# ctu-mrs/vofod

Hardware: AMD Instinct MI355X
Metric: LiDAR frames/sec (131k-pt OS1-128) at 1/2/4/8 MI355X + HBM roofline % (higher is better)
Workload: dtype f32; 1 GPU; os1-128 128x1024 scans, 0.25 m voxels, batched process_scan (configs[1] scan shape in configs[3]'s batched form); points_per_frame=131072, map_voxels=19480981, map_warm_scans=96, gpu_max_hw_queues=4

## Files before the change

vofod_amd/csrc/driver_aux.h:

```cpp
#pragma once

namespace
{

int gscan(vofod_handle* h, const uint32_t* d_in, uint32_t n, uint32_t* d_out, uint32_t* d_bsum, uint32_t* d_total)
{
  const uint32_t nblk = (n + vr::GS_EPB - 1) / vr::GS_EPB;
  if (n == 0)
  {
    HIPCHK(hipMemsetAsync(d_out, 0, sizeof(uint32_t), h->stream));
    if (d_total)
      HIPCHK(hipMemsetAsync(d_total, 0, sizeof(uint32_t), h->stream));
    return VOFOD_OK;
  }
  KLAUNCH(h, vr::k_gscan_a, dim3(nblk), dim3(256), d_in, n, d_bsum);
  KLAUNCH(h, vr::k_gscan_b, dim3(1), dim3(1024), d_bsum, nblk, d_total);
  KLAUNCH(h, vr::k_gscan_c, dim3(nblk), dim3(256), d_in, n, d_bsum, d_out);
  HIPCHK(hipGetLastError());
  return VOFOD_OK;
}

int sep_ensure_words(vofod_handle* h, size_t n_words)
{
  vr::SepState& s = h->sep;
// ... 546 lines not shown
    if (F == 1)
      nt = 1;
    h->pool.reset(new vt::Pool(nt));
  }
  if (do_reset(h) != VOFOD_OK)
    return fail(VOFOD_ERR_DEVICE);
  h->sure_background_sufficient = false;
  h->background_pts_sufficient = false;
  h->last_detection_id = 0;
  (void)hipDeviceSynchronize();
  *out = h;
  return VOFOD_OK;
}

static int world_clear(vofod_handle* h);

int vofod_reset(vofod_handle* h)
{
  if (!h)
    return VOFOD_ERR_INVALID_ARG;
  ApiLock lock(h);
  VCHK(admit(h, WS0_FREE | MAP_UNREAD));
  if (h->world.enabled)
    VCHK(world_clear(h));
  h->wsync.end_chains();
  const int r = do_reset(h);
  h->sure_background_sufficient = false;
  h->background_pts_sufficient = false;
  h->last_detection_id = 0;
  h->cf_off = false;
  forget_detections(h);
  return r;
}

int vofod_set_dynamic_params(vofod_handle* h, const vofod_dyn_params* dp)
{
  if (!h || !dp)
    return VOFOD_ERR_INVALID_ARG;
  ApiLock lock(h, ApiLock::LOCK_ONLY);
  VCHK(admit(h, NEEDS_NOTHING));
  h->dp = *dp;
  return VOFOD_OK;
}

const char* vofod_last_error_string(vofod_handle* h) { return h ? h->err.c_str() : "null handle"; }

int vofod_get_status(vofod_handle* h, vofod_status_info* out)
{
  if (!h || !out)
    return VOFOD_ERR_INVALID_ARG;
  ApiLock lock(h, ApiLock::LOCK_ONLY);
  VCHK(admit(h, NEEDS_NOTHING));
  out->detection_its = h->detection_its;
  out->last_detection_id = h->last_detection_id;
  out->background_pts_sufficient = h->background_pts_sufficient;
  out->sure_background_sufficient = h->sure_background_sufficient;
  out->raycast_pending = h->raycast_pending;
  out->map_size[0] = h->mg.sx;
  out->map_size[1] = h->mg.sy;
  out->map_size[2] = h->mg.sz;
  for (int a = 0; a < 3; a++)
    out->map_offset[a] = h->mg.off[a];
  return VOFOD_OK;
}

int vofod_raycast_begin(vofod_handle* h, const vofod_scan* scan, const float tf[12])
{
  if (!h || !tf)
    return VOFOD_ERR_INVALID_ARG;
  ApiLock lock(h);
  VCHK(admit(h, WS0_FREE));
  return raycast_begin_locked(h, scan, tf, nullptr);
}

int vofod_set_raycast_motion(vofod_handle* h, int on)
{
  if (!h)
    return VOFOD_ERR_INVALID_ARG;
  ApiLock lock(h, ApiLock::LOCK_ONLY);
  VCHK(admit(h, WS0_FREE | MAP_UNREAD | NO_RAYCAST_PASS));
  h->raycast_motion = on != 0;
  return VOFOD_OK;
}

int vofod_set_raycast_exact(vofod_handle* h, int on)
{
  if (!h)
    return VOFOD_ERR_INVALID_ARG;
  ApiLock lock(h, ApiLock::LOCK_ONLY);
  VCHK(admit(h, WS0_FREE | MAP_UNREAD | NO_RAYCAST_PASS));
  if (on && h->ray_log2_units < 0)
  {
    h->err = "exact raycast accumulation: sensor_hrays * sensor_vrays * (2 * voxel_size + 1) does not fit in 32 bits";
    return VOFOD_ERR_INDEX_OVERFLOW;
  }
  h->raycast_exact = on != 0;
  return VOFOD_OK;
}

int vofod_raycast_units(vofod_handle* h, uint32_t* units, size_t n, int32_t* log2_units_per_m)
{
  if (!h || !units || !log2_units_per_m)
    return VOFOD_ERR_INVALID_ARG;
  ApiLock lock(h);
  VCHK(admit(h, NEEDS_NOTHING));
  if (!h->raycast_pending || !h->ray_pass_exact)
    return VOFOD_ERR_NOT_PENDING;
  if (n != h->mg.n)
    return VOFOD_ERR_SIZE_MISMATCH;
  HIPCHK(hipStreamSynchronize(h->stream));
  HIPCHK(hipMemcpy(units, h->d_ray.p, n * sizeof(uint32_t), hipMemcpyDeviceToHost));
  *log2_units_per_m = h->ray_log2_units;
  return VOFOD_OK;
}

int vofod_raycast_finish(vofod_handle* h)
{
  if (!h)
    return VOFOD_ERR_INVALID_ARG;
  ApiLock lock(h);
  VCHK(admit(h, MAP_UNREAD));
  return raycast_finish_locked(h);
}

int vofod_sepclusters_begin(vofod_handle* h, int* sure)
{
  if (!h)
    return VOFOD_ERR_INVALID_ARG;
  ApiLock lock(h);
  VCHK(admit(h, WS0_FREE));
  return sepclusters_begin_locked(h, sure);
}

int vofod_sepclusters_finish(vofod_handle* h)
{
  if (!h)
    return VOFOD_ERR_INVALID_ARG;
  ApiLock lock(h);
  VCHK(admit(h, WS0_FREE | MAP_UNREAD));
  return sepclusters_finish_locked(h);
}

int vofod_voxel_grid_weighted(vofod_handle* h, const vofod_cloud_view* in, float leaf, int align, const float align_center[3], vofod_point_xyzr* out, uint32_t* keys,
                              size_t cap, size_t* n_out, vofod_grid_desc* grid)
{
  if (!h || !in || !(leaf > 0) || (align && !align_center) || in->n > 0x7fffffffu)
    return VOFOD_ERR_INVALID_ARG;
  ApiLock lock(h);
  VCHK(admit(h, WS0_FREE));
  GridParams g;
  FrameHdr hdr{};
  const float l[3] = {leaf, leaf, leaf};
  if (in->n == 0)
  {
    if (n_out)
      *n_out = 0;
    if (grid)
      *grid = vofod_grid_desc{{leaf, leaf, leaf}, {0, 0, 0}, {0, 0, 0}, {0, 0, 0}};
    return VOFOD_OK;
  }
  const int r = voxelize_cloud(h, h->aux, in, g, l, align != 0, align_center, hdr);
  if (r != VOFOD_OK)
  {
    if (n_out)
      *n_out = 0;
    return r;
  }
  return copy_grid_out(h, h->aux, g, hdr, out, keys, cap, n_out, grid);
}

int vofod_voxel_grid_counted(vofod_handle* h, const vofod_cloud_view* in, float leaf, float threshold, vofod_point_xyzr* out, uint32_t* keys, size_t cap, size_t* n_out,
                             vofod_grid_desc* grid)
{
  if (!h || !in || !(leaf > 0) || !in->intensity || in->n > 0x7fffffffu)
    return VOFOD_ERR_INVALID_ARG;
  ApiLock lock(h);
  VCHK(admit(h, WS0_FREE));
  GridParams g;
  FrameHdr hdr{};
  const float l[3] = {leaf, leaf, leaf};
  if (in->n == 0)
  {
    if (n_out)
      *n_out = 0;
    return VOFOD_OK;
  }
  int r = voxelize_cloud(h, h->aux, in, g, l, false, nullptr, hdr);
  if (r != VOFOD_OK)
  {
    if (n_out)
      *n_out = 0;
    return r;
  }
  const uint32_t P = static_cast<uint32_t>(in->n);
  VCHK(sep_ensure_words(h, 1));
  VCHK(sep_ensure_pts(h, P));
  const FrameArgs& a = h->aux.h_args[0];
  KLAUNCH(h, vr::k_flag_over, dim3((P + 255) / 256), dim3(256), a.intensity, a.stride, P, threshold, h->sep.d_sure);
  VCHK(counted_tail(h, h->aux, hdr.V, P, h->sep.d_sure));
  HIPCHK(hipStreamSynchronize(h->stream));
  return copy_grid_out(h, h->aux, g, hdr, out, keys, cap, n_out, grid);
}

int vofod_cluster(vofod_handle* h, const vofod_point_xyzr* pts, const uint32_t* keys, const vofod_grid_desc* grid, size_t n, float tolerance, uint32_t* labels,
                  size_t* n_clusters)
{
  if (!h || (!pts && n) || !labels || !keys || !grid || !(tolerance > 0) || n > 0x7fffffffu)
    return VOFOD_ERR_INVALID_ARG;
  ApiLock lock(h);
  VCHK(admit(h, WS0_FREE));
  if (n_clusters)
    *n_clusters = 0;
  if (n == 0)
    return VOFOD_OK;
  const uint64_t cells = static_cast<uint64_t>(grid->div_b[0]) * grid->div_b[1] * grid->div_b[2];
  if (grid->div_b[0] <= 0 || grid->div_b[1] <= 0 || grid->div_b[2] <= 0 || cells > 0x7fffffffull)
    return VOFOD_ERR_INVALID_ARG;
  for (size_t i = 0; i < n; i++)
    if (keys[i] >= cells || (i && keys[i] <= keys[i - 1]))
    {
      h->err = "vofod_cluster: keys must be strictly ascending lattice keys";
      return VOFOD_ERR_INVALID_ARG;
    }
  Workspace& ws = h->aux;
  const uint32_t words = static_cast<uint32_t>((cells + 63) / 64);
  const uint32_t need_bricks = static_cast<uint32_t>(std::min<uint64_t>(static_cast<uint64_t>((grid->div_b[0] + 3) / 4) * ((grid->div_b[1] + 3) / 4) * ((grid->div_b[2] + 3) / 4), 1u << 28));
  VCHK(grow_workspace(h, ws, "workspace allocation: ", 1, static_cast<uint32_t>(n), static_cast<uint32_t>(n), words + 64, need_bricks));
  GridParams g;
  const float zero[3] = {0, 0, 0};
  fill_grid_params(h, g, grid->leaf, false, zero, ws);
  FrameHdr hdr{};
  hdr.n_in = static_cast<uint32_t>(n);
  hdr.status = VOFOD_OK;
  for (int a = 0; a < 3; a++)
  {
    hdr.offset[a] = grid->offset[a];
    hdr.min_b[a] = grid->min_b[a];
    hdr.div_b[a] = grid->div_b[a];
  }
  hdr.n_cells = static_cast<uint32_t>(cells);
  hdr.n_words = words;
  hdr.V = static_cast<uint32_t>(n);
  std::vector<unsigned long long> bm(words + 2, 0ull);
  for (size_t i = 0; i < n; i++)
    bm[keys[i] >> 6] |= 1ull << (keys[i] & 63);
  std::vector<uint32_t> prefix(words + 2, 0u), ident(n);
  uint32_t run = 0;
  for (uint32_t w = 0; w < words; w++)
  {
    prefix[w] = run;
    run += __builtin_popcountll(bm[w]);
  }
  for (size_t i = 0; i < n; i++)
    ident[i] = static_cast<uint32_t>(i);
  std::vector<int32_t> cbox(6 * n);
  for (size_t i = 0; i < n; i++)
    for (int c = 0; c < 3; c++)
    {
      cbox[6 * i + c] = 0x7fffffff;
      cbox[6 * i + 3 + c] = static_cast<int32_t>(0x80000000u);
    }
  HIPCHK(hipMemcpyAsync(ws.d_hdrs, &hdr, sizeof(hdr), hipMemcpyHostToDevice, h->stream));
  ws.bitmap_clean = false;
  HIPCHK(hipMemcpyAsync(ws.d_bitmaps, bm.data(), sizeof(unsigned long long) * (words + 2), hipMemcpyHostToDevice, h->stream));
  HIPCHK(hipMemcpyAsync(ws.d_wprefix, prefix.data(), sizeof(uint32_t) * (words + 2), hipMemcpyHostToDevice, h->stream));
  HIPCHK(hipMemcpyAsync(ws.va.pts, pts, sizeof(float4) * n, hipMemcpyHostToDevice, h->stream));
  HIPCHK(hipMemcpyAsync(ws.va.key, keys, sizeof(uint32_t) * n, hipMemcpyHostToDevice, h->stream));
  HIPCHK(hipMemcpyAsync(ws.va.parent, ident.data(), sizeof(uint32_t) * n, hipMemcpyHostToDevice, h->stream));
  HIPCHK(hipMemsetAsync(ws.va.csize, 0, sizeof(uint32_t) * n, h->stream));
  HIPCHK(hipMemsetAsync(ws.va.cclose, 0, sizeof(uint32_t) * n, h->stream));
  HIPCHK(hipMemcpyAsync(ws.va.cbox, cbox.data(), sizeof(int32_t) * 6 * n, hipMemcpyHostToDevice, h->stream));
  float cmax = 0;
  for (int a = 0; a < 3; a++)
    cmax = std::max({cmax, std::fabs(grid->offset[a]), std::fabs(grid->offset[a] + grid->leaf[a] * (grid->div_b[a] + 1))});
  vofod_handle::ClusterTables* ct = nullptr;
  VCHK(cluster_tables(h, g, tolerance, cmax, &ct));
  VCHK(launch_cluster(h, ws, plan_cluster_only(h, ws, ct), g, ct));
  HIPCHK(hipMemcpyAsync(labels, ws.d_labels, sizeof(uint32_t) * n, hipMemcpyDeviceToHost, h->stream));
  HIPCHK(hipStreamSynchronize(h->stream));
  if (n_clusters)
  {
    size_t c = 0;
    for (size_t i = 0; i < n; i++)
      c += labels[i] == i;
    *n_clusters = c;
  }
  return VOFOD_OK;
}

int vofod_profile_enable(vofod_handle* h, int on)
{
  if (!h)
    return VOFOD_ERR_INVALID_ARG;
  ApiLock lock(h);
  VCHK(admit(h, NEEDS_NOTHING));
  (void)hipStreamSynchronize(h->stream);
  for (auto& r : h->prof.recs)
  {
    h->prof.pool.push_back(r.a);
    h->prof.pool.push_back(r.b);
  }
  h->prof.recs.clear();
  h->prof.on = on != 0;
  return VOFOD_OK;
}

size_t vofod_profile_read(vofod_handle* h, char* names, double* ms, uint64_t* calls, size_t cap)
{
  if (!h || !names || !ms || !calls)
    return 0;
  ApiLock lock(h);
  if (admit(h, NEEDS_NOTHING) != VOFOD_OK)
    return 0;
  (void)hipStreamSynchronize(h->stream);
  std::vector<std::string> order;
  std::map<std::string, std::pair<double, uint64_t>> acc;
  for (auto& r : h->prof.recs)
  {
    float t = 0;
    (void)hipEventElapsedTime(&t, r.a, r.b);
    std::string nm = r.name;
    const size_t c = nm.rfind(':');
    if (c != std::string::npos)
      nm = nm.substr(c + 1);
    if (!acc.count(nm))
      order.push_back(nm);
    acc[nm].first += t;
    acc[nm].second += 1;
    h->prof.pool.push_back(r.a);
    h->prof.pool.push_back(r.b);
  }
  h->prof.recs.clear();
  size_t n = 0;
  for (const auto& nm : order)
  {
    if (n >= cap)
      break;
    std::memset(names + 64 * n, 0, 64);
    std::strncpy(names + 64 * n, nm.c_str(), 63);
    ms[n] = acc[nm].first;
    calls[n] = acc[nm].second;
    n++;
  }
  return n;
}

}
```

vofod_amd/csrc/frame_prof.h:

```cpp
#pragma once

namespace
{

struct Quantiles
{
  double mean = 0, median = 0, p90 = 0, max = 0;
  explicit Quantiles(std::vector<double>& v)
  {
    std::sort(v.begin(), v.end());
    for (double x : v)
      mean += x / v.size();
    median = v[v.size() / 2];
    p90 = v[v.size() * 9 / 10];
    max = v.back();
  }
  void json(FILE* fp, const char* name) const { std::fprintf(fp, "\"%s\": {\"mean\": %.2f, \"median\": %.2f, \"p90\": %.2f, \"max\": %.2f}", name, mean, median, p90, max); }
};

int slab_emit_prof_buffer(vofod_handle* h, unsigned long long*& d_prof)
{
  if (!h->d_prof_slab && std::getenv("VOFOD_LDS_PROF"))
    HIPCHK(h->d_prof_slab.alloc(16 * 4096));
  d_prof = h->d_prof_slab;
  return VOFOD_OK;
}

int print_slab_emit_prof(vofod_handle* h, uint32_t n)
{
  std::vector<unsigned long long> all(16 * n);
  HIPCHK(hipStreamSynchronize(h->stream));
  HIPCHK(hipMemcpy(all.data(), h->d_prof_slab, sizeof(unsigned long long) * 16 * n, hipMemcpyDeviceToHost));
  const unsigned long long* t = all.data();
  std::fprintf(stderr, "[k_slab_emit] keys %.1f | zero %.1f mark %.1f count+scan %.1f out+emit %.1f us (all slabs of frame 0)\n", t[0] * 0.01, t[1] * 0.01, t[2] * 0.01, t[3] * 0.01, t[4] * 0.01);
  unsigned long long t0 = ~0ull, t1 = 0;
  for (uint32_t f = 0; f < n; f++)
  {
    t0 = std::min(t0, all[16 * f + 5]);
    t1 = std::max(t1, all[16 * f + 6]);
  }
  double smax = 0;
  std::vector<double> dur;
  std::vector<std::pair<double, uint32_t>> byd;
  for (uint32_t f = 0; f < n; f++)
  {
    dur.push_back((all[16 * f + 6] - all[16 * f + 5]) * 0.01);
    byd.push_back({dur.back(), f});
    smax = std::max(smax, (all[16 * f + 5] - t0) * 0.01);
  }
  std::sort(byd.begin(), byd.end());
  for (size_t q : {size_t(0), byd.size() / 4, byd.size() / 2, 3 * byd.size() / 4, byd.size() - 1})
  {
    const uint32_t f = byd[q].second;
    std::fprintf(stderr, "[k_slab_emit]   frame %u: %.1f us, keys %llu, zero %.1f mark %.1f count %.1f emit %.1f\n", f, byd[q].first, all[16 * f + 7], all[16 * f + 1] * 0.01, all[16 * f + 2] * 0.01,
                 all[16 * f + 3] * 0.01, all[16 * f + 4] * 0.01);
  }
  const Quantiles q(dur);
  std::fprintf(stderr, "[k_slab_emit] %u workgroups: span %.1f us, per-workgroup min %.1f mean %.1f max %.1f us, latest start +%.1f us\n", n, (t1 - t0) * 0.01, dur.front(), q.mean, q.max, smax);
  return VOFOD_OK;
}

int frame_prof_slots(vofod_handle* h, Workspace& ws, unsigned long long*& d_prof)
{
  DevBuf<unsigned long long>& d_prof_all = h->d_prof_ccl;
  if (!d_prof_all && std::getenv("VOFOD_LDS_PROF"))
  {
    HIPCHK(d_prof_all.alloc(FR_PROF_WORDS));
    HIPCHK(hipMemset(d_prof_all, 0, sizeof(unsigned long long) * FR_PROF_WORDS));
  }
  ws.prof_deferred = false;
  uint32_t prof_slot0 = 0;
  if (d_prof_all && std::atoi(std::getenv("VOFOD_LDS_PROF") ? std::getenv("VOFOD_LDS_PROF") : "0") == 2 && ws.F <= 256)
    for (int t = 0; t < vofod_handle::MAX_INFLIGHT; t++)
      if (&ws == h->slot(t))
      {
        ws.prof_deferred = true;
        prof_slot0 = 256u * static_cast<uint32_t>(t);
      }
  ws.prof_slot0 = prof_slot0;
  d_prof = d_prof_all ? d_prof_all + 32 * static_cast<size_t>(prof_slot0) : nullptr;
  return VOFOD_OK;
}

int print_frame_prof(vofod_handle* h, uint32_t s0, uint32_t cnt, bool sync)
{
  unsigned long long* d_prof = h->d_prof_ccl;
  std::vector<unsigned long long> t(32 * cnt);
  if (sync)
    HIPCHK(hipStreamSynchronize(h->stream));
  HIPCHK(hipMemcpy(t.data(), d_prof + 32 * static_cast<size_t>(s0), sizeof(unsigned long long) * 32 * cnt, hipMemcpyDeviceToHost));
  unsigned long long* d_wave = d_prof + 32 * static_cast<size_t>(FR_PROF_FRAMES) + 32 * static_cast<size_t>(s0);
  std::vector<unsigned long long> tw(32 * cnt);
  HIPCHK(hipMemcpy(tw.data(), d_wave, sizeof(unsigned long long) * 32 * cnt, hipMemcpyDeviceToHost));
  if (const char* rawf = std::getenv("VOFOD_LDS_PROF_RAW"))
  {
    struct RawLog
    {
      std::vector<unsigned long long> v;
      std::string path;
      uint64_t launch = 0;
      ~RawLog()
      {
        if (FILE* fp = std::fopen(path.c_str(), "w"))
        {
          for (size_t i = 0; i + 3 < v.size(); i += 4)
            std::fprintf(fp, "%llu %.2f %.2f %u %u %u %u\n", v[i], v[i + 1] * 0.01, v[i + 2] * 0.01, static_cast<unsigned>(v[i + 3] >> 32) & 15u, static_cast<unsigned>(v[i + 3] >> 13) & 7u,
                         static_cast<unsigned>(v[i + 3] >> 12) & 1u, static_cast<unsigned>(v[i + 3] >> 8) & 15u);
          std::fclose(fp);
        }
      }
    };
    static RawLog log;
    log.path = rawf;
    for (uint32_t f = 0; f < cnt; f++)
      if (t[32 * f + 13])
      {
        const unsigned long long rec[4] = {log.launch, t[32 * f], t[32 * f + 13], t[32 * f + 21]};
        log.v.insert(log.v.end(), rec, rec + 4);
      }
    log.launch++;
    HIPCHK(hipMemsetAsync(d_prof + 32 * static_cast<size_t>(s0), 0, sizeof(unsigned long long) * 32 * cnt, h->stream));
    HIPCHK(hipMemsetAsync(d_wave, 0, sizeof(unsigned long long) * 32 * cnt, h->stream));
    return VOFOD_OK;
  }
  static const char* names[13] = {"bits", "prefix", "words", "rank-a/b", "rank-c", "emit", "extras", "probe", "adjacent", "far", "exact", "minima+stats", "labels"};
  std::vector<std::pair<double, uint32_t>> byd;
  unsigned long long t0 = ~0ull, t1 = 0;
  for (uint32_t f = 0; f < cnt; f++)
  {
    if (!t[32 * f + 13])
      continue;
    byd.push_back({(t[32 * f + 13] - t[32 * f]) * 0.01, f});
    t0 = std::min(t0, t[32 * f]);
    t1 = std::max(t1, t[32 * f + 13]);
  }
  std::sort(byd.begin(), byd.end());
  double mean = 0;
  for (auto& b : byd)
    mean += b.first / byd.size();
  for (size_t q : {size_t(0), byd.size() / 2, byd.size() - 1})
  {
    if (byd.empty())
      break;
    const uint32_t f = byd[q].second;
    if (t[32 * f + 31] == ~0ull)
    {
      auto us = [&](int a, int b) { return (t[32 * f + b] - t[32 * f + a]) * 0.01; };
      const double t_count = us(15, 14), t_closebits = us(3, 15);
      std::fprintf(stderr,
                   "[k_frame_lds_far] frame %u: %.1f us | keys %llu V %llu bricks %llu pure-far bricks %llu far clusters %llu candidate members %llu | input+fragile %.1f prefix %.1f words %.1f count %.1f closebits "
                   "%.1f rank-a/b %.1f rank-c %.1f emit %.1f extras %.1f near+far %.1f open %.1f stats %.1f table %.1f members %.1f\n",
                   f, byd[q].first, t[32 * f + 27], t[32 * f + 29], t[32 * f + 26], t[32 * f + 24], t[32 * f + 25], t[32 * f + 30], us(0, 1), us(1, 2), us(2, 3), t_count, t_closebits, us(14, 4), us(4, 5),
                   us(5, 6), us(6, 7), us(7, 8), us(8, 9), us(9, 10), us(10, 11), us(11, 13));
      continue;
    }
    std::fprintf(stderr, "[k_frame_lds] frame %u: %.1f us | keys %llu V %llu bricks %llu extras %llu hits %llu open %llu surviving %llu |", f, byd[q].first, t[32 * f + 27], t[32 * f + 29],
                 t[32 * f + 26], t[32 * f + 28], t[32 * f + 24], t[32 * f + 25], t[32 * f + 30]);
    for (int i = 0; i < 13; i++)
      std::fprintf(stderr, " %s %.1f", names[i], (t[32 * f + i + 1] - t[32 * f + i]) * 0.01);
    std::fprintf(stderr, " (count %.1f of rank-a/b; %llu bricks outside the largest component, %llu far hits)\n", (t[32 * f + 14] - t[32 * f + 3]) * 0.01, t[32 * f + 31] & 0xffffffffull,
                 t[32 * f + 31] >> 32);
  }
  if (!byd.empty())
    std::fprintf(stderr, "[k_frame_lds] %zu workgroups: span %.1f us, mean %.1f us\n", byd.size(), (t1 - t0) * 0.01, mean);
  if (const char* jf = std::getenv("VOFOD_LDS_PROF_JSON"); jf && !byd.empty() && t[32 * byd[0].second + 31] == ~0ull)
  {
    static const int cuts[][2] = {{0, 16}, {16, 17}, {17, 18}, {18, 19}, {19, 20}, {20, 1}, {1, 2}, {2, 3}, {15, 14}, {3, 15}, {14, 4}, {4, 5}, {5, 6}, {6, 7}, {7, 8}, {8, 9}, {9, 10}, {10, 11}, {11, 13}, {0, 13}};
    static const char* cnames[] = {"input", "input_wait", "grid", "grid_wait", "fragile", "fragile_wait", "prefix", "words", "count", "closebits", "rank_ab", "rank_c", "emit", "extras_restore", "cf_edges", "cf_open", "cf_stats", "cf_table", "cf_members", "total"};
    if (FILE* fp = std::fopen(jf, "a"))
    {
      double busy = 0;
      for (auto& b : byd)
        busy += b.first;
      std::fprintf(fp, "{\"frames\": %zu, \"span_us\": %.1f, \"t0_abs_us\": %.1f, \"busy_us_sum\": %.1f, \"phases\": {", byd.size(), (t1 - t0) * 0.01, t0 * 0.01, busy);
      for (size_t c = 0; c < sizeof(cuts) / sizeof(cuts[0]); c++)
      {
        std::vector<double> v;
        for (auto& b : byd)
          v.push_back((t[32 * b.second + cuts[c][1]] - t[32 * b.second + cuts[c][0]]) * 0.01);
        std::fprintf(fp, "%s", c ? ", " : "");
        Quantiles(v).json(fp, cnames[c]);
      }
      std::vector<double> st, en;
      for (auto& b : byd)
      {
        st.push_back((t[32 * b.second] - t0) * 0.01);
        en.push_back((t[32 * b.second + 13] - t0) * 0.01);
      }
      std::sort(st.begin(), st.end());
      std::sort(en.begin(), en.end());
      std::vector<double> w_mean, w_last, w_share;
      for (auto& b : byd)
      {
        const unsigned long long* w = &tw[32 * b.second];
        const unsigned long long f0 = t[32 * b.second];
        double e_sum = 0, e_max = 0, s_sum = 0;
        int nw = 0;
        for (int k = 0; k < FR_THREADS / 64; k++)
          if (w[2 * k] > f0)
          {
            const double e = (w[2 * k] - f0) * 0.01;
            e_sum += e;
            e_max = std::max(e_max, e);
            s_sum += w[2 * k + 1] / e;
            nw++;
          }
        if (nw)
        {
          w_mean.push_back(e_sum / nw);
          w_last.push_back(e_max);
          w_share.push_back(s_sum / nw);
        }
      }
      std::fprintf(fp, "}");
      if (!w_mean.empty())
      {
        std::fprintf(fp, ", \"input_waves\": {");
        Quantiles(w_mean).json(fp, "mean_wave_end");
        std::fprintf(fp, ", ");
        Quantiles(w_last).json(fp, "last_wave_end");
        std::fprintf(fp, ", ");
        Quantiles(w_share).json(fp, "load_wait_pct");
        std::fprintf(fp, "}");
      }
      std::fprintf(fp, ", \"start_us\": {\"median\": %.1f, \"max\": %.1f}, \"end_us\": {\"median\": %.1f, \"max\": %.1f}", st[st.size() / 2], st.back(), en[en.size() / 2], en.back());
      std::vector<double> bx, ex, fi, to, lag;
      for (auto& b : byd)
      {
        const unsigned long long a0 = t[32 * b.second + 22], pk = t[32 * b.second + 23];
        if (!a0)
          continue;
        const double d1 = (pk & 0xfffffull) * 0.01, d2 = ((pk >> 20) & 0xfffffull) * 0.01, d3 = ((pk >> 40) & 0xfffffull) * 0.01;
        bx.push_back(d1);
        ex.push_back(d2 - d1);
        fi.push_back(d3 - d2);
        to.push_back(d3);
        lag.push_back((static_cast<double>(a0) - static_cast<double>(t[32 * b.second + 13])) * 0.01);
      }
      if (!to.empty())
      {
        std::fprintf(fp, ", \"tail\": {");
        Quantiles(bx).json(fp, "boxes_gates");
        std::fprintf(fp, ", ");
        Quantiles(ex).json(fp, "flood_fills");
        std::fprintf(fp, ", ");
        Quantiles(fi).json(fp, "records");
        std::fprintf(fp, ", ");
        Quantiles(to).json(fp, "total");
        std::fprintf(fp, ", ");
        Quantiles(lag).json(fp, "start_after_frame_end");
        std::fprintf(fp, "}");
      }
      std::fprintf(fp, "}\n");
      std::fclose(fp);
    }
  }
  HIPCHK(hipMemset(d_prof + 32 * static_cast<size_t>(s0), 0, sizeof(unsigned long long) * 32 * cnt));
  HIPCHK(hipMemset(d_wave, 0, sizeof(unsigned long long) * 32 * cnt));
  return VOFOD_OK;
}

int print_deferred_prof(vofod_handle* h, Workspace& ws, uint32_t n)
{
  if (!ws.prof_deferred || !h->d_prof_ccl)
    return VOFOD_OK;
  ws.prof_deferred = false;
  return print_frame_prof(h, ws.prof_slot0, n, false);
}

}
```

vofod_amd/csrc/frames_collect.h:

```cpp
#pragma once

namespace
{

int adopt_status(vofod_handle* h, Workspace& ws, uint32_t n)
{
  if (ws.plan.dtail)
    for (uint32_t f = 0; f < n; f++)
      ws.h_packed[f].hdr.status = ws.h_dets[f].status;
  for (uint32_t f = 0; f < n; f++)
    if (ws.h_packed[f].hdr.status == CCL_RETRY_STATUS)
    {
      h->lds_ccl_off = true;
      ws.rerun = true;
      ws.job_n = n;
      ws.bitmap_clean = false;
      return CCL_RETRY_STATUS;
    }
  return VOFOD_OK;
}

void book_map_images(vofod_handle* h, Workspace& ws)
{
  if (ws.plan.mapbits_patched && ws.h_packed[0].hdr.status == VOFOD_OK && h->mapbits_valid)
  {
    h->bgcount_stale = true;
    h->mapbits_gen++;
  }
  else
    h->mapbits_valid = false;
}

int check_close_first_overflow(vofod_handle* h, Workspace& ws, uint32_t n)
{
  for (uint32_t f = 0; f < n; f++)
    if (ws.h_packed[f].hdr.status == CF_RETRY_STATUS)
    {
      h->cf_off = true;
      h->cf_off_bg = h->n_bg_voxels;
      ws.rerun = true;
      ws.job_n = n;
      return CCL_RETRY_STATUS;
    }
  return VOFOD_OK;
}

struct RecordSink
{
  vofod_handle* h;
  Workspace& ws;
  const FrameCall& call;
  vofod_detection* out;
  size_t cap;
  uint32_t* n_out_per_frame;
  size_t total = 0, frame_begin = 0;
  RecordSink(vofod_handle* h_, Workspace& ws_, const FrameCall& call_, vofod_detection* out_, size_t cap_, uint32_t* n_out_per_frame_)
      : h(h_), ws(ws_), call(call_), out(out_), cap(cap_), n_out_per_frame(n_out_per_frame_)
  {
    ws.det_begin(call.submitted, call.g);
  }
  void add(uint32_t f, uint32_t root, const float center[3], uint32_t n_points, double conf_sum)
  {
    const vofod_detection det = vt::make_detection(h->last_detection_id++, call.tfs + 12 * f, center, n_points, conf_sum, f, h->sp, *call.dp);
    ws.det_refs.push_back({det.id, f, root, n_points});
    if (out && total < cap)
      out[total] = det;
    total++;
  }
  void frame_done(uint32_t f)
  {
    if (n_out_per_frame)
      n_out_per_frame[f] = static_cast<uint32_t>(total - frame_begin);
    frame_begin = total;
  }
  int close(int ret, size_t* n_out)
  {
    *n_out = total;
    if (total > cap)
      ret = VOFOD_ERR_CAPACITY;
    ws.det_valid = ret == VOFOD_OK;
    return ret;
  }
};

int device_tail_records(vofod_handle* h, Workspace& ws, const FrameCall& call, vofod_detection* out, size_t cap, uint32_t* n_out_per_frame, size_t* n_out)
{
  const uint32_t n = call.n;
  int ret = VOFOD_OK;
  if (call.submitted && out)
  {
    size_t need = 0;
    for (uint32_t f = 0; f < n; f++)
      need += ws.h_dets[f].n;
    if (need > cap)
    {
      ws.pending = true;
      *n_out = need;
      return VOFOD_ERR_CAPACITY;
    }
  }
  RecordSink sink(h, ws, call, out, cap, n_out_per_frame);
  for (uint32_t f = 0; f < n; f++)
  {
    const vtd::FrameDets& D = ws.h_dets[f];
    if (D.status != VOFOD_OK)
      ret = D.status;
    for (uint32_t i = 0; i < D.n; i++)
      sink.add(f, D.d[i].root, D.d[i].center, D.d[i].n_points, D.d[i].conf_sum);
    sink.frame_done(f);
  }
  if (trace_on())
    std::fprintf(stderr, "[vofod trace] n=%u device tail: sync %.3f end %.3f ms, %zu detections\n", n, call.tr_sync1, ms_since(call.t0), sink.total);
  return sink.close(ret, n_out);
}

int device_tail_overflow_records(vofod_handle* h, Workspace& ws, const FrameCall& call, uint32_t fb, vofod_detection* out, size_t cap, uint32_t* n_out_per_frame, size_t* n_out)
{
  if (fb & vtd::TAIL_FB_EXPLORE)
  {
    h->err = "device tail: flood-fill work list overflow";
    return VOFOD_ERR_DEVICE;
  }
  std::vector<vtd::TailCluster> tc(vtd::TP_MAXC);
  std::vector<vc::ExploreResult> res(vtd::TP_MAXC);
  HIPCHK(hipMemcpy(tc.data(), ws.d_tailc, sizeof(vtd::TailCluster) * vtd::TP_MAXC, hipMemcpyDeviceToHost));
  HIPCHK(hipMemcpy(res.data(), h->explore.d_results, sizeof(vc::ExploreResult) * vtd::TP_MAXC, hipMemcpyDeviceToHost));
  RecordSink sink(h, ws, call, out, cap, n_out_per_frame);
  for (int c = 0; c < vtd::TP_MAXC; c++)
    if (tc[c].job >= 0 && tc[c].job < vtd::TP_MAXC && res[tc[c].job].floating)
      sink.add(0u, tc[c].root, tc[c].obb_center, tc[c].n_members, res[tc[c].job].conf_sum);
  sink.frame_done(0u);
  return sink.close(VOFOD_OK, n_out);
}

struct FrameTail
{
  std::vector<HostCluster> cl;
  vt::MemberIndex by_root;
  std::vector<int> job_of;
  bool host_fallback = false;
  std::vector<ClusterRec> recs_big;
  std::vector<CandMemberX> members_big;
  bool big_recs = false, big_members = false;
  std::vector<vc::ExploreJob> jobs;
  std::vector<int> members;
};

struct ExploreWork
{
  std::vector<vc::ExploreJob> jobs;
  std::vector<uint32_t> job_begin;
  std::vector<int> job_members;
  std::vector<vc::ExploreResult> results;
};

int fetch_big_tables(vofod_handle* h, Workspace& ws, const GridParams& g, uint32_t n, std::vector<FrameTail>& tails, int& ret)
{
  for (uint32_t f = 0; f < n; f++)
  {
    FrameTail& T = tails[f];
    const FrameHdr& hdr = ws.h_packed[f].hdr;
    if (hdr.status != VOFOD_OK)
      ret = hdr.status;
    T.big_recs = hdr.C > SPEC_C;
    T.big_members = hdr.n_cand > SPEC_M;
    if (T.big_recs)
    {
      T.recs_big.resize(hdr.C);
      HIPCHK(hipMemcpy(T.recs_big.data(), ws.d_table + static_cast<size_t>(f) * ws.vox_cap, sizeof(ClusterRec) * hdr.C, hipMemcpyDeviceToHost));
    }
    if (T.big_members)
    {
      T.members_big.resize(hdr.n_cand);
      CandMemberX* d_tmp = static_cast<CandMemberX*>(ws.d_members_big);
      KLAUNCH(h, k_gather_members, dim3((hdr.n_cand + 255) / 256), dim3(256), g, f, hdr.n_cand, ws.d_cand, ws.va, d_tmp);
      HIPCHK(hipMemcpyAsync(T.members_big.data(), d_tmp, sizeof(CandMemberX) * hdr.n_cand, hipMemcpyDeviceToHost, h->stream));
      HIPCHK(hipStreamSynchronize(h->stream));
    }
  }
  return VOFOD_OK;
}

void prep_frame_tail(const vofod_handle* h, const PackedFrame& pf, uint32_t f, const float* tf, const vt::TailParams& tp, FrameTail& T)
{
  const FrameHdr& hdr = pf.hdr;
  const ClusterRec* recs = T.big_recs ? T.recs_big.data() : pf.table;
  const CandMemberX* members = T.big_members ? T.members_big.data() : pf.members;
  T.cl.resize(hdr.C);
  for (uint32_t c = 0; c < hdr.C; c++)
    T.cl[c].rec = recs[c];
  std::sort(T.cl.begin(), T.cl.end(), [](const HostCluster& a, const HostCluster& b) {
    if (a.rec.size != b.rec.size)
      return a.rec.size > b.rec.size;
    return a.rec.root < b.rec.root;
  });
  {
    std::vector<std::pair<uint64_t, vt::Member>> tmp(hdr.n_cand);
    for (uint32_t i = 0; i < hdr.n_cand; i++)
    {
      const CandMemberX& m = members[i];
      tmp[i] = {(static_cast<uint64_t>(m.root) << 32) | m.v, vt::Member{m.v, {m.x, m.y, m.z}, m.count}};
    }
    T.by_root.build(tmp);
  }
  T.job_of.assign(hdr.C, -1);
  std::vector<vc::ExploreJob>& jl = T.jobs;
  std::vector<int>& ml = T.members;
  for (uint32_t ci = 0; ci < hdr.C; ci++)
  {
    HostCluster& c = T.cl[ci];
    if (c.rec.close)
      continue;
    c.cclass = VOFOD_CLASS_INVALID;
    if (!c.rec.cand)
      continue;
    const vt::MemberSpan mem = T.by_root.of(c.rec.root);
    auto get = [&](size_t i, float p[3]) {
      for (int a = 0; a < 3; a++)
        p[a] = mem[i].p[a];
    };
    c.gates = vt::classify_gates(static_cast<uint32_t>(mem.size()), get, tf, tp, h->hg.off, h->hg.vs_inv, h->hg.s);
    if (c.gates.passed && !c.gates.explore)
      c.cclass = VOFOD_CLASS_UNKNOWN;
    if (!c.gates.explore)
      continue;
    vc::ExploreJob job{};
    job.frame = f;
    job.n_members = static_cast<uint32_t>(mem.size());
    job.member_off = static_cast<uint32_t>(ml.size() / 3);
    job.R = c.gates.R;
    for (int a = 0; a < 3; a++)
    {
      job.box_lo[a] = c.gates.box_lo[a];
      job.box_hi[a] = c.gates.box_hi[a];
    }
    for (const vt::Member& m : mem)
    {
      int o[3];
      h->hg.coordToIdx(m.p, o);
      ml.insert(ml.end(), o, o + 3);
    }
    if (job.R > vc::EX_MAX_R || job.R < 0)
      T.host_fallback = true;
    T.job_of[ci] = static_cast<int>(jl.size());
    jl.push_back(job);
  }
  if (jl.size() > vc::EX_MAX_JOBS)
    T.host_fallback = true;
}

void concat_jobs(std::vector<FrameTail>& tails, ExploreWork& w)
{
  const uint32_t n = static_cast<uint32_t>(tails.size());
  w.job_begin.assign(n + 1, 0);
  for (uint32_t f = 0; f < n; f++)
  {
    w.job_begin[f] = static_cast<uint32_t>(w.jobs.size());
    const uint32_t jbase = static_cast<uint32_t>(w.jobs.size()), mbase = static_cast<uint32_t>(w.job_members.size() / 3);
    for (vc::ExploreJob j : tails[f].jobs)
    {
      j.member_off += mbase;
      j.result_slot = static_cast<uint32_t>(w.jobs.size());
      w.jobs.push_back(j);
    }
    w.job_members.insert(w.job_members.end(), tails[f].members.begin(), tails[f].members.end());
    for (int& ji : tails[f].job_of)
      if (ji >= 0)
        ji += static_cast<int>(jbase);
  }
  w.job_begin[n] = static_cast<uint32_t>(w.jobs.size());
  w.results.resize(w.jobs.size());
}

int explore_on_device(vofod_handle* h, const FrameCall& call, ExploreWork& w, float thr_new, bool no_update)
{
  const uint32_t n = call.n;
  VCHK(ensure_explore(h, h->explore, h->ws.F, w.jobs.size(), w.job_members.size() / 3));
  StreamScope tail_scope(h, call.submitted ? h->stream_tail : nullptr);
  ExploreBufs& eb = h->explore;
  if (h->ev_explore)
    HIPCHK(hipStreamWaitEvent(h->stream, h->ev_explore, 0));
  HIPCHK(hipMemcpyAsync(eb.d_jobs, w.jobs.data(), sizeof(vc::ExploreJob) * w.jobs.size(), hipMemcpyHostToDevice, h->stream));
  HIPCHK(hipMemcpyAsync(eb.d_job_begin, w.job_begin.data(), sizeof(uint32_t) * (n + 1), hipMemcpyHostToDevice, h->stream));
  HIPCHK(hipMemcpyAsync(eb.d_members, w.job_members.data(), sizeof(int) * w.job_members.size(), hipMemcpyHostToDevice, h->stream));
  const vc::ExploreParams ep = explore_params(*call.dp, thr_new, no_update);
  KLAUNCH(h, vc::k_explore, dim3(n), dim3(64), ep, h->mg, eb.d_jobs, eb.d_job_begin, eb.d_job_begin + 1, eb.d_members, h->d_map, eb.d_overlay, eb.d_stack, eb.d_explored, eb.d_touched,
          eb.d_ovl_list, eb.d_ovl_count, eb.d_results, eb.d_visited);
  HIPCHK(hipMemcpyAsync(w.results.data(), eb.d_results, sizeof(vc::ExploreResult) * w.jobs.size(), hipMemcpyDeviceToHost, h->stream));
  if (h->ev_explore)
    HIPCHK(hipEventRecord(h->ev_explore, h->stream));
  HIPCHK(hipStreamSynchronize(h->stream));
  if (!no_update)
    h->mapbits_valid = false;
  return VOFOD_OK;
}

void extract_detections(RecordSink& sink, const FrameTail& T, uint32_t f, const std::vector<vc::ExploreResult>& results)
{
  for (size_t ci = 0; ci < T.cl.size(); ci++)
  {
    const HostCluster& c = T.cl[ci];
    if (c.rec.close || c.cclass != VOFOD_CLASS_MAV)
      continue;
    sink.add(f, c.rec.root, c.gates.obb_center, static_cast<uint32_t>(T.by_root.of(c.rec.root).size()), results[T.job_of[ci]].conf_sum);
  }
  sink.frame_done(f);
}

int fill_debug_view(vofod_handle* h, Workspace& ws, const GridParams& g, uint32_t f, const FrameTail& T, bool far_view, vofod_scan_debug& d, int& ret)
{
  const FrameHdr& hdr = ws.h_packed[f].hdr;
  d.n_input_after_crop = hdr.n_in;
  d.n_bg_voxels = h->n_bg_voxels;
  d.background_pts_sufficient = h->background_pts_sufficient;
  d.sure_background_sufficient = h->sure_background_sufficient;
  uint32_t n_shown = hdr.C;
  if (far_view && !hdr.far_only)
  {
    n_shown = 0;
    for (uint32_t c = 0; c < hdr.C; c++)
      n_shown += T.cl[c].rec.close ? 0u : 1u;
  }
  d.n_weighted = hdr.V;
  d.n_clusters = n_shown;
  if ((d.weighted || d.labels) && d.weighted_cap < hdr.V)
    ret = VOFOD_ERR_CAPACITY;
  else
  {
    if (d.weighted && hdr.V)
      HIPCHK(hipMemcpy(d.weighted, ws.va.pts + static_cast<size_t>(f) * ws.vox_cap, sizeof(float4) * hdr.V, hipMemcpyDeviceToHost));
    if (d.labels && hdr.V)
    {
      HIPCHK(hipMemcpy(d.labels, ws.d_labels + static_cast<size_t>(f) * ws.vox_cap, sizeof(uint32_t) * hdr.V, hipMemcpyDeviceToHost));
      if (far_view && !hdr.far_only)
      {
        std::vector<uint32_t> far_roots;
        for (uint32_t c = 0; c < hdr.C; c++)
          if (!T.cl[c].rec.close)
            far_roots.push_back(T.cl[c].rec.root);
        std::sort(far_roots.begin(), far_roots.end());
        for (uint32_t v = 0; v < hdr.V; v++)
          if (!std::binary_search(far_roots.begin(), far_roots.end(), d.labels[v]))
            d.labels[v] = CF_LABEL_NONE;
      }
    }
  }
  if (d.clusters)
  {
    if (d.clusters_cap < n_shown)
      ret = VOFOD_ERR_CAPACITY;
    else
      for (uint32_t c = 0, c_out = 0; c < hdr.C; c++)
      {
        const HostCluster& hc = T.cl[c];
        if (far_view && hc.rec.close)
          continue;
        vofod_cluster_info& ci = d.clusters[c_out++];
        ci.first_member = hc.rec.root;
        ci.n_points = hc.rec.size;
        ci.is_close = hc.rec.close;
        ci.cclass = hc.cclass;
        for (int a = 0; a < 3; a++)
        {
          ci.aabb_min[a] = (static_cast<float>(hc.rec.imin[a]) + 0.5f) * g.leaf[a] + hdr.offset[a];
          ci.aabb_max[a] = (static_cast<float>(hc.rec.imax[a]) + 0.5f) * g.leaf[a] + hdr.offset[a];
          ci.obb_center[a] = hc.gates.evaluated ? hc.gates.obb_center[a] : NAN;
        }
        ci.obb_size = hc.gates.obb_size;
      }
  }
  return VOFOD_OK;
}

int host_tail(vofod_handle* h, Workspace& ws, const FrameCall& call, const double dev_ms[4], vofod_detection* out, size_t cap, uint32_t* n_out_per_frame, size_t* n_out)
{
  const uint32_t n = call.n;
  const vofod_dyn_params& dp = *call.dp;
  vofod_scan_debug* dbg = call.dbg;
  const bool no_update = call.flags & VOFOD_SCAN_NO_MAP_UPDATE;
  const auto t_tail = clk::now();
  const float thr_new = static_cast<float>(dp.voxel_map__thresholds__new_obstacles);
  const float thr_frontiers = static_cast<float>(dp.voxel_map__thresholds__frontiers);
  const vt::TailParams tp = tail_params(h, dp);
  int ret = VOFOD_OK;
  std::vector<FrameTail> tails(n);
  ExploreWork w;
  VCHK(fetch_big_tables(h, ws, call.g, n, tails, ret));
  h->pool->parallel_for(n, [&](uint32_t f) { prep_frame_tail(h, ws.h_packed[f], f, call.tfs + 12 * f, tp, tails[f]); });
  concat_jobs(tails, w);
  const double tr_prep = ms_since(call.t0);

  bool any_host = std::getenv("VOFOD_EXPLORE") && std::strcmp(std::getenv("VOFOD_EXPLORE"), "host") == 0;
  for (const FrameTail& T : tails)
    any_host |= T.host_fallback;
  if (!w.jobs.empty() && !any_host)
    VCHK(explore_on_device(h, call, w, thr_new, no_update));
  const double tr_explore = ms_since(call.t0);

  RecordSink sink(h, ws, call, out, cap, n_out_per_frame);
  for (uint32_t f = 0; f < n; f++)
  {
    FrameTail& T = tails[f];
    if (any_host && w.job_begin[f + 1] > w.job_begin[f])
    {
      VCHK(host_explore_frame(h, T.cl, T.by_root, T.job_of, w.jobs, w.results, no_update, thr_frontiers, thr_new, dp));
    }
    for (size_t ci = 0; ci < T.cl.size(); ci++)
      if (const int ji = T.job_of[ci]; ji >= 0)
        T.cl[ci].cclass = w.results[ji].floating ? VOFOD_CLASS_MAV : VOFOD_CLASS_UNKNOWN;
    extract_detections(sink, T, f, w.results);
    if (dbg)
    {
      vofod_scan_debug& d = dbg[f];
      VCHK(fill_debug_view(h, ws, call.g, f, T, dbg[0].far_only != 0, d, ret));
      for (int i = 0; i < 4; i++)
        d.stage_ms[i] = dev_ms[i];
      d.stage_ms[4] = ms_since(t_tail);
      d.stage_ms[5] = ms_since(call.t0);
    }
  }
  if (trace_on())
  {
    size_t sumC = 0, sumCand = 0, sumEval = 0;
    for (uint32_t f = 0; f < n; f++)
    {
      sumC += ws.h_packed[f].hdr.C;
      sumCand += ws.h_packed[f].hdr.n_cand;
      for (const auto& c : tails[f].cl)
        sumEval += c.gates.evaluated;
    }
    std::fprintf(stderr, "[vofod trace] n=%u launch %.3f sync1 %.3f prep %.3f explore %.3f end %.3f ms jobs %zu C %zu cand_members %zu evaluated %zu\n", n, call.tr_launch, call.tr_sync1, tr_prep,
                 tr_explore, ms_since(call.t0), w.jobs.size(), sumC, sumCand, sumEval);
  }
  return sink.close(ret, n_out);
}

int collect_frames(vofod_handle* h, Workspace& ws, FrameCall& call, vofod_detection* out, size_t cap, uint32_t* n_out_per_frame, size_t* n_out)
{
  const uint32_t n = call.n;
  if (n == 0)
  {
    GridParams g{};
    g.vox_cap = ws.vox_cap;
    ws.det_begin(call.submitted, g);
    ws.det_valid = true;
    return VOFOD_OK;
  }
  const bool no_update = call.flags & VOFOD_SCAN_NO_MAP_UPDATE;
  if (call.submitted)
  {
    HIPCHK(hipEventSynchronize(ws.ev_done));
    ws.pending = false;
  }
  else
    HIPCHK(hipStreamSynchronize(h->stream));
  VCHK(print_deferred_prof(h, ws, n));
  call.tr_sync1 = ms_since(call.t0);

  VCHK(adopt_status(h, ws, n));
  if (!no_update)
    book_map_images(h, ws);
  VCHK(latch_background(h));
  VCHK(check_close_first_overflow(h, ws, n));
  if (!no_update && !call.rc_done)
  {
    h->detection_its++;
    if (call.flags & VOFOD_SCAN_AUTO_RAYCAST)
    {
      if (h->raycast_pending)
        raycast_finish_locked(h);
      else
        raycast_begin_locked(h, &call.scans[0], call.tfs, staged_pose_table(ws, call.scans[0]));
    }
  }
  double dev_ms[4] = {0, 0, 0, 0};
  if (call.dbg)
    for (int i = 0; i < 4; i++)
    {
      float ms = 0;
      (void)hipEventElapsedTime(&ms, call.ev[i], call.ev[i + 1]);
      dev_ms[i] = ms;
    }

  if (ws.plan.dtail)
  {
    uint32_t fb = 0;
    for (uint32_t f = 0; f < n; f++)
      fb |= ws.h_dets[f].fallback;
    if (!fb)
      return device_tail_records(h, ws, call, out, cap, n_out_per_frame, n_out);
    if (!no_update && (fb & (vtd::TAIL_FB_DETS | vtd::TAIL_FB_EXPLORE)))
      return device_tail_overflow_records(h, ws, call, fb, out, cap, n_out_per_frame, n_out);
    VCHK(read_back_full(h, ws, call.g, n));
    HIPCHK(hipStreamSynchronize(h->stream));
  }
  return host_tail(h, ws, call, dev_ms, out, cap, n_out_per_frame, n_out);
}

template <class First, class Again>
int with_reruns(First&& first, Again&& again)
{
  int r = first();
  for (int attempt = 0; attempt < 2 && r == CCL_RETRY_STATUS; attempt++)
    r = again();
  return r;
}

int process_frames(vofod_handle* h, const vofod_scan* scans, const float* tfs, uint32_t n, int flags, vofod_detection* out, size_t cap, uint32_t* n_out_per_frame, size_t* n_out,
                   vofod_scan_debug* dbg)
{
  auto once = [&] {
    FrameCall call{false, scans, tfs, n, flags, dbg};
    const int r = launch_frames(h, h->ws, call);
    return r != VOFOD_OK ? r : collect_frames(h, h->ws, call, out, cap, n_out_per_frame, n_out);
  };
  return with_reruns(once, once);
}

}
```

vofod_amd/csrc/frames_launch.h:

```cpp
#pragma once

namespace
{

struct FrameCall
{
  bool submitted;
  const vofod_scan* scans;
  const float* tfs;
  uint32_t n;
  int flags;
  vofod_scan_debug* dbg;
  const vofod_dyn_params* dp = nullptr;
  GridParams g{};
  bool rc_done = false;
  hipStream_t tail_stream_used = nullptr;
  DevEvent ev[5];
  clk::time_point t0 = clk::now();
  double tr_launch = 0, tr_sync1 = 0;
};

struct LaunchRoute
{
  bool staged = false;
  hipStream_t chain = nullptr;
  int own_tail = -1;
};

struct StreamScope
{
  vofod_handle* h;
  hipStream_t saved;
  explicit StreamScope(vofod_handle* h_, hipStream_t st = nullptr) : h(h_), saved(h_->stream)
  {
    if (st)
      h->stream = st;
  }
  ~StreamScope() { h->stream = saved; }
};

int ensure_chain_stream(vofod_handle* h, int t)
{
  if (!h->chain_stream[t])
    HIPCHK(h->chain_stream[t].create(hipStreamCreateWithFlags, hipStreamNonBlocking));
  return VOFOD_OK;
}

int slot_index(vofod_handle* h, const Workspace& ws)
{
  for (int t = 0; t < vofod_handle::MAX_INFLIGHT; t++)
    if (&ws == h->slot(t))
      return t;
  return -1;
}

inline bool trace_on()
{
  static const bool v = std::getenv("VOFOD_TRACE") != nullptr;
  return v;
}

int latch_background(vofod_handle* h)
{
  if (h->bgcount_fresh)
  {
    if (h->ev_bgcount)
      HIPCHK(hipEventSynchronize(h->ev_bgcount));
    uint64_t t = 0;
    for (int i = 0; i < MB_SLOTS; i++)
      t += h->h_bgcount[8 * i];
    h->n_bg_voxels = t;
    h->bgcount_fresh = false;
  }
  if (h->n_bg_voxels > h->background_min_sufficient_pts)
    h->background_pts_sufficient = true;
  return VOFOD_OK;
}

vc::ExploreParams explore_params(const vofod_dyn_params& dp, float thr_new, bool no_update)
{
  vc::ExploreParams ep{};
  ep.thr_unknown = static_cast<float>(dp.voxel_map__thresholds__frontiers);
  ep.thr_ground = thr_new;
  ep.frontier_value = static_cast<float>(dp.voxel_map__thresholds__frontiers);
  ep.ray_score = dp.voxel_map__scores__ray;
  ep.no_update = no_update ? 1 : 0;
  ep.stack_cap = vc::EX_CELLS;
  return ep;
}

vt::TailParams tail_params(const vofod_handle* h, const vofod_dyn_params& dp)
{
  vt::TailParams tp{};
  tp.min_points = dp.classification__min_points;
  tp.max_distance = dp.classification__max_distance;
  tp.max_size = dp.classification__max_size;
  tp.max_explore = dp.classification__max_explore_distance;
  tp.voxel_size = h->sp.voxel_size;
  tp.latches = (h->background_pts_sufficient && h->sure_background_sufficient) ? 1 : 0;
  return tp;
}

int read_back_full(vofod_handle* h, Workspace& ws, const GridParams& g, uint32_t n)
{
  KLAUNCH(h, k_pack, fgrid(g, (std::max(SPEC_C, SPEC_M) + 255) / 256), dim3(256), g, ws.d_hdrs, ws.d_table, ws.d_cand, ws.va, ws.d_packed);
  HIPCHK(hipMemcpyAsync(ws.h_packed, ws.d_packed, sizeof(PackedFrame) * n, hipMemcpyDeviceToHost, h->stream));
  return VOFOD_OK;
}

int route_submitted(vofod_handle* h, const Workspace& ws, uint32_t n, LaunchRoute& rt)
{
  if (!h->stream_key || !h->stream_frame || n < 128u)
  {
    const int t = slot_index(h, ws);
    if (t >= 1)
    {
      VCHK(ensure_chain_stream(h, t));
      rt.chain = h->chain_stream[t];
    }
    if (n < 128u)
      rt.own_tail = t;
  }
  else
  {
    rt.chain = h->stream_key;
    rt.staged = true;
  }
  return VOFOD_OK;
}

inline bool is_range_image(const vofod_scan& s) { return !s.x && !s.y && !s.z && s.range; }

inline int check_col_tfs(vofod_handle* h, const vofod_scan& s)
{
  if (!s.col_tfs)
    return VOFOD_OK;
  if (!is_range_image(s) && !h->point_motion)
  {
    h->err = "col_tfs: only a range image (x == y == z == NULL) may carry a pose per column unless vofod_set_point_motion is on";
    return VOFOD_ERR_INVALID_ARG;
  }
  if (s.memspace == VOFOD_MEM_DEVICE && reinterpret_cast<uintptr_t>(s.col_tfs) % 4 != 0)
  {
    h->err = "device-resident col_tfs: the table must be 4-byte aligned";
    return VOFOD_ERR_INVALID_ARG;
  }
  return VOFOD_OK;
}

int pose_slot(vofod_handle* h, Workspace& ws, size_t k, const float* src, hipStream_t st, float*& slot)
{
  const size_t tab = static_cast<size_t>(h->sp.sensor_hrays) * 12;
  if (!ws.d_poses)
    HIPCHK(ws.d_poses.alloc(static_cast<size_t>(ws.F) * tab));
  slot = ws.d_poses + k * tab;
  if (src)
    HIPCHK(hipMemcpyAsync(slot, src, tab * sizeof(float), hipMemcpyHostToDevice, st));
  return VOFOD_OK;
}

int stage_pose_tables(vofod_handle* h, Workspace& ws, const vofod_scan* scans, uint32_t n)
{
  const size_t tab = static_cast<size_t>(h->sp.sensor_hrays) * 12;
  std::vector<const float*> host;
  std::vector<const float**> entry_of;
  uint32_t jm = 0, jp = 0;
  for (uint32_t f = 0; f < n; f++)
  {
    if (!scans[f].col_tfs)
      continue;
    const float** entry = is_range_image(scans[f]) ? &ws.h_rjobs.p[jm++].poses : &ws.h_pjobs.p[jp++].poses;
    if (scans[f].memspace != VOFOD_MEM_DEVICE)
    {
      host.push_back(scans[f].col_tfs);
      entry_of.push_back(entry);
    }
  }
  if (host.empty())
    return VOFOD_OK;
  const ptrdiff_t pitch = host.size() >= 2 ? reinterpret_cast<const char*>(host[1]) - reinterpret_cast<const char*>(host[0]) : 0;
  bool constant = pitch >= static_cast<ptrdiff_t>(tab * sizeof(float));
  for (size_t k = 2; k < host.size() && constant; k++)
    constant = reinterpret_cast<const char*>(host[k]) == reinterpret_cast<const char*>(host[0]) + static_cast<ptrdiff_t>(k) * pitch;
  for (size_t k = 0; k < host.size(); k++)
  {
    float* slot = nullptr;
    VCHK(pose_slot(h, ws, k, constant ? nullptr : host[k], h->stream, slot));
    *entry_of[k] = slot;
  }
  if (constant)
    HIPCHK(hipMemcpy2DAsync(ws.d_poses, tab * sizeof(float), host[0], static_cast<size_t>(pitch), tab * sizeof(float), host.size(), hipMemcpyHostToDevice, h->stream));
  return VOFOD_OK;
}

inline const float* staged_pose_table(const Workspace& ws, const vofod_scan& s) { return s.col_tfs ? ws.first_poses : nullptr; }

int stage_inputs(vofod_handle* h, Workspace& ws, const vofod_scan* scans, const float* tfs, uint32_t n, size_t npts, bool& host_copies)
{
  bool staged_2d = false;
  ws.det_valid = false;
  ws.n_rjobs = ws.n_mjobs = ws.n_pjobs = 0;
  ws.first_poses = nullptr;
  vrd::RangeJob* const jobs = ws.h_rjobs.p;
  uint32_t n_jobs = 0;
  vpd::PointJob* const pjobs = ws.h_pjobs.p;
  uint32_t n_pjobs = 0;
  auto slot = [&](uint32_t f) { return ws.d_stage + static_cast<size_t>(f) * ws.pt_cap * 5; };
  auto slot_args = [&](uint32_t f) {
    float* base = slot(f);
    return stage_cloud(h, ws, f, base, base + ws.pt_cap, base + 2 * static_cast<size_t>(ws.pt_cap), nullptr, nullptr, 4, npts, VOFOD_MEM_DEVICE, FA_SCAN, tfs + 12 * f);
  };
  if (n >= 2 && scans[0].memspace == VOFOD_MEM_HOST && scans[0].x)
  {
    const char* x0 = static_cast<const char*>(scans[0].x);
    const ptrdiff_t pitch = static_cast<const char*>(scans[1].x) - x0;
    bool ok = pitch >= static_cast<ptrdiff_t>(npts * 12);
    for (uint32_t f = 0; f < n && ok; f++)
    {
      const vofod_scan& s = scans[f];
      const char* xf = x0 + static_cast<ptrdiff_t>(f) * pitch;
      ok = s.memspace == VOFOD_MEM_HOST && s.stride_bytes == 4 && static_cast<const char*>(s.x) == xf && static_cast<const char*>(s.y) == xf + npts * 4 &&
           static_cast<const char*>(s.z) == xf + npts * 8;
    }
    if (ok && ws.pt_cap == npts)
    {
      HIPCHK(hipMemcpy2DAsync(ws.d_stage, sizeof(float) * 5 * ws.pt_cap, x0, static_cast<size_t>(pitch), npts * 12, n, hipMemcpyHostToDevice, h->stream));
      for (uint32_t f = 0; f < n; f++)
      {
        VCHK(slot_args(f));
        if (scans[f].col_tfs)
          pjobs[n_pjobs++] = vpd::PointJob{ws.h_args[f].x, ws.h_args[f].y, ws.h_args[f].z, slot(f), 4, scans[f].col_tfs};
      }
      staged_2d = true;
    }
  }
  if (n >= 2 && scans[0].memspace == VOFOD_MEM_HOST && is_range_image(scans[0]))
  {
    const char* r0 = static_cast<const char*>(scans[0].range);
    const ptrdiff_t pitch = static_cast<const char*>(scans[1].range) - r0;
    bool ok = pitch >= static_cast<ptrdiff_t>(npts * 4);
    for (uint32_t f = 0; f < n && ok; f++)
    {
      const vofod_scan& s = scans[f];
      ok = s.memspace == VOFOD_MEM_HOST && is_range_image(s) && s.stride_bytes == 4 && static_cast<const char*>(s.range) == r0 + static_cast<ptrdiff_t>(f) * pitch;
    }
    if (ok)
    {
      HIPCHK(hipMemcpy2DAsync(ws.d_stage + 4 * static_cast<size_t>(ws.pt_cap), sizeof(float) * 5 * ws.pt_cap, r0, static_cast<size_t>(pitch), npts * 4, n, hipMemcpyHostToDevice, h->stream));
      for (uint32_t f = 0; f < n; f++)
      {
        VCHK(slot_args(f));
        jobs[n_jobs++] = vrd::RangeJob{reinterpret_cast<const char*>(slot(f) + 4 * static_cast<size_t>(ws.pt_cap)), slot(f), 4, scans[f].col_tfs};
      }
      staged_2d = true;
    }
  }
  host_copies = staged_2d;
  for (uint32_t f = 0; f < n && !staged_2d; f++)
  {
    const vofod_scan& s = scans[f];
    host_copies |= s.memspace != VOFOD_MEM_DEVICE;
    if (!is_range_image(s))
    {
      VCHK(stage_cloud(h, ws, f, s.x, s.y, s.z, nullptr, nullptr, s.stride_bytes, npts, s.memspace, FA_SCAN, tfs + 12 * f));
      if (!s.col_tfs)
        continue;
      if (s.memspace == VOFOD_MEM_DEVICE &&
          (s.stride_bytes % 4 != 0 || (reinterpret_cast<uintptr_t>(s.x) | reinterpret_cast<uintptr_t>(s.y) | reinterpret_cast<uintptr_t>(s.z)) % 4 != 0))
      {
        h->err = "device-resident point scan with col_tfs: the columns' bases and stride must be multiples of 4 bytes";
        return VOFOD_ERR_INVALID_ARG;
      }
      const FrameArgs& a = ws.h_args[f];
      pjobs[n_pjobs++] = vpd::PointJob{a.x, a.y, a.z, slot(f), a.stride, s.col_tfs};
      VCHK(slot_args(f));
      continue;
    }
    vrd::RangeJob job{static_cast<const char*>(s.range), slot(f), s.stride_bytes, s.col_tfs};
    if (s.memspace != VOFOD_MEM_DEVICE)
    {
      VCHK(stage_host_column(h, slot(f) + 4 * static_cast<size_t>(ws.pt_cap), s.range, s.stride_bytes, npts));
      job.src = reinterpret_cast<const char*>(slot(f) + 4 * static_cast<size_t>(ws.pt_cap));
      job.stride = 4;
    }
    else if (s.stride_bytes % 4 != 0 || reinterpret_cast<uintptr_t>(s.range) % 4 != 0)
    {
      h->err = "device-resident range column: base and stride must be multiples of 4 bytes";
      return VOFOD_ERR_INVALID_ARG;
    }
    VCHK(slot_args(f));
    jobs[n_jobs++] = job;
  }
  ws.n_mjobs = static_cast<uint32_t>(std::stable_partition(jobs, jobs + n_jobs, [](const vrd::RangeJob& job) { return job.poses != nullptr; }) - jobs);
  ws.n_rjobs = n_jobs - ws.n_mjobs;
  ws.n_pjobs = n_pjobs;
  if (ws.n_mjobs || n_pjobs)
    VCHK(stage_pose_tables(h, ws, scans, n));
  ws.first_poses = !scans[0].col_tfs ? nullptr : is_range_image(scans[0]) ? jobs[0].poses : pjobs[0].poses;
  if (n_jobs)
    HIPCHK(hipMemcpyAsync(ws.d_rjobs, jobs, sizeof(vrd::RangeJob) * n_jobs, hipMemcpyHostToDevice, h->stream));
  if (n_pjobs)
    HIPCHK(hipMemcpyAsync(ws.d_pjobs, pjobs, sizeof(vpd::PointJob) * n_pjobs, hipMemcpyHostToDevice, h->stream));
  return VOFOD_OK;
}

int deskew_points(vofod_handle* h, Workspace& ws, size_t npts)
{
  if (!ws.n_pjobs || !npts)
    return VOFOD_OK;
  bool vec = npts % 4 == 0 && ws.pt_cap % 4 == 0, pose16 = true;
  for (uint32_t j = 0; j < ws.n_pjobs; j++)
  {
    const vpd::PointJob& job = ws.h_pjobs.p[j];
    vec = vec && job.stride == 4 &&
          (reinterpret_cast<uintptr_t>(job.x) | reinterpret_cast<uintptr_t>(job.y) | reinterpret_cast<uintptr_t>(job.z) | reinterpret_cast<uintptr_t>(job.dst)) % 16 == 0;
    pose16 = pose16 && reinterpret_cast<uintptr_t>(job.poses) % 16 == 0;
  }
  vrd::MotionArgs ma{};
  ma.shift = h->d_col_shift.p;
  ma.width = static_cast<uint32_t>(h->sp.sensor_hrays);
  exclude_box(h, ma.lo, ma.hi);
  const uint32_t n_px = static_cast<uint32_t>(npts), per_block = vpd::PD_THREADS * (vec ? 4u : 1u);
  const dim3 grid((n_px + per_block - 1) / per_block, ws.n_pjobs);
  auto pick = [&](auto v) {
    constexpr bool V = decltype(v)::value;
    return pose16 ? vpd::k_point_deskew_t<V, true> : vpd::k_point_deskew_t<V, false>;
  };
  auto kern = vec ? pick(std::true_type{}) : pick(std::false_type{});
  KLAUNCH_AS(h, "k_point_deskew", kern, grid, dim3(vpd::PD_THREADS), ws.d_pjobs.p, n_px, ws.pt_cap, ma);
  HIPCHK(hipGetLastError());
  return VOFOD_OK;
}

int decode_span(vofod_handle* h, Workspace& ws, size_t npts, bool motion, uint32_t first, uint32_t n_jobs)
{
  if (!n_jobs)
    return VOFOD_OK;
  bool vec = npts % 4 == 0 && ws.pt_cap % 4 == 0, pose16 = true;
  for (uint32_t j = first; j < first + n_jobs; j++)
  {
    const vrd::RangeJob& job = ws.h_rjobs.p[j];
    vec = vec && job.stride == 4 && reinterpret_cast<uintptr_t>(job.src) % 16 == 0;
    pose16 = pose16 && reinterpret_cast<uintptr_t>(job.poses) % 16 == 0;
  }
  vrd::MotionArgs ma{};
  if (motion)
  {
    ma.shift = h->d_col_shift.p;
    ma.width = static_cast<uint32_t>(h->sp.sensor_hrays);
    exclude_box(h, ma.lo, ma.hi);
  }
  const uint32_t chunk = std::min(std::max(n_jobs / 16u, 1u), vrd::RD_CHUNK_MAX);
  const uint32_t n_px = static_cast<uint32_t>(npts), threads = vec ? n_px / 4u : n_px;
  const dim3 grid((threads + vrd::RD_THREADS - 1) / vrd::RD_THREADS, (n_jobs + chunk - 1) / chunk);
  auto pick = [&](auto v) {
    constexpr bool V = decltype(v)::value;
    return !motion ? vrd::k_range_decode_t<V, false, true> : pose16 ? vrd::k_range_decode_t<V, true, true> : vrd::k_range_decode_t<V, true, false>;
  };
  auto kern = vec ? pick(std::true_type{}) : pick(std::false_type{});
  KLAUNCH_AS(h, motion ? "k_range_decode_motion" : "k_range_decode", kern, grid, dim3(vrd::RD_THREADS), ws.d_rjobs.p + first, n_jobs, chunk, n_px, ws.pt_cap, h->d_lut_dirs.p, h->d_lut_offs.p, ma);
  HIPCHK(hipGetLastError());
  return VOFOD_OK;
}

int decode_ranges(vofod_handle* h, Workspace& ws, size_t npts)
{
  VCHK(decode_span(h, ws, npts, true, 0, ws.n_mjobs));
  return decode_span(h, ws, npts, false, ws.n_mjobs, ws.n_rjobs);
}

struct H2DGuard
{
  hipEvent_t ev;
  bool armed;
  ~H2DGuard()
  {
    if (armed)
      (void)hipEventSynchronize(ev);
  }
};

int prepare_map_images(vofod_handle* h, const vofod_dyn_params& dp, float thr_new, bool use_dilated, bool want_bgcount, CloseParams& cpar)
{
  VCHK(ensure_mapbits(h, thr_new));
  if (want_bgcount)
    VCHK(refresh_bgcount(h));
  if (!h->closetab.valid || h->closetab.max_dist != static_cast<float>(dp.ground_points_max_distance))
  {
    std::vector<CloseRow> crows;
    if (const int r = build_close_rows(static_cast<float>(dp.ground_points_max_distance), h->mg.vs_inv, crows); r != VOFOD_OK)
    {
      h->err = "ground_points_max_distance / voxel_size exceeds the 63-bit window";
      return r;
    }
    HIPCHK(hipMemcpy(h->d_crows, crows.data(), sizeof(CloseRow) * crows.size(), hipMemcpyHostToDevice));
    h->closetab.valid = true;
    h->closetab.max_dist = static_cast<float>(dp.ground_points_max_distance);
    h->closetab.n_rows = static_cast<int>(crows.size());
  }
  cpar = CloseParams{h->closetab.n_rows, thr_new};
  if (use_dilated)
    return ensure_mapclose(h, cpar);
  return VOFOD_OK;
}

int enter_frame_stream(vofod_handle* h, Workspace& ws)
{
  HIPCHK(hipEventRecord(ws.ev_key, h->stream));
  h->frame_toggle = (h->frame_toggle + 1) % std::max(h->n_frame_streams, 1);
  h->stream = h->stream_frames[h->frame_toggle];
  HIPCHK(hipStreamWaitEvent(h->stream, ws.ev_key, 0));
  return VOFOD_OK;
}

int cluster_far_single(vofod_handle* h, Workspace& ws, const vplan::ChainPlan& plan, const GridParams& g, const vofod_handle::ClusterTables* ct, const CloseParams& cpar, const UpdateParams& up,
                       float thr_new)
{
  const uint32_t gv = (ws.vox_cap + 255u) / 256u;
  uint32_t* far_list = ws.d_labels;
  KLAUNCH(h, k_closefar, fgrid(g, gv), dim3(256), g, h->mg, cpar, h->d_crows, ws.d_hdrs, h->d_mapbits, ws.va, static_cast<const uint32_t*>(nullptr), static_cast<const unsigned long long*>(nullptr), ws.d_cand,
          ws.d_hdrs);
  KLAUNCH(h, k_closefar_sweep, fgrid(g, (ws.vox_cap * 16u + 255u) / 256u), dim3(256), g, h->mg, cpar, h->d_crows, ws.d_hdrs, h->d_mapbits, ws.va, ws.d_cand, far_list, ws.d_hdrs, ws.vox_cap);
  const uint32_t items = FAR_MAX * 2u * static_cast<uint32_t>(ct->n_rows);
  KLAUNCH(h, k_far_edges, dim3((items + 255u) / 256u), dim3(256), g, ct->cp, ct->d_rows, ws.d_hdrs, ws.d_bitmaps, ws.d_wprefix, ws.va, far_list);
  KLAUNCH(h, k_far_final, dim3(1), dim3(1024), g, ws.d_hdrs, ws.va, far_list, up, ws.d_table, ws.d_cand);
  KLAUNCH(h, k_finalize_far, dim3(gv), dim3(256), g, h->mg, up, ws.d_hdrs, ws.va, h->d_map, h->d_flags, ws.d_bitmaps, plan.mapbits_patched ? h->d_mapbits : nullptr, h->d_bgcount, thr_new);
  return VOFOD_OK;
}

int closefar_and_finalize(vofod_handle* h, Workspace& ws, const vplan::ChainPlan& plan, const GridParams& g, const CloseParams& cpar, const UpdateParams& up, vofod_scan_debug* dbg, const DevEvent* ev)
{
  const uint32_t gv = (ws.vox_cap + 255u) / 256u;
  if (plan.closefar != vplan::CloseFar::Fused)
  {
    const bool split = plan.closefar == vplan::CloseFar::Split;
    KLAUNCH(h, k_closefar, fgrid(g, gv), dim3(256), g, h->mg, cpar, h->d_crows, ws.d_hdrs, h->d_mapbits, ws.va, ws.d_labels, plan.use_dilated ? h->d_mapclose : nullptr,
            split ? ws.d_cand : nullptr, ws.d_hdrs);
    if (split)
      KLAUNCH(h, k_closefar_sweep, fgrid(g, (ws.vox_cap * 16u + 255u) / 256u), dim3(256), g, h->mg, cpar, h->d_crows, ws.d_hdrs, h->d_mapbits, ws.va, ws.d_cand);
  }
  if (dbg)
    HIPCHK(hipEventRecord(ev[3], h->stream));
  if (plan.finalize == vplan::Finalize::Finalize)
    KLAUNCH(h, k_finalize, fgrid(g, gv), dim3(256), g, h->mg, up, ws.d_hdrs, ws.va, ws.d_labels, h->d_map, h->d_flags, ws.d_table, ws.d_cand, plan.keep_dirty ? nullptr : ws.d_bitmaps);
  return VOFOD_OK;
}

int raycast_ahead_of_tail(vofod_handle* h, Workspace& ws, FrameCall& call)
{
  HIPCHK(hipMemcpyAsync(&ws.h_packed[0].hdr, ws.d_hdrs, sizeof(FrameHdr), hipMemcpyDeviceToHost, h->stream));
  HIPCHK(hipStreamSynchronize(h->stream));
  if (ws.h_packed[0].hdr.status == VOFOD_OK)
  {
    h->detection_its++;
    if (h->raycast_pending)
      raycast_finish_locked(h);
    else
      raycast_begin_locked(h, &call.scans[0], call.tfs, staged_pose_table(ws, call.scans[0]));
    call.rc_done = true;
  }
  return VOFOD_OK;
}

int launch_device_tail(vofod_handle* h, Workspace& ws, const vplan::ChainPlan& plan, const LaunchRoute& rt, FrameCall& call)
{
  const uint32_t n = call.n;
  const GridParams& g = call.g;
  const vofod_dyn_params& dp = *call.dp;
  VCHK(latch_background(h));
  ExploreBufs& eb = rt.own_tail >= 0 ? h->explore_slot[rt.own_tail] : h->explore;
  const uint32_t ebF = rt.own_tail >= 0 ? std::max<uint32_t>(eb.F(), (n + 31u) & ~31u) : h->ws.F;
  VCHK(ensure_explore(h, eb, ebF, static_cast<size_t>(ebF) * vtd::TP_MAXC, static_cast<size_t>(ebF) * vtd::TP_MAXM));
  hipStream_t chain_stream = h->stream;
  StreamScope tail_scope(h);
  if (!h->ev_explore)
    HIPCHK(h->ev_explore.create(hipEventCreateWithFlags, hipEventDisableTiming));
  if (rt.own_tail >= 0)
    ;
  else if (call.submitted && h->stream_tail)
  {
    HIPCHK(hipEventRecord(ws.ev_packed, chain_stream));
    h->stream = h->stream_tail;
    HIPCHK(hipStreamWaitEvent(h->stream, ws.ev_packed, 0));
  }
  else
    HIPCHK(hipStreamWaitEvent(h->stream, h->ev_explore, 0));
  const vt::TailParams tp = tail_params(h, dp);
  const vc::ExploreParams ep = explore_params(dp, static_cast<float>(dp.voxel_map__thresholds__new_obstacles), plan.no_update);
  static const bool diag_no_tail = std::getenv("VOFOD_DIAG_NO_TAIL") != nullptr;
  if (diag_no_tail && n >= 128u)
    ;
  else if (plan.tail == vplan::Tail::Far)
    KLAUNCH(h, vtd::k_tail_far, dim3((n + vtd::TAIL_WPB - 1) / vtd::TAIL_WPB), dim3(64 * vtd::TAIL_WPB), g, ws.d_hdrs, ws.d_args, ws.d_table, ws.d_cand, ws.va, h->mg, tp, ep, eb.d_jobs, eb.d_members, h->d_map, eb.d_overlay, eb.d_stack, eb.d_explored, eb.d_touched,
            eb.d_ovl_list, eb.d_ovl_count, eb.d_results, eb.d_visited, ws.d_dets, ws.h_dets_dev, plan.far_single ? ws.d_tailc : static_cast<vtd::TailCluster*>(nullptr),
            (ws.prof_deferred && h->d_prof_ccl && !plan.far_single) ? h->d_prof_ccl + 32 * static_cast<size_t>(ws.prof_slot0) : static_cast<unsigned long long*>(nullptr));
  else
  {
    KLAUNCH(h, vtd::k_tail_prep, dim3(n), dim3(vtd::TP_THREADS), g, ws.d_hdrs, ws.d_args, ws.d_table, ws.d_cand, ws.va, h->mg, tp, eb.d_jobs, ws.d_job_be, ws.d_job_be + ws.F, eb.d_members, ws.d_tailc,
            ws.d_dets);
    KLAUNCH(h, vc::k_explore, dim3(n), dim3(64), ep, h->mg, eb.d_jobs, ws.d_job_be, ws.d_job_be + ws.F, eb.d_members, h->d_map, eb.d_overlay, eb.d_stack, eb.d_explored, eb.d_touched, eb.d_ovl_list,
            eb.d_ovl_count, eb.d_results, eb.d_visited);
    KLAUNCH(h, vtd::k_tail_finish, dim3(n), dim3(64), ws.d_tailc, eb.d_results, ws.d_dets, ws.h_dets_dev);
  }
  if (rt.own_tail < 0)
    HIPCHK(hipEventRecord(h->ev_explore, h->stream));
  call.tail_stream_used = h->stream;
  return VOFOD_OK;
}

int launch_frames(vofod_handle* h, Workspace& ws, FrameCall& call)
{
  const vofod_static_params& sp = h->sp;
  const bool submitted = call.submitted;
  const uint32_t n = call.n;
  vofod_scan_debug* dbg = call.dbg;
  ws.det_valid = false;
  if (submitted && !ws.rerun)
    ws.job_dp = h->dp;
  call.dp = submitted ? &ws.job_dp : &h->dp;
  const vofod_dyn_params& dp = *call.dp;
  if (n == 0)
    return VOFOD_OK;
  if (n > ws.F)
  {
    h->err = "batch larger than max_batch_frames";
    return VOFOD_ERR_CAPACITY;
  }
  const size_t npts = static_cast<size_t>(sp.sensor_hrays) * sp.sensor_vrays;
  for (uint32_t f = 0; f < n; f++)
  {
    const vofod_scan& s = call.scans[f];
    if ((!s.x || !s.y || !s.z) && !is_range_image(s))
      return VOFOD_ERR_INVALID_ARG;
    VCHK(check_col_tfs(h, s));
    if (static_cast<size_t>(s.width) * s.height != npts)
      return VOFOD_ERR_SIZE_MISMATCH;
  }
  const bool rerun = ws.rerun && ws.job_n == n;
  ws.rerun = false;
  DevEvent* ev = call.ev;
  if (dbg)
    for (int i = 0; i < 5; i++)
      HIPCHK(ev[i].create(hipEventCreate));
  const float thr_new = static_cast<float>(dp.voxel_map__thresholds__new_obstacles);

  const vplan::Switches sw = vplan::read_switches();
  const bool no_update = call.flags & VOFOD_SCAN_NO_MAP_UPDATE;
  const bool use_dilated = vplan::wants_dilated(sw, no_update, n);
  LaunchRoute rt;
  if (submitted)
    VCHK(route_submitted(h, ws, n, rt));
  StreamScope chain_scope(h, rt.chain);
  if (submitted && h->ev_stagger_set)
    HIPCHK(hipStreamWaitEvent(h->stream, h->ev_stagger, 0));
  if (submitted && !(h->mapbits_valid && h->mapbits_thr == thr_new))
  {
    VCHK(ensure_mapbits(h, thr_new));
    HIPCHK(hipStreamSynchronize(h->stream));
  }

  bool host_copies = false;
  if (!rerun)
    VCHK(stage_inputs(h, ws, call.scans, call.tfs, n, npts, host_copies));
  if (host_copies && submitted && ws.ev_h2d)
    HIPCHK(hipEventRecord(ws.ev_h2d, h->stream));
  else
    host_copies = false;
  H2DGuard h2d_guard{ws.ev_h2d, host_copies};
  if (!rerun)
  {
    VCHK(decode_ranges(h, ws, npts));
    VCHK(deskew_points(h, ws, npts));
  }

  GridParams& g = call.g;
  const float leaf[3] = {sp.voxel_size, sp.voxel_size, sp.voxel_size};
  const int zero[3] = {0, 0, 0};
  float align_center[3];
  h->hg.idxToCoord(zero, align_center);
  fill_grid_params(h, g, leaf, true, align_center, ws);
  CloseParams cpar{};
  VCHK(prepare_map_images(h, dp, thr_new, use_dilated, !h->background_pts_sufficient || dbg, cpar));
  if (dbg)
    HIPCHK(hipEventRecord(ev[0], h->stream));

  vofod_handle::ClusterTables* ct = nullptr;
  VCHK(cluster_tables(h, g, static_cast<float>(dp.ground_points_max_distance), map_cmax(h), &ct));
  const bool rerun_off_lds = h->lds_ccl_off;
  h->lds_ccl_off = false;
  if (h->cf_off)
    VCHK(latch_background(h));
  if (h->cf_off && (h->n_bg_voxels > h->cf_off_bg + h->cf_off_bg / 4 + 1000 || h->n_bg_voxels < h->cf_off_bg))
    h->cf_off = false;
  vplan::PlanInputs in = plan_inputs(h, ws, ct, sw);
  in.lds_ccl_off = rerun_off_lds;
  in.n = n;
  in.no_update = no_update;
  in.submitted = submitted;
  in.dbg = dbg != nullptr;
  in.dbg_far_only = dbg && dbg[0].far_only;
  in.auto_raycast = call.flags & VOFOD_SCAN_AUTO_RAYCAST;
  const RefLattice ref_lattice = fill_ref_lattice(g);
  in.ref_lattice_on = ref_lattice.on != 0;
  in.layout_packed = true;
  for (uint32_t f = 0; f < n && in.layout_packed; f++)
  {
    const FrameArgs& a = ws.h_args[f];
    in.layout_packed = a.stride == 4 && (a.n & 3u) == 0 && a.n >= 4 && ((reinterpret_cast<uintptr_t>(a.x) | reinterpret_cast<uintptr_t>(a.y) | reinterpret_cast<uintptr_t>(a.z)) & 15u) == 0;
  }
  in.patchable = g.align && static_cast<float>(dp.voxel_map__thresholds__frontiers) <= thr_new;
  const vplan::ChainPlan& plan = ws.plan = vplan::plan_chain(in);
  if (trace_on())
    std::fprintf(stderr, "[vofod trace] n=%u plan: %s, %s, %s, %s, %s\n", n, name(plan.voxeliser), name(plan.clusterer), name(plan.closefar), name(plan.finalize), name(plan.tail));
  g.sparse_prefix = plan.bricks ? 1u : 0u;

  VCHK(launch_voxelize(h, ws, plan, g, n, static_cast<uint32_t>(npts)));
  if (dbg)
    HIPCHK(hipEventRecord(ev[1], h->stream));
  if (rt.staged)
    VCHK(enter_frame_stream(h, ws));

  UpdateParams up{};
  up.score_point = static_cast<float>(dp.voxel_map__scores__point);
  up.score_unknown = static_cast<float>(dp.voxel_map__scores__unknown);
  up.min_points = dp.classification__min_points;
  up.cand_max_extent = static_cast<float>(dp.classification__max_size * (1.0 + 1e-4) + 1e-3 * sp.voxel_size);
  up.no_update = no_update;
  if (plan.far_single)
    VCHK(cluster_far_single(h, ws, plan, g, ct, cpar, up, thr_new));
  else if (plan.frame())
    VCHK(launch_frame_kernel(h, ws, plan, g, n, ct, ref_lattice, up));
  else
    VCHK(launch_cluster(h, ws, plan, g, ct));
  if (dbg)
    HIPCHK(hipEventRecord(ev[2], h->stream));
  VCHK(closefar_and_finalize(h, ws, plan, g, cpar, up, dbg, ev));
  ws.bitmap_clean = plan.bitmap_clean_after;

  call.tail_stream_used = h->stream;
  if (plan.raycast_ahead)
    VCHK(raycast_ahead_of_tail(h, ws, call));
  if (plan.dtail)
    VCHK(launch_device_tail(h, ws, plan, rt, call));
  else
    VCHK(read_back_full(h, ws, g, n));
  if (dbg)
    HIPCHK(hipEventRecord(ev[4], h->stream));
  call.tr_launch = ms_since(call.t0);
  if (!submitted)
    return VOFOD_OK;

  h2d_guard.armed = false;
  if (host_copies)
    HIPCHK(hipEventSynchronize(ws.ev_h2d));
  HIPCHK(hipEventRecord(ws.ev_done, plan.dtail ? call.tail_stream_used : h->stream));
  ws.pending = true;
  ws.job_n = n;
  ws.job_g = g;
  if (call.tfs != ws.job_tfs.data())
    ws.job_tfs.assign(call.tfs, call.tfs + 12 * static_cast<size_t>(n));
  if (call.scans != ws.job_scans.data())
    ws.job_scans.assign(call.scans, call.scans + n);
  return VOFOD_OK;
}

}
```

vofod_amd/csrc/kernels_classify.h:

```cpp
#pragma once
#include <hip/hip_runtime.h>

#include "common.h"

namespace vc
{
using namespace vk;

constexpr int EX_MAX_R = 32;
constexpr int EX_SIDE = 2 * EX_MAX_R + 1;
constexpr uint32_t EX_CELLS = EX_SIDE * EX_SIDE * EX_SIDE;
constexpr uint32_t EX_WORDS = (EX_CELLS + 31) / 32;
constexpr uint32_t EX_MAX_JOBS = 1024;

struct ExploreJob
{
  uint32_t frame;
  uint32_t n_members;
  uint32_t member_off;
  int32_t R;
  int32_t box_lo[3], box_hi[3];
  uint32_t result_slot;
};

struct ExploreResult
{
  uint32_t floating;
  uint32_t overflow;
  double conf_sum;
};

struct ExploreParams
{
  float thr_unknown, thr_ground, frontier_value;
  double ray_score;
  int32_t no_update;
  uint32_t stack_cap;
};

__device__ __forceinline__ void wave_sync()
{
  __builtin_amdgcn_fence(__ATOMIC_RELEASE, "workgroup");
  __builtin_amdgcn_wave_barrier();
  __builtin_amdgcn_fence(__ATOMIC_ACQUIRE, "workgroup");
}

__device__ __forceinline__ uint32_t pack_rel(int dx, int dy, int dz) { return static_cast<uint32_t>((dx + 128) | ((dy + 128) << 8) | ((dz + 128) << 16)); }

__device__ __forceinline__ void explore_frame(const ExploreParams& ep, const MapGeom& mg, const ExploreJob* __restrict__ jobs, const uint32_t jb, const uint32_t je, const int* __restrict__ members,
                                              float* __restrict__ map, unsigned long long* __restrict__ overlay_all, uint32_t* __restrict__ stack_all, uint32_t* __restrict__ explored_all,
                                              uint32_t* __restrict__ touched_all, uint32_t* __restrict__ ovl_list_all, uint32_t* __restrict__ ovl_count_all, ExploreResult* __restrict__ results,
                                              uint32_t* __restrict__ visited_all, const uint32_t slot, uint8_t* s_float, uint8_t* s_walk)
{
  const int lane = threadIdx.x & 63;
  if (jb == je)
    return;
  const uint64_t ovl_words = (mg.n + 63) >> 6;
  unsigned long long* overlay = overlay_all + static_cast<uint64_t>(slot) * ovl_words;
  uint32_t* stack = stack_all + static_cast<uint64_t>(slot) * ep.stack_cap;
  uint32_t* explored = explored_all + static_cast<uint64_t>(slot) * ep.stack_cap;
  uint32_t* ovl_list = ovl_list_all + static_cast<uint64_t>(slot) * ep.stack_cap;
  uint32_t* touched = touched_all + static_cast<uint64_t>(slot) * ep.stack_cap;
  uint32_t* visited = visited_all + static_cast<uint64_t>(slot) * EX_WORDS;

  auto map_read = [&](uint64_t li) -> float {
    const float mv = map[li];
    if (!ep.no_update)
      return mv;
    const unsigned long long ow = __hip_atomic_load(&overlay[li >> 6], __ATOMIC_RELAXED, __HIP_MEMORY_SCOPE_AGENT);
    return ((ow >> (li & 63)) & 1ull) ? ep.frontier_value : mv;
  };

  for (uint32_t j = jb; j < je; j++)
  {
    const ExploreJob job = jobs[j];
    bool floating = true;
    uint32_t overflow = 0;
    const float max_voxel_dist = static_cast<float>(job.R);
    uint32_t m = 0;
    while (m < job.n_members && floating)
    {
      {
        const uint32_t mm = m + lane;
        int kind = 0;
        if (mm < job.n_members)
        {
          const int sx_ = members[3 * (job.member_off + mm)], sy_ = members[3 * (job.member_off + mm) + 1], sz_ = members[3 * (job.member_off + mm) + 2];
          if (sx_ <= 0 || sy_ <= 0 || sz_ <= 0 || sx_ >= mg.sx - 1 || sy_ >= mg.sy - 1 || sz_ >= mg.sz - 1)
            kind = 1;
          else
          {
            const float sv = map_read((static_cast<uint64_t>(sz_) * mg.sy + sy_) * mg.sx + sx_);
            kind = sv > ep.thr_ground ? 1 : (sv > ep.thr_unknown ? 2 : 0);
          }
        }
        const unsigned long long need = __ballot(kind != 0);
        if (!need)
        {
          m += 64;
          continue;
        }
        const int first = __ffsll(static_cast<long long>(need)) - 1;
        m += first;
        if (__shfl(kind, first) == 1)
        {
          floating = false;
          break;
        }
      }
      const int ox = members[3 * (job.member_off + m)], oy = members[3 * (job.member_off + m) + 1], oz = members[3 * (job.member_off + m) + 2];
      if (job.R - 1 >= 1 && job.R - 1 <= 31)
      {
        const int len = job.R - 1;
        float wv[3];
        bool win[3];
        const uint64_t li0 = (static_cast<uint64_t>(oz) * mg.sy + oy) * mg.sx + ox;
#pragma unroll
        for (int u = 0; u < 3; u++)
        {
          const int e = lane + 64 * u, q = e >> 5, d = (e & 31) + 1;
          const int ax = ox + (q == 0 ? d : q == 3 ? -d : 0), ay = oy + (q == 1 ? d : q == 4 ? -d : 0), az = oz + (q == 2 ? d : q == 5 ? -d : 0);
          win[u] = d <= len && ax >= 0 && ax <= mg.sx - 1 && ay >= 0 && ay <= mg.sy - 1 && az >= 0 && az <= mg.sz - 1;
          wv[u] = map_read(win[u] ? (static_cast<uint64_t>(az) * mg.sy + ay) * mg.sx + ax : li0);
        }
#pragma unroll
        for (int u = 0; u < 3; u++)
          s_walk[lane + 64 * u] = !win[u] ? 0 : (wv[u] > ep.thr_ground ? 2 : (wv[u] > ep.thr_unknown ? 1 : 0));
        wave_sync();
        bool walk_ok = false;
        if (lane < 6)
        {
          walk_ok = true;
          for (int d = 1; d <= len; d++)
          {
            const uint8_t st = s_walk[(lane << 5) + d - 1];
            if (st == 2)
              break;
            if (st == 0)
            {
              walk_ok = false;
              break;
            }
          }
        }
        const bool any_walk = __ballot(walk_ok) != 0ull;
        wave_sync();
        if (any_walk)
        {
          floating = false;
          break;
        }
      }
      uint32_t n_stack = 1, n_expl = 0, n_touched = 1;
      if (lane == 0)
      {
        stack[0] = pack_rel(0, 0, 0);
        const uint32_t c = (EX_MAX_R * EX_SIDE + EX_MAX_R) * EX_SIDE + EX_MAX_R;
        atomicOr(&visited[c >> 5], 1u << (c & 31));
        touched[0] = c;
      }
      wave_sync();
      bool connected = false;
      while (n_stack > 0 && !connected)
      {
        const uint32_t take = min(n_stack, 64u);
        const uint32_t base = n_stack - take;
        n_stack = base;
        bool have = static_cast<uint32_t>(lane) < take;
        int dx = 0, dy = 0, dz = 0;
        float val = 0.0f;
        if (have)
        {
          const uint32_t e = stack[base + lane];
          dx = static_cast<int>(e & 255u) - 128;
          dy = static_cast<int>((e >> 8) & 255u) - 128;
          dz = static_cast<int>((e >> 16) & 255u) - 128;
          val = map_read((static_cast<uint64_t>(oz + dz) * mg.sy + (oy + dy)) * mg.sx + (ox + dx));
        }
        const bool ground = have && val > ep.thr_ground;
        const bool unknown = have && !ground && val > ep.thr_unknown;
        const int md = abs(dx) + abs(dy) + abs(dz);
        const bool rim = unknown && static_cast<float>(md) == max_voxel_dist - 1.0f;
        if (__ballot(ground || rim))
        {
          connected = true;
          break;
        }
        const unsigned long long um = __ballot(unknown);
        if (unknown)
        {
          const uint32_t pos = n_expl + __popcll(um & ((1ull << lane) - 1ull));
          if (pos < ep.stack_cap)
            explored[pos] = pack_rel(dx, dy, dz);
        }
        n_expl += __popcll(um);
        uint32_t mine[6];
        int n_mine = 0;
        if (unknown)
        {
          const int nb[6][3] = {{1, 0, 0}, {0, 1, 0}, {0, 0, 1}, {-1, 0, 0}, {0, -1, 0}, {0, 0, -1}};
          uint32_t oldw[6], bitq[6];
          bool okq[6];
#pragma unroll
          for (int q = 0; q < 6; q++)
          {
            const int tx = dx + nb[q][0], ty = dy + nb[q][1], tz = dz + nb[q][2];
            const int ax = ox + tx, ay = oy + ty, az = oz + tz;
            const int tmd = abs(tx) + abs(ty) + abs(tz);
            okq[q] = !(ax < 0 || ax > mg.sx - 1 || ay < 0 || ay > mg.sy - 1 || az < 0 || az > mg.sz - 1) && static_cast<float>(tmd) <= max_voxel_dist;
            const uint32_t c = okq[q] ? ((tz + EX_MAX_R) * EX_SIDE + (ty + EX_MAX_R)) * EX_SIDE + (tx + EX_MAX_R) : 0u;
            bitq[q] = 1u << (c & 31);
            oldw[q] = okq[q] ? atomicOr(&visited[c >> 5], bitq[q]) : 0xffffffffu;
          }
#pragma unroll
          for (int q = 0; q < 6; q++)
            if (okq[q] && !(oldw[q] & bitq[q]))
              mine[n_mine++] = pack_rel(dx + nb[q][0], dy + nb[q][1], dz + nb[q][2]);
        }
        uint32_t incl = static_cast<uint32_t>(n_mine);
#pragma unroll
        for (int s = 1; s < 64; s <<= 1)
        {
          const uint32_t t = __shfl_up(incl, s);
          if (lane >= s)
            incl += t;
        }
        const uint32_t total = __shfl(incl, 63);
        uint32_t at = n_stack + incl - n_mine;
        uint32_t tat = n_touched + incl - n_mine;
        for (int q = 0; q < n_mine; q++, at++, tat++)
        {
          if (at < ep.stack_cap)
            stack[at] = mine[q];
          else
            overflow = 1;
          if (tat < ep.stack_cap)
          {
            const int tx = static_cast<int>(mine[q] & 255u) - 128, ty = static_cast<int>((mine[q] >> 8) & 255u) - 128, tz = static_cast<int>((mine[q] >> 16) & 255u) - 128;
            touched[tat] = ((tz + EX_MAX_R) * EX_SIDE + (ty + EX_MAX_R)) * EX_SIDE + (tx + EX_MAX_R);
          }
        }
        n_stack = min(n_stack + total, ep.stack_cap);
        n_touched += total;
        wave_sync();
      }
      wave_sync();
      if (n_touched <= ep.stack_cap)
      {
        for (uint32_t e = lane; e < n_touched; e += 64)
          __hip_atomic_store(&visited[touched[e] >> 5], 0u, __ATOMIC_RELAXED, __HIP_MEMORY_SCOPE_AGENT);
      }
      else
        for (uint32_t w = lane; w < EX_WORDS; w += 64)
          __hip_atomic_store(&visited[w], 0u, __ATOMIC_RELAXED, __HIP_MEMORY_SCOPE_AGENT);
      __threadfence_block();
      wave_sync();
      if (connected)
      {
        floating = false;
        break;
      }
      for (uint32_t e = lane; e < min(n_expl, ep.stack_cap); e += 64)
      {
        const uint32_t pk = explored[e];
        const int dx = static_cast<int>(pk & 255u) - 128, dy = static_cast<int>((pk >> 8) & 255u) - 128, dz = static_cast<int>((pk >> 16) & 255u) - 128;
        const uint64_t li = (static_cast<uint64_t>(oz + dz) * mg.sy + (oy + dy)) * mg.sx + (ox + dx);
        if (ep.no_update)
        {
          const unsigned long long bit = 1ull << (li & 63);
          const unsigned long long old = atomicOr(&overlay[li >> 6], bit);
          if (!(old & bit))
          {
            const uint32_t pos = atomicAdd(&ovl_count_all[slot], 1u);
            if (pos < ep.stack_cap)
              ovl_list[pos] = static_cast<uint32_t>(li >> 6);
          }
        }
        else
          map[li] = ep.frontier_value;
      }
      __threadfence_block();
      wave_sync();
      m++;
    }
    if (lane == 0)
    {
      s_float[j - jb] = floating ? 1 : 0;
      results[job.result_slot].floating = floating ? 1u : 0u;
      results[job.result_slot].overflow = overflow;
      results[job.result_slot].conf_sum = 0.0;
    }
  }
  __threadfence_block();
  wave_sync();

  for (uint32_t j = jb; j < je; j++)
  {
    const ExploreJob job = jobs[j];
    if (!s_float[j - jb])
      continue;
    const int nx = job.box_hi[0] - job.box_lo[0] + 1, ny = job.box_hi[1] - job.box_lo[1] + 1, nz = job.box_hi[2] - job.box_lo[2] + 1;
    const uint32_t cells = static_cast<uint32_t>(nx) * ny * nz;
    double acc = 0.0;
    for (uint32_t c = lane; c < cells; c += 64)
    {
      const int x = job.box_lo[0] + static_cast<int>(c % nx), y = job.box_lo[1] + static_cast<int>((c / nx) % ny), z = job.box_lo[2] + static_cast<int>(c / (nx * ny));
      bool is_member = false;
      for (uint32_t m = 0; m < job.n_members; m++)
      {
        const int* o = &members[3 * (job.member_off + m)];
        is_member |= (o[0] == x && o[1] == y && o[2] == z);
      }
      const float v = is_member ? static_cast<float>(ep.ray_score) : map_read((static_cast<uint64_t>(z) * mg.sy + y) * mg.sx + x);
      acc += 1.0 - static_cast<double>(v) / ep.ray_score;
    }
#pragma unroll
    for (int s = 32; s > 0; s >>= 1)
      acc += __shfl_xor(acc, s);
    if (lane == 0)
      results[job.result_slot].conf_sum = acc;
  }
  if (ep.no_update)
  {
    wave_sync();
    const uint32_t n = __hip_atomic_load(&ovl_count_all[slot], __ATOMIC_RELAXED, __HIP_MEMORY_SCOPE_AGENT);
    if (n <= ep.stack_cap)
      for (uint32_t e = lane; e < n; e += 64)
        overlay[ovl_list[e]] = 0ull;
    else
      for (uint64_t w = lane; w < ovl_words; w += 64)
        overlay[w] = 0ull;
    wave_sync();
    if (lane == 0)
      ovl_count_all[slot] = 0;
  }
}

__global__ __attribute__((amdgpu_waves_per_eu(8, 8))) __launch_bounds__(64) void k_explore(const ExploreParams ep, const MapGeom mg, const ExploreJob* __restrict__ jobs, const uint32_t* __restrict__ job_begin, const uint32_t* __restrict__ job_end,
                                                const int* __restrict__ members, float* __restrict__ map, unsigned long long* __restrict__ overlay_all,
                                                uint32_t* __restrict__ stack_all, uint32_t* __restrict__ explored_all, uint32_t* __restrict__ touched_all,
                                                uint32_t* __restrict__ ovl_list_all, uint32_t* __restrict__ ovl_count_all, ExploreResult* __restrict__ results, uint32_t* __restrict__ visited_all)
{
  __shared__ uint8_t s_float[EX_MAX_JOBS];
  __shared__ uint8_t s_walk[6 * 32];
  const uint32_t slot = blockIdx.x;
  explore_frame(ep, mg, jobs, job_begin[slot], job_end[slot], members, map, overlay_all, stack_all, explored_all, touched_all, ovl_list_all, ovl_count_all, results, visited_all, slot, s_float, s_walk);
}

}
```

vofod_amd/csrc/kernels_frame.h:

```cpp
#pragma once
#include <hip/hip_runtime.h>

#include "column_pose.h"
#include "kernels_brick_lds.h"
#include "kernels_slab.h"

namespace vk
{

constexpr int FR_THREADS = 1024;
#ifndef FR_WRITE_BACK_DEF
#define FR_WRITE_BACK_DEF 1
#endif
constexpr bool FR_WRITE_BACK = FR_WRITE_BACK_DEF != 0;
constexpr int FR_BW64 = LB_BITWORDS / 2;
#ifndef FR_WAVE_PRIO
#define FR_WAVE_PRIO 3
#endif
constexpr int FR_EREC = LB_MAX / 2;
constexpr int FR_CHUNKS = LB_MAX / 64;
constexpr int FR_MAX_NBZ = 64;
constexpr uint32_t FR_ROWS_MAX = 8192;
constexpr uint32_t FR_CODE_NONE = 0xffffffffu;
constexpr int FR_BB64 = FR_BW64 + 2 + FR_BW64 / 4;
constexpr uint32_t FR_CNT_CAP = FR_BB64 * 8;
#ifndef FR_VGPR_CAP
#define FR_VGPR_ATTR
#else
#define FR_VGPR_ATTR __attribute__((amdgpu_num_vgpr(FR_VGPR_CAP)))
#endif
#ifndef FR_REG_ROUNDS_DEF
#define FR_REG_ROUNDS_DEF 3
#endif
constexpr int FR_REG_ROUNDS = FR_REG_ROUNDS_DEF;
constexpr int CF_MAX = FR_THREADS;
#ifndef CF_G_DEF
#define CF_G_DEF 4
#endif
constexpr int CF_G = CF_G_DEF;
constexpr uint16_t FR_VBASE_NONE = 0xffffu;
constexpr uint32_t CF_LABEL_NONE = 0xffffffffu;
constexpr uint32_t FR_PROF_FRAMES = 4096;
constexpr size_t FR_PROF_WORDS = 2 * 32 * static_cast<size_t>(FR_PROF_FRAMES);

struct FrameScratch
{
  unsigned long long* rowT;
  uint32_t* rowQ;
  uint32_t* bmin;
  unsigned long long* bbsave;
  unsigned long long* nodeA;
  float4* frag;
  uint32_t keys_cap;
};

struct RefLattice
{
  float off[3];
  float eps;
  int32_t dims[3];
  int32_t nb[3];
  int32_t on;
};

constexpr int IN_PPT = 8;
constexpr uint32_t IN_ROUND = FR_THREADS * IN_PPT;
constexpr uint32_t IN_SEG_ALIGN = 16u * 64u * IN_PPT;

struct FrNodeLds
{
  unsigned long long word[LB_MAX];
  uint32_t xyz[LB_MAX];
  uint32_t x2[FR_EREC];
};
constexpr uint32_t IN_Q_UNITS = 64;
constexpr uint32_t IN_Q_PLANES = 3 * IN_PPT / 4;
constexpr uint32_t IN_Q_BYTES = IN_Q_UNITS * (IN_PPT * 12 + 2);
static_assert(IN_PPT % 4 == 0 && IN_Q_BYTES % 16 == 0 && IN_Q_BYTES * (FR_THREADS / 64) <= sizeof(FrNodeLds), "the input pass's unit queues live in the per-node arrays");

__device__ __forceinline__ float min3_raw(float a, float b, float c)
{
  float d;
  asm("v_min3_f32 %0, %1, %2, %3" : "=v"(d) : "v"(a), "v"(b), "v"(c));
  return d;
}
__device__ __forceinline__ float max3_raw(float a, float b, float c)
{
  float d;
  asm("v_max3_f32 %0, %1, %2, %3" : "=v"(d) : "v"(a), "v"(b), "v"(c));
  return d;
}
__device__ __forceinline__ float max3_abs(float a, float b, float c)
{
  float d;
  asm("v_max3_f32 %0, |%1|, |%2|, |%3|" : "=v"(d) : "v"(a), "v"(b), "v"(c));
  return d;
}
__device__ __forceinline__ float wave_fmin(float v)
{
  asm("s_nop 1\n\tv_min_f32_dpp %0, %0, %0 row_shr:1 row_mask:0xf bank_mask:0xf\n\ts_nop 1\n\t"
      "v_min_f32_dpp %0, %0, %0 row_shr:2 row_mask:0xf bank_mask:0xf\n\ts_nop 1\n\t"
      "v_min_f32_dpp %0, %0, %0 row_shr:4 row_mask:0xf bank_mask:0xf\n\ts_nop 1\n\t"
      "v_min_f32_dpp %0, %0, %0 row_shr:8 row_mask:0xf bank_mask:0xf\n\ts_nop 1\n\t"
      "v_min_f32_dpp %0, %0, %0 row_bcast:15 row_mask:0xa bank_mask:0xf\n\ts_nop 1\n\t"
      "v_min_f32_dpp %0, %0, %0 row_bcast:31 row_mask:0xc bank_mask:0xf\n\ts_nop 1"
      : "+v"(v));
  return __int_as_float(__builtin_amdgcn_readlane(__float_as_int(v), 63));
}
__device__ __forceinline__ float wave_fmax(float v)
{
  asm("s_nop 1\n\tv_max_f32_dpp %0, %0, %0 row_shr:1 row_mask:0xf bank_mask:0xf\n\ts_nop 1\n\t"
      "v_max_f32_dpp %0, %0, %0 row_shr:2 row_mask:0xf bank_mask:0xf\n\ts_nop 1\n\t"
      "v_max_f32_dpp %0, %0, %0 row_shr:4 row_mask:0xf bank_mask:0xf\n\ts_nop 1\n\t"
      "v_max_f32_dpp %0, %0, %0 row_shr:8 row_mask:0xf bank_mask:0xf\n\ts_nop 1\n\t"
      "v_max_f32_dpp %0, %0, %0 row_bcast:15 row_mask:0xa bank_mask:0xf\n\ts_nop 1\n\t"
      "v_max_f32_dpp %0, %0, %0 row_bcast:31 row_mask:0xc bank_mask:0xf\n\ts_nop 1"
      : "+v"(v));
  return __int_as_float(__builtin_amdgcn_readlane(__float_as_int(v), 63));
}

__device__ __forceinline__ void wave_bbox(float (&mn)[3], float (&mx)[3])
{
#define VOFOD_BBOX_STEP(ctl)                          \
  "v_min_f32_dpp %0, %0, %0 " ctl "\n\t"              \
  "v_min_f32_dpp %1, %1, %1 " ctl "\n\t"              \
  "v_min_f32_dpp %2, %2, %2 " ctl "\n\t"              \
  "v_max_f32_dpp %3, %3, %3 " ctl "\n\t"              \
  "v_max_f32_dpp %4, %4, %4 " ctl "\n\t"              \
  "v_max_f32_dpp %5, %5, %5 " ctl "\n\t"
  asm("s_nop 1\n\t" VOFOD_BBOX_STEP("row_shr:1 row_mask:0xf bank_mask:0xf") VOFOD_BBOX_STEP("row_shr:2 row_mask:0xf bank_mask:0xf")
          VOFOD_BBOX_STEP("row_shr:4 row_mask:0xf bank_mask:0xf") VOFOD_BBOX_STEP("row_shr:8 row_mask:0xf bank_mask:0xf")
              VOFOD_BBOX_STEP("row_bcast:15 row_mask:0xa bank_mask:0xf") VOFOD_BBOX_STEP("row_bcast:31 row_mask:0xc bank_mask:0xf") "s_nop 1"
      : "+v"(mn[0]), "+v"(mn[1]), "+v"(mn[2]), "+v"(mx[0]), "+v"(mx[1]), "+v"(mx[2]));
#undef VOFOD_BBOX_STEP
#pragma unroll
  for (int c = 0; c < 3; c++)
  {
    mn[c] = __int_as_float(__builtin_amdgcn_readlane(__float_as_int(mn[c]), 63));
    mx[c] = __int_as_float(__builtin_amdgcn_readlane(__float_as_int(mx[c]), 63));
  }
}

typedef float f32x2 __attribute__((ext_vector_type(2)));

__device__ __forceinline__ f32x2 pk_mul_s(float c, f32x2 v)
{
  f32x2 d;
  const unsigned long long c64 = __float_as_uint(c);
  asm("v_pk_mul_f32 %0, %1, %2 op_sel_hi:[0,1]" : "=v"(d) : "s"(c64), "v"(v));
  return d;
}
__device__ __forceinline__ f32x2 pk_add_s(float c, f32x2 v)
{
  f32x2 d;
  const unsigned long long c64 = __float_as_uint(c);
  asm("v_pk_add_f32 %0, %1, %2 op_sel_hi:[0,1]" : "=v"(d) : "s"(c64), "v"(v));
  return d;
}

__device__ __forceinline__ uint32_t fr_pack(uint32_t bx, uint32_t by, uint32_t bz) { return bx | (by << 9) | (bz << 18); }
__device__ __forceinline__ int fr_bx(uint32_t d) { return static_cast<int>(d & 511u); }
__device__ __forceinline__ int fr_by(uint32_t d) { return static_cast<int>((d >> 9) & 511u); }
__device__ __forceinline__ int fr_bz(uint32_t d) { return static_cast<int>((d >> 18) & 63u); }
__device__ __forceinline__ uint32_t fr_row(uint32_t d, int nby) { return ((d >> 18) & 63u) * static_cast<uint32_t>(nby) + ((d >> 9) & 511u); }

__device__ __forceinline__ uint32_t fr_node(const unsigned long long* bits64, const uint16_t* pre, uint32_t b)
{
  return pre[b >> 6] + __popcll(bits64[b >> 6] & ((1ull << (b & 63u)) - 1ull));
}

__device__ __forceinline__ unsigned long long fr_chan(unsigned long long W, int zz)
{
  uint32_t x = static_cast<uint32_t>(W >> (16 * zz)) & 0xffffu;
  x = x - ((x >> 1) & 0x5555u);
  x = (x & 0x3333u) + ((x >> 2) & 0x3333u);
  return static_cast<unsigned long long>(x & 0xfu) | (static_cast<unsigned long long>((x >> 4) & 0xfu) << 16) | (static_cast<unsigned long long>((x >> 8) & 0xfu) << 32) |
         (static_cast<unsigned long long>((x >> 12) & 0xfu) << 48);
}

__device__ __forceinline__ unsigned long long fr_excl16(unsigned long long x) { return (x << 16) + (x << 32) + (x << 48); }
__device__ __forceinline__ uint32_t fr_hsum16(unsigned long long x)
{
  return static_cast<uint32_t>(x & 0xffffu) + static_cast<uint32_t>((x >> 16) & 0xffffu) + static_cast<uint32_t>((x >> 32) & 0xffffu) + static_cast<uint32_t>(x >> 48);
}

__device__ __forceinline__ unsigned long long fr_shfl64(unsigned long long v, int src)
{
  const uint32_t lo = __shfl(static_cast<uint32_t>(v), src), hi = __shfl(static_cast<uint32_t>(v >> 32), src);
  return static_cast<unsigned long long>(lo) | (static_cast<unsigned long long>(hi) << 32);
}

template <int CTRL, int ROW_MASK>
__device__ __forceinline__ unsigned long long dpp_mov0_64(unsigned long long v)
{
  return static_cast<unsigned long long>(dpp_mov0<CTRL, ROW_MASK>(static_cast<uint32_t>(v))) | (static_cast<unsigned long long>(dpp_mov0<CTRL, ROW_MASK>(static_cast<uint32_t>(v >> 32))) << 32);
}

template <int CTRL, int ROW_MASK>
__device__ __forceinline__ void fr_segstep(unsigned long long v[4], uint32_t& f)
{
  unsigned long long t[4];
#pragma unroll
  for (int q = 0; q < 4; q++)
    t[q] = dpp_mov0_64<CTRL, ROW_MASK>(v[q]);
  const uint32_t ft = dpp_mov0<CTRL, ROW_MASK>(f);
  if (!f)
  {
#pragma unroll
    for (int q = 0; q < 4; q++)
      v[q] += t[q];
  }
  f |= ft;
}

__device__ __forceinline__ void fr_segscan(unsigned long long v[4], bool& head)
{
  uint32_t f = head ? 1u : 0u;
  fr_segstep<0x111, 0xf>(v, f);
  fr_segstep<0x112, 0xf>(v, f);
  fr_segstep<0x114, 0xf>(v, f);
  fr_segstep<0x118, 0xf>(v, f);
  fr_segstep<0x142, 0xa>(v, f);
  fr_segstep<0x143, 0xc>(v, f);
  head = f != 0u;
}

struct FrNodes
{
  unsigned long long W;
  unsigned long long P[4], A[4];
  uint32_t xyz, row;
  bool live, began_here, tail;
};

__device__ __forceinline__ FrNodes fr_load_nodes(const unsigned long long* s_word, const uint32_t* s_xyz, uint32_t i, uint32_t n, int nby, int lane, const unsigned long long (*s_cin)[4],
                                                 uint32_t chunk, bool with_carry)
{
  FrNodes o;
  o.live = i < n;
  o.W = o.live ? s_word[i] : 0ull;
  o.xyz = o.live ? s_xyz[i] : 0u;
  o.row = o.live ? fr_row(o.xyz, nby) : 0xffffffffu;
  uint32_t prev = __shfl_up(o.row, 1);
  if (lane == 0)
  {
    prev = 0xfffffffeu;
    if (o.live && i > 0)
    {
      prev = fr_row(s_xyz[i - 1], nby);
    }
  }
  bool head = o.row != prev;
  uint32_t next = __shfl_down(o.row, 1);
  if (lane == 63)
  {
    next = 0xfffffffeu;
    if (i + 1 < n)
    {
      next = fr_row(s_xyz[i + 1], nby);
    }
  }
  o.tail = o.live && next != o.row;
#pragma unroll
  for (int zz = 0; zz < 4; zz++)
    o.A[zz] = o.P[zz] = fr_chan(o.W, zz);
  fr_segscan(o.A, head);
  o.began_here = head;
  if (with_carry && !head)
  {
#pragma unroll
    for (int zz = 0; zz < 4; zz++)
      o.A[zz] += s_cin[chunk][zz];
  }
  return o;
}

template <int CFM, bool PACKED>
__global__ FR_VGPR_ATTR __launch_bounds__(FR_THREADS) void k_frame_lds(const GridParams g, const BrickParams bp, const LbTables* __restrict__ tab, FrameHdr* hdrs, SlabArrays sa, uint32_t pt_cap,
                                                         VoxelArrays va_all, uint32_t* __restrict__ labels_all, uint32_t lb_limit, uint32_t* __restrict__ scratch_all, FrameScratch fs,
                                                         const MapGeom mg, const unsigned long long* __restrict__ mapclose, const unsigned long long* __restrict__ mapbits,
                                                         const CloseRow* __restrict__ crows, int n_crows, const UpdateParams up, ClusterRec* __restrict__ table_all,
                                                         CandMember* __restrict__ cand_all, int write_tables, unsigned long long* __restrict__ prof, const RefLattice rl, const FrameArgs* __restrict__ args,
                                                         int close_first, int lean)
{
#pragma clang fp contract(off)
  __shared__ __attribute__((aligned(16))) unsigned long long s_bb[FR_BB64];
  __shared__ __attribute__((aligned(16))) FrNodeLds s_nodes;
  unsigned long long (&s_word)[LB_MAX] = s_nodes.word;
  uint32_t (&s_xyz)[LB_MAX] = s_nodes.xyz;
  uint32_t (&s_x2)[FR_EREC] = s_nodes.x2;
  __shared__ LbTables s_tab;
  __shared__ unsigned long long s_cin[FR_CHUNKS + 1][4];
  __shared__ uint32_t s_cflag[FR_CHUNKS + 1];
  __shared__ uint32_t s_wsum[FR_THREADS / 64];
  __shared__ uint32_t s_n, s_nh, s_nn, s_nf, s_no, s_ne;
  __shared__ uint32_t s_nhn;
  __shared__ uint16_t s_pf[CF_MAX];
  __shared__ __attribute__((aligned(16))) uint16_t s_pfpar[CF_MAX];
  __shared__ uint32_t s_taint[CF_MAX / 32], s_troot[CF_MAX / 32];
  __shared__ uint32_t s_npf, s_nc, s_no2, s_ncand;
  __shared__ __attribute__((aligned(16))) uint32_t s_cfd[32][4];
  __shared__ uint8_t s_cfl[2][32];
  __shared__ uint32_t s_cfn[2];
  __shared__ int s_red[FR_THREADS / 64][6];
  __shared__ uint32_t s_wcnt[FR_THREADS / 64];
  __shared__ uint32_t s_nfrag;
  __shared__ __attribute__((aligned(16))) uint32_t s_qc[FR_MAX_NBZ][4];
  __shared__ int s_lat[4];
  __shared__ float s_latf[3];
  __shared__ int s_shift[4];
  static_assert(sizeof(unsigned long long) * (FR_MAX_NBZ + 1 + FR_THREADS / 64) <= sizeof(uint16_t) * CF_MAX, "rank pass c borrows the union-find's storage");
  unsigned long long* s_gs = reinterpret_cast<unsigned long long*>(s_pfpar);
  unsigned long long* s_w4 = s_gs + FR_MAX_NBZ + 1;
  unsigned long long* s_bits64 = s_bb;
  uint16_t* s_pre = reinterpret_cast<uint16_t*>(s_bb + FR_BW64 + 2);
  uint32_t* s_cnt32 = reinterpret_cast<uint32_t*>(s_bb);
  uint32_t* s_bits = reinterpret_cast<uint32_t*>(s_bits64);
  uint16_t* s_vbase = reinterpret_cast<uint16_t*>(s_x2);
  uint16_t* s_par = reinterpret_cast<uint16_t*>(s_x2);
  __builtin_amdgcn_s_setprio(FR_WAVE_PRIO);
  const uint32_t FRAME = blockIdx.x;
  FrameHdr& h = hdrs[FRAME];
  __shared__ int s_mapk[4];
  __shared__ __attribute__((aligned(16))) uint32_t s_near[5][4];
  __shared__ uint32_t s_near_n;
  const VoxelArrays va = frame_voxels(va_all, FRAME, g.vox_cap);
  uint32_t* labels = labels_all + static_cast<size_t>(FRAME) * g.vox_cap;
  uint32_t* s_cmin = reinterpret_cast<uint32_t*>(s_word);
  const int tid = threadIdx.x, lane = tid & 63, wave = tid >> 6;
  const int nbx = rl.nb[0], nby = rl.nb[1], nbz = rl.nb[2];
#define FR_STAMP(i)     \
  if (prof && tid == 0) \
  prof[static_cast<size_t>(FRAME) * 32 + (i)] = wall_clock64()
  FR_STAMP(0);
  if (prof && tid == 0)
    prof[static_cast<size_t>(FRAME) * 32 + 21] = (static_cast<unsigned long long>(__builtin_amdgcn_s_getreg((31 << 11) | 20)) << 32) | static_cast<unsigned long long>(__builtin_amdgcn_s_getreg((31 << 11) | 4));
  for (int s = tid; s < FR_BW64 + 2; s += FR_THREADS)
    s_bits64[s] = 0ull;
  for (int s = tid; s < static_cast<int>(sizeof(LbTables) / 4); s += FR_THREADS)
    reinterpret_cast<uint32_t*>(&s_tab)[s] = reinterpret_cast<const uint32_t*>(tab)[s];
  if (tid == 0)
  {
    s_ne = 0;
    s_nh = 0;
    s_nhn = 0;
    s_nn = 0;
// ... 2233 lines not shown
```

vofod_amd/csrc/kernels_tail.h:

```cpp
#pragma once
#include <hip/hip_runtime.h>

#include "host_tail.h"
#include "kernels_classify.h"
#include "kernels_voxelize.h"

namespace vtd
{

#ifndef TAIL_WPB_DEF
#define TAIL_WPB_DEF 8
#endif
constexpr int TAIL_WPB = TAIL_WPB_DEF;
#if TAIL_WPB_DEF >= 16
#define TAIL_OCC_ATTR
#else
#define TAIL_OCC_ATTR __attribute__((amdgpu_waves_per_eu(5, 5)))
#endif
using namespace vk;

constexpr int TAIL_STAGE = 512;
constexpr int TP_THREADS = 256;
constexpr int TP_MAXM = TAIL_MAXM;
constexpr int TP_MAXC = TAIL_MAXC;
constexpr int TP_MAXD = 16;

using vt::TailParams;

struct TailCluster
{
  uint32_t root, n_members;
  float obb_center[3];
  int32_t job;
};

struct DetRaw
{
  uint32_t root, n_points;
  float center[3];
  uint32_t pad;
  double conf_sum;
};

struct FrameDets
{
  uint32_t n;
  uint32_t fallback;
  int32_t status;
  uint32_t n_jobs;
  DetRaw d[TP_MAXD];
};

enum : uint32_t { TAIL_FB_MEMBERS = 1u, TAIL_FB_CLUSTERS = 2u, TAIL_FB_RADIUS = 4u, TAIL_FB_DETS = 8u, TAIL_FB_EXPLORE = 16u };

__device__ __forceinline__ uint32_t rank_in_wave(bool flag, int lane, uint32_t& count)
{
  const unsigned long long m = __ballot(flag);
  count = __popcll(m);
  return __popcll(m & ((1ull << lane) - 1ull));
}

__device__ __forceinline__ void put_header(FrameDets& out, FrameDets* hout, uint32_t f, uint32_t n, uint32_t fb, int32_t status, uint32_t n_jobs)
{
  out.n = n;
  out.fallback = fb;
  out.status = status;
  out.n_jobs = n_jobs;
  if (hout)
  {
    hout[f].n = n;
    hout[f].fallback = fb;
    hout[f].status = status;
    hout[f].n_jobs = n_jobs;
  }
}

__device__ __forceinline__ void write_records(const TailCluster& tc, const vc::ExploreResult* __restrict__ results, int lane, FrameDets& out, FrameDets* hout, uint32_t f, uint32_t& n, uint32_t& fb)
{
  bool det = false, bad = false;
  double conf = 0.0;
  if (tc.job >= 0)
  {
    const vc::ExploreResult r = results[tc.job];
    det = r.floating != 0u;
    bad = r.overflow != 0u;
    conf = r.conf_sum;
  }
  const uint32_t pos = rank_in_wave(det, lane, n);
  const unsigned long long bm = __ballot(bad);
  if (det && pos < TP_MAXD)
  {
    DetRaw d;
    d.root = tc.root;
    d.n_points = tc.n_members;
    for (int q = 0; q < 3; q++)
      d.center[q] = tc.obb_center[q];
    d.pad = 0;
    d.conf_sum = conf;
    out.d[pos] = d;
    if (hout)
      hout[f].d[pos] = d;
  }
  fb = (n > TP_MAXD ? TAIL_FB_DETS : 0u) | (bm ? TAIL_FB_EXPLORE : 0u);
}

template <class Get>
__device__ __forceinline__ bool gate_cluster(uint32_t f, uint32_t m_begin, uint32_t m_count, Get get, const float* tf, const MapGeom& mg, const TailParams& tp, int* __restrict__ members_out, TailCluster& tc,
                                             vc::ExploreJob& job, uint32_t& fallback)
{
  const int s3[3] = {mg.sx, mg.sy, mg.sz};
  const vt::Gates gt = vt::classify_gates(m_count, get, tf, tp, mg.off, mg.vs_inv, s3);
  for (int q = 0; q < 3; q++)
    tc.obb_center[q] = gt.obb_center[q];
  if (!gt.explore)
    return false;
  job.frame = f;
  job.n_members = m_count;
  job.member_off = f * TP_MAXM + m_begin;
  job.R = gt.R;
  if (job.R > vc::EX_MAX_R || job.R < 0)
    fallback |= TAIL_FB_RADIUS;
  for (int q = 0; q < 3; q++)
  {
    job.box_lo[q] = gt.box_lo[q];
    job.box_hi[q] = gt.box_hi[q];
  }
  for (uint32_t i = 0; i < m_count; i++)
  {
    float p[3];
    get(i, p);
    int* o = members_out + 3 * static_cast<size_t>(job.member_off + i);
    for (int q = 0; q < 3; q++)
      o[q] = vt::map_cell(p[q], mg.off[q], mg.vs_inv);
  }
  return true;
}

__global__ __launch_bounds__(TP_THREADS) void k_tail_prep(const GridParams g, const FrameHdr* __restrict__ hdrs, const FrameArgs* __restrict__ args, const ClusterRec* __restrict__ table_all,
                                                         const CandMember* __restrict__ cand_all, VoxelArrays va_all, const MapGeom mg, const TailParams tp, vc::ExploreJob* __restrict__ jobs,
                                                         uint32_t* __restrict__ job_begin, uint32_t* __restrict__ job_end, int* __restrict__ members_out, TailCluster* __restrict__ tailc,
                                                         FrameDets* __restrict__ dets)
{
  __shared__ unsigned long long s_key[TP_MAXM];
  __shared__ ClusterRec s_rec[TP_MAXC];
  __shared__ uint32_t s_ord[TP_MAXC];
  __shared__ uint32_t s_nc;
  const uint32_t f = blockIdx.x;
  const FrameHdr h = hdrs[f];
  const int tid = threadIdx.x;
  FrameDets& out = dets[f];
  uint32_t fallback = 0;
  if (tid == 0)
  {
    s_nc = 0;
    job_begin[f] = f * TP_MAXC;
    job_end[f] = f * TP_MAXC;
  }
  __syncthreads();
  const uint32_t n_cand = h.status == VOFOD_OK ? h.n_cand : 0u;
  const uint32_t C = h.status == VOFOD_OK ? h.C : 0u;
  if (n_cand > TP_MAXM)
    fallback |= TAIL_FB_MEMBERS;
  const ClusterRec* table = table_all + static_cast<size_t>(f) * g.vox_cap;
  for (uint32_t c = tid; c < C; c += TP_THREADS)
  {
    const ClusterRec r = table[c];
    if (r.cand && !r.close)
    {
      const uint32_t pos = atomicAdd(&s_nc, 1u);
      if (pos < TP_MAXC)
        s_rec[pos] = r;
    }
  }
  uint32_t np2 = 1;
  while (np2 < n_cand && np2 < TP_MAXM)
    np2 <<= 1;
  const CandMember* cands = cand_all + static_cast<size_t>(f) * g.vox_cap;
  if (!(fallback & TAIL_FB_MEMBERS))
    for (uint32_t i = tid; i < np2; i += TP_THREADS)
    {
      unsigned long long k = ~0ull;
      if (i < n_cand)
      {
        const CandMember cm = cands[i];
        k = (static_cast<unsigned long long>(cm.root) << 32) | cm.v;
      }
      s_key[i] = k;
    }
  __syncthreads();
  if (!(fallback & TAIL_FB_MEMBERS) && n_cand > 1)
    for (uint32_t k = 2; k <= np2; k <<= 1)
      for (uint32_t j = k >> 1; j > 0; j >>= 1)
      {
        for (uint32_t i = tid; i < np2; i += TP_THREADS)
        {
          const uint32_t l = i ^ j;
          if (l > i)
          {
            const unsigned long long a = s_key[i], b = s_key[l];
            const bool up = (i & k) == 0;
            if ((a > b) == up)
            {
              s_key[i] = b;
              s_key[l] = a;
            }
          }
        }
        __syncthreads();
      }
  const uint32_t nc_all = s_nc;
  if (nc_all > TP_MAXC)
    fallback |= TAIL_FB_CLUSTERS;
  const uint32_t nc = fallback ? 0u : nc_all;
  if (tid < static_cast<int>(nc))
  {
    const ClusterRec me = s_rec[tid];
    uint32_t rank = 0;
    for (uint32_t j = 0; j < nc; j++)
    {
      const ClusterRec o = s_rec[j];
      rank += (o.size > me.size || (o.size == me.size && o.root < me.root)) ? 1u : 0u;
    }
    s_ord[rank] = tid;
  }
  __syncthreads();
  if (tid >= 64)
    return;
  const int lane = tid;
  bool live = lane < static_cast<int>(nc);
  const VoxelArrays va = frame_voxels(va_all, f, g.vox_cap);
  const FrameArgs& a = args[f];
  bool wants_job = false;
  vc::ExploreJob job{};
  TailCluster tc{};
  tc.job = -1;
  uint32_t m_begin = 0, m_count = 0;
  if (live)
  {
    const ClusterRec rec = s_rec[s_ord[lane]];
    tc.root = rec.root;
    uint32_t lo = 0, hi = n_cand;
    const unsigned long long want = static_cast<unsigned long long>(rec.root) << 32;
    while (lo < hi)
    {
      const uint32_t mid = (lo + hi) >> 1;
      if (s_key[mid] < want)
        lo = mid + 1;
      else
        hi = mid;
    }
    m_begin = lo;
    while (m_begin + m_count < n_cand && static_cast<uint32_t>(s_key[m_begin + m_count] >> 32) == rec.root)
      m_count++;
    tc.n_members = m_count;
    auto get = [&](size_t i, float p[3]) {
      const float4 q = va.pts[static_cast<uint32_t>(s_key[m_begin + i])];
      p[0] = q.x;
      p[1] = q.y;
      p[2] = q.z;
    };
    wants_job = gate_cluster(f, m_begin, m_count, get, a.tf, mg, tp, members_out, tc, job, fallback);
  }
  uint32_t n_jobs;
  const uint32_t slot = f * TP_MAXC + rank_in_wave(wants_job, lane, n_jobs);
  if (wants_job)
  {
    job.result_slot = slot;
    jobs[slot] = job;
    tc.job = static_cast<int32_t>(slot);
  }
  uint32_t fb_all = fallback;
#pragma unroll
  for (int s = 32; s > 0; s >>= 1)
    fb_all |= __shfl_xor(fb_all, s);
  if (live)
    tailc[f * TP_MAXC + lane] = tc;
  if (lane == 0)
  {
    put_header(out, nullptr, f, 0u, fb_all, h.status, fb_all ? 0u : n_jobs);
    if (!fb_all)
      job_end[f] = f * TP_MAXC + n_jobs;
  }
  if (!live && lane < TP_MAXC)
  {
    TailCluster e{};
    e.job = -1;
    tailc[f * TP_MAXC + lane] = e;
  }
}

__global__ TAIL_OCC_ATTR __launch_bounds__(64 * TAIL_WPB) void k_tail_far(const GridParams g, const FrameHdr* __restrict__ hdrs, const FrameArgs* __restrict__ args, const ClusterRec* __restrict__ table_all,
                                                const CandMember* __restrict__ cand_all, VoxelArrays va_all, const MapGeom mg, const TailParams tp, const vc::ExploreParams ep, vc::ExploreJob* __restrict__ jobs,
                                                int* __restrict__ members_out, float* __restrict__ map, unsigned long long* __restrict__ overlay_all, uint32_t* __restrict__ stack_all,
                                                uint32_t* __restrict__ explored_all, uint32_t* __restrict__ touched_all, uint32_t* __restrict__ ovl_list_all, uint32_t* __restrict__ ovl_count_all,
                                                vc::ExploreResult* __restrict__ results, uint32_t* __restrict__ visited_all, FrameDets* __restrict__ dets, FrameDets* __restrict__ hout,
                                                TailCluster* __restrict__ tailc, unsigned long long* __restrict__ prof)
{
  __shared__ uint8_t s_float_all[TAIL_WPB][TP_MAXC];
  __shared__ uint8_t s_walk_all[TAIL_WPB][6 * 32];
  __shared__ float s_pts_all[TAIL_WPB][TAIL_STAGE][3];
  const uint32_t f = blockIdx.x * TAIL_WPB + (threadIdx.x >> 6);
  if (f >= g.n_frames)
    return;
  uint8_t* s_float = s_float_all[threadIdx.x >> 6];
  uint8_t* s_walk = s_walk_all[threadIdx.x >> 6];
  const FrameHdr h = hdrs[f];
  const int lane = threadIdx.x & 63;
  const unsigned long long tp0 = prof ? wall_clock64() : 0ull;
  unsigned long long tp1 = 0ull, tp2 = 0ull;
  FrameDets& out = dets[f];
  uint32_t fallback = 0;
  const bool ok = h.status == VOFOD_OK;
  const uint32_t n_cand = ok ? h.n_cand : 0u;
  const uint32_t nc_all = ok ? h.n_cand_clusters : 0u;
  if (n_cand > static_cast<uint32_t>(TP_MAXM))
    fallback |= TAIL_FB_MEMBERS;
  if (nc_all > static_cast<uint32_t>(TP_MAXC))
    fallback |= TAIL_FB_CLUSTERS;
  const uint32_t nc = fallback ? 0u : nc_all;
  const bool live = lane < static_cast<int>(nc);
  const ClusterRec* table = table_all + static_cast<size_t>(f) * g.vox_cap;
  const CandMember* cands = cand_all + static_cast<size_t>(f) * g.vox_cap;
  const VoxelArrays va = frame_voxels(va_all, f, g.vox_cap);
  const FrameArgs& a = args[f];
  ClusterRec rec{};
  if (live)
    rec = table[lane];
  uint32_t m_count = live ? rec.size : 0u, m_begin = 0;
  {
    uint32_t incl = m_count;
#pragma unroll
    for (int s = 1; s < 64; s <<= 1)
    {
      const uint32_t t = __shfl_up(incl, s);
      if (lane >= s)
        incl += t;
    }
    m_begin = incl - m_count;
  }
  float (*s_pts)[3] = s_pts_all[threadIdx.x >> 6];
  {
    const uint32_t total = min(static_cast<uint32_t>(__shfl(m_begin + m_count, 63)), static_cast<uint32_t>(TAIL_STAGE));
    for (uint32_t i = lane; i < total; i += 64)
    {
      const float4 q = va.pts[cands[i].v];
      s_pts[i][0] = q.x;
      s_pts[i][1] = q.y;
      s_pts[i][2] = q.z;
    }
    vc::wave_sync();
  }
  bool wants_job = false;
  vc::ExploreJob job{};
  TailCluster tc{};
  tc.job = -1;
  if (live)
  {
    tc.root = rec.root;
    tc.n_members = m_count;
    auto get = [&](size_t i, float p[3]) {
      const uint32_t k = m_begin + static_cast<uint32_t>(i);
      if (k < static_cast<uint32_t>(TAIL_STAGE))
      {
        p[0] = s_pts[k][0];
        p[1] = s_pts[k][1];
        p[2] = s_pts[k][2];
        return;
      }
      const float4 q = va.pts[cands[k].v];
      p[0] = q.x;
      p[1] = q.y;
      p[2] = q.z;
    };
    wants_job = gate_cluster(f, m_begin, m_count, get, a.tf, mg, tp, members_out, tc, job, fallback);
  }
  uint32_t n_jobs;
  const uint32_t jb = f * TP_MAXC;
  const uint32_t slot = jb + rank_in_wave(wants_job, lane, n_jobs);
  if (wants_job)
  {
    job.result_slot = slot;
    jobs[slot] = job;
    tc.job = static_cast<int32_t>(slot);
  }
  if (tailc)
  {
    if (!live)
    {
      tc = TailCluster{};
      tc.job = -1;
    }
    tailc[f * TP_MAXC + lane] = tc;
  }
  uint32_t fb_all = fallback;
#pragma unroll
  for (int s = 32; s > 0; s >>= 1)
    fb_all |= __shfl_xor(fb_all, s);
  if (fb_all)
  {
    if (lane == 0)
      put_header(out, hout, f, 0u, fb_all, h.status, 0u);
    return;
  }
  __threadfence_block();
  vc::wave_sync();
  if (prof)
    tp1 = wall_clock64();
  vc::explore_frame(ep, mg, jobs, jb, jb + n_jobs, members_out, map, overlay_all, stack_all, explored_all, touched_all, ovl_list_all, ovl_count_all, results, visited_all, f, s_float, s_walk);
  __threadfence_block();
  vc::wave_sync();
  if (prof)
    tp2 = wall_clock64();
  uint32_t n, fb;
  write_records(tc, results, lane, out, hout, f, n, fb);
  if (lane == 0)
  {
    put_header(out, hout, f, n, fb, h.status, n_jobs);
    if (prof)
    {
      const unsigned long long te = wall_clock64();
      auto d20 = [&](unsigned long long t) { return (t - tp0) > 0xfffffull ? 0xfffffull : (t - tp0); };
      prof[static_cast<size_t>(f) * 32 + 22] = tp0;
      prof[static_cast<size_t>(f) * 32 + 23] = d20(tp1) | (d20(tp2) << 20) | (d20(te) << 40) | (static_cast<unsigned long long>(n_jobs > 15u ? 15u : n_jobs) << 60);
    }
  }
}

__global__ __launch_bounds__(64) void k_tail_finish(const TailCluster* __restrict__ tailc, const vc::ExploreResult* __restrict__ results, FrameDets* __restrict__ dets, FrameDets* __restrict__ hout)
{
  const uint32_t f = blockIdx.x;
  const int lane = threadIdx.x;
  FrameDets& out = dets[f];
  const uint32_t fb_in = out.fallback;
  if (fb_in)
  {
    if (lane == 0)
      put_header(out, hout, f, 0u, fb_in, out.status, out.n_jobs);
    return;
  }
  const TailCluster tc = tailc[f * TP_MAXC + lane];
  uint32_t n, fb;
  write_records(tc, results, lane, out, hout, f, n, fb);
  if (lane == 0)
    put_header(out, hout, f, n, fb, out.status, out.n_jobs);
}

}
```

vofod_amd/csrc/vofod_hip.hip:

```cpp
#include <hip/hip_runtime.h>

#include <atomic>
#include <chrono>
#include <cmath>
#include <cstdio>
#include <cstring>
#include <fstream>
#include <map>
#include <memory>
#include <mutex>
#include <string>
#include <type_traits>
#include <vector>

#include "chain_plan.h"
#include "common.h"
#include "device_mem.h"
#include "host_tail.h"
#include "thread_pool.h"
#include "kernels_brick.h"
#include "kernels_brick_lds.h"
#include "kernels_classify.h"
#include "kernels_frame.h"
#include "kernels_cluster.h"
// ... 94 lines not shown
  {
    static const bool v = std::getenv("VOFOD_CALLTRACE") != nullptr;
    return v;
  }
  SlowCall(const char* w, int l) : what(w), line(l)
  {
    if (on())
      t0 = std::chrono::steady_clock::now();
  }
  ~SlowCall()
  {
    if (!on())
      return;
    const double ms = std::chrono::duration<double, std::milli>(std::chrono::steady_clock::now() - t0).count();
    if (ms > 0.3)
      std::fprintf(stderr, "[vofod calltrace] %.2f ms in %s (line %d)\n", ms, what, line);
  }
};

#define HIPCHK(expr)                                                                                         \
  do                                                                                                         \
  {                                                                                                          \
    SlowCall sc_(#expr, __LINE__);                                                                           \
    const hipError_t e_ = (expr);                                                                            \
    if (e_ != hipSuccess)                                                                                    \
    {                                                                                                        \
      h->err = std::string(#expr) + ": " + hipGetErrorString(e_) + " (" + __FILE__ + ":" + std::to_string(__LINE__) + ")"; \
      return VOFOD_ERR_DEVICE;                                                                               \
    }                                                                                                        \
  } while (0)

#define HIP_TRY(expr)                                      \
  do                                                       \
  {                                                        \
    if (const hipError_t e_ = (expr); e_ != hipSuccess)    \
      return e_;                                           \
  } while (0)

#define VCHK(expr)                             \
  do                                           \
  {                                            \
    if (const int r_ = (expr); r_ != VOFOD_OK) \
      return r_;                               \
  } while (0)

struct Prof
{
  bool on = false;
  struct Rec
  {
    const char* name;
    hipEvent_t a, b;
  };
  std::vector<Rec> recs;
  std::vector<hipEvent_t> pool;
  std::vector<DevEvent> owned;
  hipEvent_t get()
  {
    if (!pool.empty())
    {
      hipEvent_t e = pool.back();
      pool.pop_back();
      return e;
    }
    owned.emplace_back();
    (void)owned.back().create(hipEventCreate);
    return owned.back();
  }
};

#define KLAUNCH_AS(h, label, kern, grid, block, ...)                        \
  do                                                                         \
  {                                                                          \
    if ((h)->prof.on)                                                        \
    {                                                                        \
      Prof::Rec r_{label, (h)->prof.get(), (h)->prof.get()};                 \
      (void)hipEventRecord(r_.a, (h)->stream);                               \
      hipLaunchKernelGGL(kern, grid, block, 0, (h)->stream, __VA_ARGS__);    \
      (void)hipEventRecord(r_.b, (h)->stream);                               \
      (h)->prof.recs.push_back(r_);                                          \
    }                                                                        \
    else                                                                     \
    {                                                                        \
      SlowCall sc_(label, __LINE__);                                         \
      hipLaunchKernelGGL(kern, grid, block, 0, (h)->stream, __VA_ARGS__);    \
    }                                                                        \
  } while (0)
#define KLAUNCH(h, kern, grid, block, ...) KLAUNCH_AS(h, #kern, kern, grid, block, __VA_ARGS__)

template <class T>
hipError_t alloc_view(DevBuf<T>& own, T*& v, size_t n)
{
  const hipError_t e = own.alloc(n);
  v = own;
  return e;
}

struct Workspace
{
  uint32_t F = 0, pt_cap = 0, vox_cap = 0, words_cap = 0, nblk_cap = 0, bricks_cap = 0;
  BrickArrays ba{};
  VoxelArrays va{};
  SlabArrays sa{};
  FrameScratch fs{};
  DevBuf<unsigned long long> ba_bricks, fs_rowT, fs_nodeA, fs_bbsave;
  DevBuf<uint32_t> ba_bparent, ba_bmin, ba_bcmin, ba_blist, va_key, va_parent, va_csize, va_cclose, va_bb, sa_extras, sa_counts, fs_rowQ, fs_bmin;
  DevBuf<float4> va_pts, fs_frag;
  DevBuf<int32_t> va_cbox;
  DevBuf<unsigned long long> d_bconn;
  DevBuf<FrameArgs> d_args;
  DevBuf<FrameHdr> d_hdrs;
  DevBuf<unsigned long long> d_bitmaps;
  DevBuf<uint32_t> d_wprefix;
  DevBuf<uint32_t> d_blocksums;
  DevBuf<uint32_t> d_labels;
  DevBuf<ClusterRec> d_table;
  DevBuf<CandMember> d_cand;
  DevBuf<uint32_t> d_keys;
  DevBuf<float> d_stage;
  DevBuf<char> d_stage_aos;
  size_t aos_pitch = 0;
  DevBuf<vrd::RangeJob> d_rjobs;
  PinBuf<vrd::RangeJob> h_rjobs;
  uint32_t n_mjobs = 0, n_rjobs = 0;
  DevBuf<float> d_poses;
  DevBuf<vpd::PointJob> d_pjobs;
  PinBuf<vpd::PointJob> h_pjobs;
  uint32_t n_pjobs = 0;
  const float* first_poses = nullptr;
  DevBuf<PackedFrame> d_packed;
  PinBuf<PackedFrame> h_packed;
  bool prof_deferred = false;
  uint32_t prof_slot0 = 0;
  vplan::ChainPlan plan;
  DevBuf<vtd::TailCluster> d_tailc;
  DevBuf<vtd::FrameDets> d_dets;
  PinBuf<vtd::FrameDets> h_dets;
  vtd::FrameDets* h_dets_dev = nullptr;
  DevBuf<uint32_t> d_job_be;
  struct PinnedArgs
  {
    PinBuf<FrameArgs> buf;
    FrameArgs& operator[](size_t i) { return buf.p[i]; }
    const FrameArgs& operator[](size_t i) const { return buf.p[i]; }
    FrameArgs* data() { return buf; }
    hipError_t assign(size_t n, const FrameArgs& v)
    {
      HIP_TRY(buf.alloc(n));
      std::fill_n(buf.p, n, v);
      return hipSuccess;
    }
  } h_args;
  std::vector<vofod_scan> job_scans;
  bool bitmap_clean = false;
  vofod_dyn_params job_dp{};
  bool rerun = false;
  DevBuf<CandMemberX> d_members_big;
  struct DetRef
  {
    uint32_t id, frame, root, n_points;
  };
  std::vector<DetRef> det_refs;
  bool det_valid = false;
  bool det_submitted = false;
  uint32_t det_vox_cap = 0;
  GridParams det_g{};
  std::vector<vpx::PixSize> det_px_sizes;
  void det_begin(bool submitted, const GridParams& g)
  {
    det_refs.clear();
    det_px_sizes.clear();
    det_valid = false;
    det_submitted = submitted;
    det_vox_cap = g.vox_cap;
    det_g = g;
  }
  DevBuf<vdp::DetDesc> d_detdesc;
  DevBuf<vdp::DetBox> d_detbox;
  DevBuf<float4> d_detpts;
  DevBuf<uint32_t> d_detidx;
  DevBuf<vpx::PixDesc> d_pxdesc;
  DevBuf<vpx::PixSize> d_pxsize;
  DevBuf<vpx::PixFound> d_pxfound;
  DevBuf<uint32_t> d_pxkey, d_pxrank, d_pxidx, d_pxmember;
  DevBuf<float> d_pxxyz;
  bool pending = false;
  uint32_t job_n = 0;
  GridParams job_g{};
  std::vector<float> job_tfs;
  DevEvent ev_done;
  DevEvent ev_packed;
  DevEvent ev_key;
  DevEvent ev_h2d;

  hipError_t ensure(uint32_t F_, uint32_t pt_cap_, uint32_t vox_cap_, uint32_t words_cap_, uint32_t bricks_cap_ = 0)
  {
    if (F_ <= F && pt_cap_ <= pt_cap && vox_cap_ <= vox_cap && words_cap_ <= words_cap && bricks_cap_ <= bricks_cap)
      return hipSuccess;
    F_ = std::max(F_, F);
    pt_cap_ = std::max(pt_cap_, pt_cap);
    vox_cap_ = std::max(vox_cap_, vox_cap);
    words_cap_ = std::max(words_cap_, words_cap);
    bricks_cap_ = std::max(bricks_cap_, bricks_cap);
    *this = Workspace();
    const hipError_t e = allocate(F_, pt_cap_, vox_cap_, words_cap_, bricks_cap_);
    if (e != hipSuccess)
      *this = Workspace();
    return e;
  }

private:
  hipError_t allocate(const uint32_t F_, const uint32_t pt_cap_, const uint32_t vox_cap_, const uint32_t words_cap_, const uint32_t bricks_cap_)
  {
    const uint32_t nblk_cap_ = (words_cap_ + SCAN_WPB - 1) / SCAN_WPB + 1;
    const size_t FV = static_cast<size_t>(F_) * vox_cap_;
    const size_t FB = F_ * std::max<size_t>(bricks_cap_, 1);
    const size_t FW = F_ * (static_cast<size_t>(words_cap_) + 2);
    HIP_TRY(alloc_view(ba_bricks, ba.bricks, FB));
    HIP_TRY(hipMemset(ba.bricks, 0, sizeof(unsigned long long) * FB));
    HIP_TRY(d_bconn.alloc(FB));
    HIP_TRY(alloc_view(ba_bparent, ba.bparent, FB));
    HIP_TRY(alloc_view(ba_bmin, ba.bmin, FB));
    HIP_TRY(alloc_view(ba_bcmin, ba.bcmin, FB));
    HIP_TRY(hipMemset(ba.bmin, 0xff, sizeof(uint32_t) * FB));
    HIP_TRY(hipMemset(ba.bcmin, 0xff, sizeof(uint32_t) * FB));
    HIP_TRY(alloc_view(ba_blist, ba.blist, FV));
    HIP_TRY(d_args.alloc(F_));
    HIP_TRY(d_hdrs.alloc(F_));
    HIP_TRY(d_bitmaps.alloc(FW));
    HIP_TRY(d_wprefix.alloc(FW));
    HIP_TRY(d_blocksums.alloc(static_cast<size_t>(F_) * nblk_cap_));
    HIP_TRY(alloc_view(va_pts, va.pts, FV));
    HIP_TRY(alloc_view(va_key, va.key, FV));
    HIP_TRY(alloc_view(va_parent, va.parent, FV));
    HIP_TRY(alloc_view(va_csize, va.csize, FV));
    HIP_TRY(alloc_view(va_cbox, va.cbox, 6 * FV));
    HIP_TRY(alloc_view(va_cclose, va.cclose, FV));
    HIP_TRY(alloc_view(va_bb, va.bb, FV));
    HIP_TRY(d_labels.alloc(FV));
    HIP_TRY(d_table.alloc(FV));
    HIP_TRY(d_cand.alloc(FV));
    fs.keys_cap = (pt_cap_ + IN_SEG_ALIGN - 1u) / IN_SEG_ALIGN * IN_SEG_ALIGN;
    HIP_TRY(d_keys.alloc(static_cast<size_t>(F_) * fs.keys_cap));
    HIP_TRY(alloc_view(sa_extras, sa.extras, static_cast<size_t>(F_) * pt_cap_));
    HIP_TRY(alloc_view(sa_counts, sa.counts, 2 * static_cast<size_t>(F_)));
    sa.keys = d_keys;
    HIP_TRY(d_stage.alloc(5 * static_cast<size_t>(F_) * pt_cap_));
    HIP_TRY(d_rjobs.alloc(F_));
    HIP_TRY(h_rjobs.alloc(F_));
    HIP_TRY(d_pjobs.alloc(F_));
    HIP_TRY(h_pjobs.alloc(F_));
    HIP_TRY(d_packed.alloc(F_));
    HIP_TRY(d_tailc.alloc(vtd::TP_MAXC * static_cast<size_t>(F_)));
    HIP_TRY(d_dets.alloc(F_));
    HIP_TRY(d_job_be.alloc(2 * static_cast<size_t>(F_)));
    HIP_TRY(d_members_big.alloc(vox_cap_));
    HIP_TRY(alloc_view(fs_rowT, fs.rowT, 4 * FR_ROWS_MAX * static_cast<size_t>(F_)));
    HIP_TRY(alloc_view(fs_rowQ, fs.rowQ, 4 * FR_ROWS_MAX * static_cast<size_t>(F_)));
    HIP_TRY(alloc_view(fs_bmin, fs.bmin, LB_MAX * static_cast<size_t>(F_)));
    HIP_TRY(alloc_view(fs_nodeA, fs.nodeA, 4 * LB_MAX * static_cast<size_t>(F_)));
    HIP_TRY(alloc_view(fs_bbsave, fs.bbsave, FR_BB64 * static_cast<size_t>(F_)));
    HIP_TRY(alloc_view(fs_frag, fs.frag, static_cast<size_t>(F_) * std::max<uint32_t>(pt_cap_, 1)));
    HIP_TRY(h_packed.alloc(F_));
    HIP_TRY(h_dets.alloc(F_, hipHostMallocMapped | hipHostMallocCoherent));
    std::memset(h_dets, 0, sizeof(vtd::FrameDets) * F_);
    HIP_TRY(hipHostGetDevicePointer(reinterpret_cast<void**>(&h_dets_dev), h_dets, 0));
    HIP_TRY(h_args.assign(F_, FrameArgs{}));
    HIP_TRY(ev_done.create(hipEventCreateWithFlags, hipEventDisableTiming));
    HIP_TRY(ev_packed.create(hipEventCreateWithFlags, hipEventDisableTiming));
    HIP_TRY(ev_h2d.create(hipEventCreateWithFlags, hipEventDisableTiming));
    HIP_TRY(ev_key.create(hipEventCreateWithFlags, hipEventDisableTiming));
    HIP_TRY(hipDeviceSynchronize());
    F = F_;
    pt_cap = pt_cap_;
    vox_cap = vox_cap_;
    words_cap = words_cap_;
    bricks_cap = bricks_cap_;
    nblk_cap = nblk_cap_;
    return hipSuccess;
  }
};

struct ExploreBufs
{
  DevBuf<unsigned long long> d_overlay;
  DevBuf<uint32_t> d_stack, d_explored, d_touched, d_ovl_list, d_ovl_count, d_job_begin;
  DevBuf<uint32_t> d_visited;
  DevBuf<vc::ExploreJob> d_jobs;
  DevBuf<vc::ExploreResult> d_results;
  DevBuf<int> d_members;
  uint32_t F() const { return static_cast<uint32_t>(d_visited.n / vc::EX_WORDS); }
};

struct HostCluster
{
  ClusterRec rec;
  int cclass = VOFOD_CLASS_NONE;
  vt::Gates gates;
};

struct vofod_handle
{
  DevBuf<unsigned long long> d_prof_slab, d_prof_ccl;
  bool cf_off = false;
  uint64_t cf_off_bg = 0;
  bool bgcount_stale = false;
  bool lds_ccl_off = false;
  std::mutex mtx;
  vofod_static_params sp{};
  vofod_dyn_params dp{};
  std::string err;
  Prof prof;
  int device = 0;
  hipStream_t stream = nullptr;
  DevStream stream_tail;
  DevStream stream_key;
  static constexpr int MAX_FRAME_STREAMS = 8;
  DevStream stream_frames[MAX_FRAME_STREAMS];
  int n_frame_streams = 0;
  hipStream_t stream_frame = nullptr;
  int frame_toggle = 0;
  static constexpr int MAX_INFLIGHT = 8;
  DevStream chain_stream[MAX_INFLIGHT];
  Workspace wsx[MAX_INFLIGHT - 1];
  Workspace* slot(int t) { return t == 0 ? &ws : &wsx[t - 1]; }
  ExploreBufs explore_slot[MAX_INFLIGHT];

  float exclude_center[3], oparea_center[3];
  uint64_t background_min_sufficient_pts = 0;

  MapGeom mg{};
  vt::Geom hg{};
  DevBuf<float> d_map, d_flags, d_ray;
  DevBuf<float> d_shift_spare;
  vws::Store world;
  vwy::State wsync;
  DevBuf<unsigned long long> d_mapbits;
  DevBuf<unsigned long long> d_mapclose;
  uint64_t mapbits_gen = 0, mapclose_gen = ~0ull;
  float mapclose_dist = -1.0f;
  DevBuf<unsigned long long> d_counter;
  DevBuf<unsigned long long> d_bgcount;
  PinBuf<unsigned long long> h_bgcount;
  bool bgcount_fresh = false;
  DevEvent ev_stagger;
  bool ev_stagger_set = false;
  DevEvent ev_explore;
  DevEvent ev_bgcount;
  PinBuf<unsigned long long> h_counter;
  bool mapbits_valid = false;
  float mapbits_thr = 0;
  uint64_t n_bg_voxels = 0;

  DevBuf<float> d_lut_dirs, d_lut_offs;
  DevBuf<uint8_t> d_mask;
  DevBuf<uint32_t> d_col_shift;
  bool raycast_motion = false;
  bool point_motion = false;
  bool raycast_exact = false;
  bool ray_pass_exact = false;
  int32_t ray_log2_units = -1;
  uint32_t ray_qmax = 0;

  Workspace ws, aux, sepws;
  ExploreBufs explore;
  std::unique_ptr<vt::Pool> pool;
  struct ClusterTables
  {
    bool valid = false;
    float leaf[3] = {0, 0, 0}, tol = 0, cmax = 0;
    ClusterParams cp{};
    int n_rows = 0;
    DevBuf<StencilRow> d_rows;
    bool brick_ok = false;
    BrickParams bp{};
    DevBuf<BrickOff> d_boffs;
    DevBuf<unsigned long long> d_sure, d_amb;
    DevBuf<int8_t> d_pair;
    DevBuf<LbTables> d_lbtab;
    bool lds_ok = false;
  } ctab[2];
  int ctab_next = 0;
  struct CloseTables
  {
    bool valid = false;
    float max_dist = 0;
    int n_rows = 0;
  } closetab;
  bool ray_dirty = false;
  DevBuf<StencilRow> d_rows;
  DevBuf<CloseRow> d_crows;
  DevBuf<float> d_boxstage;
  DevBuf<uint64_t> d_idxstage;

  bool background_pts_sufficient = false, sure_background_sufficient = false;
  int detection_its = 0;
  uint32_t last_detection_id = 0;
  bool raycast_pending = false;
  int raycast_start_its = 0;
  vr::SepState sep;
  struct SepBufs
  {
    DevBuf<unsigned long long> d_tbits;
    DevBuf<uint32_t> d_tpop, d_tprefix, d_bsum, d_sure, d_sure_pre, d_vcnt, d_first, d_nsure, d_small;
    DevBuf<float> d_px, d_py, d_pz, d_pi;
    DevBuf<int> d_offsets;
    PinBuf<uint32_t> h_small;
  } sep_own;
  MapSyncState msync;
  bool sep_pending = false;
  int sep_start_its = 0;
};

#include "frame_prof.h"

namespace
{


struct EdgeClassifier
{
  double leaf[3], r2, delta;
  float r2f;
  EdgeClassifier(const float leaf_[3], float tol, float cmax)
  {
    r2f = tol * tol;
    r2 = r2f;
    for (int a = 0; a < 3; a++)
      leaf[a] = leaf_[a];
    delta = 2.0 * ulp32(cmax);
  }
  int operator()(int di, int dj, int dk) const
  {
    const double ex = std::abs(di) * leaf[0], ey = std::abs(dj) * leaf[1], ez = std::abs(dk) * leaf[2];
    const double D = ex * ex + ey * ey + ez * ez;
    const double eps = 2.0 * delta + 3.0 * ulp32(static_cast<float>(std::max({ex, ey, ez, 1e-30})));
    const double E = 2.0 * eps * (ex + ey + ez) + 3.0 * eps * eps + 8.0 * D * 1.2e-7;
    if (D + E < r2)
      return 1;
    if (D - E >= r2)
      return 0;
    return 2;
  }
};

int build_cluster_stencil(const float leaf[3], float tol, float cmax, std::vector<StencilRow>& rows, ClusterParams& cp)
{
  rows.clear();
  int R[3];
  for (int a = 0; a < 3; a++)
  {
    R[a] = static_cast<int>(std::ceil(static_cast<double>(tol) / leaf[a])) + 1;
    if (R[a] > MAX_R)
      return VOFOD_ERR_INVALID_ARG;
  }
  const EdgeClassifier classify(leaf, tol, cmax);
  cp.row_gap = -1;
  for (int dk = 0; dk <= R[2]; dk++)
    for (int dj = (dk == 0 ? 0 : -R[1]); dj <= R[1]; dj++)
    {
      StencilRow row{};
      row.dj = static_cast<int16_t>(dj);
      row.dk = static_cast<int16_t>(dk);
      row.r_sure = -1;
      row.r_max = -1;
      row.amb = 0;
      bool sure_run = true;
      for (int di = 0; di <= R[0]; di++)
      {
        const int c = classify(di, dj, dk);
        if (c == 1 && sure_run)
          row.r_sure = static_cast<int16_t>(di);
        else
          sure_run = false;
        if (c == 1 && !sure_run)
          row.amb |= 1u << di;
        if (c == 2)
          row.amb |= 1u << di;
        if (c != 0)
          row.r_max = static_cast<int16_t>(di);
      }
      if (row.r_max < 0)
        continue;
      if (dj == 0 && dk == 0)
      {
        if (row.r_max < 1)
          continue;
        cp.row_gap = std::max<int>(row.r_sure, 0);
      }
      rows.push_back(row);
    }
  if (rows.size() > MAX_STENCIL_ROWS)
    return VOFOD_ERR_INVALID_ARG;
  cp.n_rows = static_cast<int>(rows.size());
  cp.r2 = classify.r2f;
  if (cp.row_gap < 0)
    cp.row_gap = 0;
  return VOFOD_OK;
}

bool build_brick_tables(const float leaf[3], float tol, float cmax, std::vector<BrickOff>& offs, std::vector<unsigned long long>& sure, std::vector<unsigned long long>& amb)
{
  offs.clear();
  sure.clear();
  amb.clear();
  const EdgeClassifier classify(leaf, tol, cmax);
  if (classify(3, 3, 3) != 1)
    return false;
  int Rb[3];
  for (int a = 0; a < 3; a++)
  {
    const int r_max = static_cast<int>(std::ceil(static_cast<double>(tol) / leaf[a])) + 1;
    Rb[a] = (r_max + 3 + 3) / 4;
  }
  for (int bz = 0; bz <= Rb[2]; bz++)
    for (int by = (bz == 0 ? 0 : -Rb[1]); by <= Rb[1]; by++)
      for (int bx = ((bz == 0 && by == 0) ? 1 : -Rb[0]); bx <= Rb[0]; bx++)
      {
        unsigned long long ms[64], ma[64];
        bool any = false, any_amb = false;
        for (int p = 0; p < 64; p++)
        {
          ms[p] = ma[p] = 0;
          const int px = p & 3, py = (p >> 2) & 3, pz = p >> 4;
          for (int q = 0; q < 64; q++)
          {
            const int qx = q & 3, qy = (q >> 2) & 3, qz = q >> 4;
            const int c = classify(4 * bx + qx - px, 4 * by + qy - py, 4 * bz + qz - pz);
            if (c == 1)
              ms[p] |= 1ull << q;
            else if (c == 2)
              ma[p] |= 1ull << q;
          }
          any |= (ms[p] | ma[p]) != 0;
          any_amb |= ma[p] != 0;
        }
        if (!any)
          continue;
        BrickOff bo{};
        bo.dx = static_cast<int8_t>(bx);
        bo.dy = static_cast<int8_t>(by);
        bo.dz = static_cast<int8_t>(bz);
        bo.has_amb = static_cast<uint8_t>(any_amb);
        for (int p = 0; p < 64; p++)
        {
          if (ms[p] | ma[p])
            bo.ua |= 1ull << p;
          bo.ub |= ms[p] | ma[p];
        }
        offs.push_back(bo);
        sure.insert(sure.end(), ms, ms + 64);
        amb.insert(amb.end(), ma, ma + 64);
      }
  return true;
}

bool build_lds_tables(const EdgeClassifier& classify, const std::vector<BrickOff>& offs, const std::vector<unsigned long long>& sure, const std::vector<unsigned long long>& amb,
                      LbTables& t)
{
  std::memset(&t, 0, sizeof(t));
  for (int c = LB_RV + 1; c <= 4 * 4 + 3; c++)
    if (classify(c, 0, 0) != 0 || classify(0, c, 0) != 0 || classify(0, 0, c) != 0)
      return false;
  for (int dz = -LB_RV; dz <= LB_RV; dz++)
    for (int dy = -LB_RV; dy <= LB_RV; dy++)
      for (int dx = -LB_RV; dx <= LB_RV; dx++)
      {
        const int c = classify(dx, dy, dz);
        if (c == 1)
          t.ball_sure[dz + LB_RV][dy + LB_RV] |= static_cast<uint16_t>(1u << (dx + LB_RV));
        else if (c == 2)
          t.ball_amb[dz + LB_RV][dy + LB_RV] |= static_cast<uint16_t>(1u << (dx + LB_RV));
      }
  if (offs.empty() || offs.size() > LB_MAX_OFF)
    return false;
  int R = 0;
  for (const auto& o : offs)
    R = std::max(R, std::abs(static_cast<int>(o.dx)));
  if (2 * R + 1 > LB_WIN)
    return false;
  t.R = R;
  for (size_t o = 0; o < offs.size(); o++)
  {
    int row = -1;
    for (int r = 0; r < t.n_rows; r++)
      if (t.rows[r].dy == offs[o].dy && t.rows[r].dz == offs[o].dz)
        row = r;
    if (row < 0)
    {
      if (t.n_rows == LB_MAX_ROWS)
        return false;
      row = t.n_rows++;
      t.rows[row].dy = offs[o].dy;
      t.rows[row].dz = offs[o].dz;
      for (auto& x : t.rows[row].o)
        x = -1;
    }
    if (std::abs(static_cast<int>(offs[o].dx)) <= 1 && std::abs(static_cast<int>(offs[o].dy)) <= 1 && std::abs(static_cast<int>(offs[o].dz)) <= 1)
      t.near_mask |= 1ull << o;
    if (std::abs(static_cast<int>(offs[o].dx)) + std::abs(static_cast<int>(offs[o].dy)) + std::abs(static_cast<int>(offs[o].dz)) == 1)
      t.axis_mask |= 1ull << o;
    const int s = offs[o].dx + R;
    t.rows[row].valid |= static_cast<uint8_t>(1u << s);
    t.rows[row].o[s] = static_cast<int8_t>(o);
    auto oct = [](int p) { return ((p & 3) >> 1) | ((((p >> 2) & 3) >> 1) << 1) | (((p >> 4) >> 1) << 2); };
    unsigned long long all = ~0ull, any = 0ull;
// ... 686 lines not shown
```

Baseline: 1.209 million frames/s.

## Move explore flood-fill visited set and stack into an LDS hash table

Adds a per-wave LDS open-addressing hash table (2048 slots plus a 256-entry stack) that serves as the flood-fill visited set and work stack in explore_frame. Small fills stay on-chip and fall back to the global bitmap path when they overflow. The same LDS area also holds a membership bitmap for the box-scoring loop, replacing a per-cell linear scan over members. To make room, k_tail_far reuses its point-staging LDS through a union and its occupancy hint drops from 5 to 4 waves per EU. This trades lower occupancy and possible redone fills on overflow for fewer global atomics and less global memory traffic. Optional fill counters are added for profiling.

```diff
diff --git a/vofod_amd/csrc/driver_aux.h b/vofod_amd/csrc/driver_aux.h
--- a/vofod_amd/csrc/driver_aux.h
+++ b/vofod_amd/csrc/driver_aux.h
@@ -872,6 +872,12 @@
   }
   h->prof.recs.clear();
   h->prof.on = on != 0;
+  if (on && std::getenv("VOFOD_FILL_COUNTS"))
+  {
+    if (!h->d_fill_counts)
+      HIPCHK(h->d_fill_counts.alloc(vc::EXC_N));
+    HIPCHK(hipMemset(h->d_fill_counts, 0, sizeof(unsigned long long) * vc::EXC_N));
+  }
   return VOFOD_OK;
 }
 
@@ -912,6 +918,21 @@
     calls[n] = acc[nm].second;
     n++;
   }
+  if (h->d_fill_counts && std::getenv("VOFOD_FILL_COUNTS"))
+  {
+    static const char* const cname[vc::EXC_N] = {"fills.started", "fills.fast", "fills.rounds", "fills.max_visited", "fills.max_stack", "fills.redone", "fills.lds", "fills.global"};
+    unsigned long long c[vc::EXC_N] = {};
+    (void)hipDeviceSynchronize();
+    if (hipMemcpy(c, h->d_fill_counts, sizeof(c), hipMemcpyDeviceToHost) == hipSuccess)
+      for (int i = 0; i < vc::EXC_N && n < cap; i++, n++)
+      {
+        std::memset(names + 64 * n, 0, 64);
+        std::strncpy(names + 64 * n, cname[i], 63);
+        ms[n] = 0.0;
+        calls[n] = c[i];
+      }
+    (void)hipMemset(h->d_fill_counts, 0, sizeof(c));
+  }
   return n;
 }
 
diff --git a/vofod_amd/csrc/explore_lds.h b/vofod_amd/csrc/explore_lds.h
--- /dev/null
+++ b/vofod_amd/csrc/explore_lds.h
@@ -0,0 +1,70 @@
+#pragma once
+#include <cstdint>
+
+#if defined(__HIPCC__) || defined(__CUDACC__)
+#define EXL_HD __host__ __device__
+#else
+#define EXL_HD
+#endif
+
+namespace vxl
+{
+
+constexpr uint32_t EXL_EMPTY = 0xffffffffu;
+constexpr uint32_t EXL_SLOTS = 2048;
+constexpr uint32_t EXL_LOAD_CAP = 1024;
+constexpr uint32_t EXL_STACK_CAP = 256;
+constexpr uint32_t EXL_WORDS = EXL_SLOTS + EXL_STACK_CAP;
+constexpr uint32_t EXL_ROUND_MAX = 64 * 6;
+static_assert(EXL_LOAD_CAP + EXL_ROUND_MAX <= EXL_SLOTS, "a round's inserts must fit the table");
+static_assert(EXL_SLOTS % 4 == 0, "the table is cleared four words at a time");
+
+enum Insert : int
+{
+  EXL_NEW = 0,
+  EXL_PRESENT = 1,
+  EXL_FULL = 2
+};
+
+EXL_HD inline uint32_t exl_home(uint32_t key, uint32_t slots) { return static_cast<uint32_t>((static_cast<uint64_t>(key * 0x9e3779b1u) * slots) >> 32); }
+EXL_HD inline uint32_t exl_next(uint32_t s, uint32_t slots) { return s + 1u == slots ? 0u : s + 1u; }
+
+template <class Cas>
+EXL_HD inline int exl_insert_from(uint32_t* table, uint32_t slots, uint32_t key, uint32_t s, uint32_t tries, Cas cas)
+{
+  for (uint32_t i = 0; i < tries; i++, s = exl_next(s, slots))
+  {
+    const uint32_t old = cas(&table[s], EXL_EMPTY, key);
+    if (old == EXL_EMPTY)
+      return EXL_NEW;
+    if (old == key)
+      return EXL_PRESENT;
+  }
+  return EXL_FULL;
+}
+template <class Cas>
+EXL_HD inline int exl_insert(uint32_t* table, uint32_t slots, uint32_t key, Cas cas)
+{
+  return exl_insert_from(table, slots, key, exl_home(key, slots), slots, cas);
+}
+template <class Cas>
+EXL_HD inline int exl_insert_rest(uint32_t* table, uint32_t slots, uint32_t key, uint32_t old, Cas cas)
+{
+  if (old == EXL_EMPTY)
+    return EXL_NEW;
+  if (old == key)
+    return EXL_PRESENT;
+  return exl_insert_from(table, slots, key, exl_next(exl_home(key, slots), slots), slots - 1u, cas);
+}
+
+EXL_HD inline bool exl_visited_fits(uint32_t n_visited, uint32_t load_cap = EXL_LOAD_CAP) { return n_visited <= load_cap; }
+EXL_HD inline bool exl_stack_fits(uint32_t n_stack, uint32_t pushes, uint32_t stack_cap = EXL_STACK_CAP) { return n_stack + pushes <= stack_cap; }
+EXL_HD inline uint32_t exl_pop(uint32_t& n_stack, uint32_t& base)
+{
+  const uint32_t take = n_stack < 64u ? n_stack : 64u;
+  base = n_stack - take;
+  n_stack = base;
+  return take;
+}
+
+}
diff --git a/vofod_amd/csrc/explore_lds_check.cpp b/vofod_amd/csrc/explore_lds_check.cpp
--- /dev/null
+++ b/vofod_amd/csrc/explore_lds_check.cpp
@@ -0,0 +1,193 @@
+#include <cstdio>
+#include <cstdlib>
+#include <cstring>
+#include <string>
+#include <vector>
+
+#include "explore_lds.h"
+
+using namespace vxl;
+
+static uint32_t plain_cas(uint32_t* p, uint32_t expected, uint32_t desired)
+{
+  const uint32_t old = *p;
+  if (old == expected)
+    *p = desired;
+  return old;
+}
+
+static uint32_t pack(int dx, int dy, int dz) { return static_cast<uint32_t>((dx + 128) | ((dy + 128) << 8) | ((dz + 128) << 16)); }
+
+static const char* word(int r) { return r == EXL_NEW ? "new" : r == EXL_PRESENT ? "present" : "full"; }
+
+static std::vector<uint32_t> keys_at(uint32_t home, uint32_t slots, size_t n)
+{
+  std::vector<uint32_t> out;
+  for (int z = -32; z <= 32 && out.size() < n; z++)
+    for (int y = -32; y <= 32 && out.size() < n; y++)
+      for (int x = -32; x <= 32 && out.size() < n; x++)
+        if (exl_home(pack(x, y, z), slots) == home)
+          out.push_back(pack(x, y, z));
+  return out;
+}
+
+static void print_slots(const std::vector<uint32_t>& t)
+{
+  std::printf(" used=");
+  bool first = true;
+  for (size_t i = 0; i < t.size(); i++)
+    if (t[i] != EXL_EMPTY)
+    {
+      std::printf("%s%zu", first ? "" : ",", i);
+      first = false;
+    }
+}
+
+static void ball(int r, bool flat)
+{
+  std::vector<uint32_t> tab(EXL_SLOTS, EXL_EMPTY), stk(EXL_STACK_CAP, 0u);
+  uint32_t n_stack = 1, n_vis = 1, rounds = 0, max_stack = 1, explored = 0;
+  stk[0] = pack(0, 0, 0);
+  tab[exl_home(pack(0, 0, 0), EXL_SLOTS)] = pack(0, 0, 0);
+  const char* why = "none";
+  while (n_stack > 0)
+  {
+    uint32_t base;
+    const uint32_t take = exl_pop(n_stack, base);
+    rounds++;
+    std::vector<uint32_t> pushes;
+    bool full = false;
+    for (uint32_t lane = 0; lane < take; lane++)
+    {
+      const uint32_t e = stk[base + lane];
+      const int dx = static_cast<int>(e & 255u) - 128, dy = static_cast<int>((e >> 8) & 255u) - 128, dz = static_cast<int>((e >> 16) & 255u) - 128;
+      if (std::abs(dx) + std::abs(dy) + std::abs(dz) > r || (flat && dz != 0))
+        continue;
+      explored++;
+      const int nb[6][3] = {{1, 0, 0}, {0, 1, 0}, {0, 0, 1}, {-1, 0, 0}, {0, -1, 0}, {0, 0, -1}};
+      for (int q = 0; q < 6; q++)
+      {
+        const uint32_t key = pack(dx + nb[q][0], dy + nb[q][1], dz + nb[q][2]);
+        const int res = exl_insert(tab.data(), EXL_SLOTS, key, plain_cas);
+        if (res == EXL_NEW)
+          pushes.push_back(key);
+        full |= res == EXL_FULL;
+      }
+    }
+    n_vis += static_cast<uint32_t>(pushes.size());
+    if (full || !exl_visited_fits(n_vis) || !exl_stack_fits(n_stack, static_cast<uint32_t>(pushes.size())))
+    {
+      why = full ? "table" : !exl_visited_fits(n_vis) ? "visited" : "stack";
+      break;
+    }
+    for (uint32_t k : pushes)
+      stk[n_stack++] = k;
+    max_stack = n_stack > max_stack ? n_stack : max_stack;
+  }
+  std::printf("overflow=%s visited=%u explored=%u rounds=%u max_stack=%u\n", why, n_vis, explored, rounds, max_stack);
+}
+
+int main(int argc, char** argv)
+{
+  const std::string c = argc > 1 ? argv[1] : "";
+  const int n = argc > 2 ? std::atoi(argv[2]) : 0;
+  if (c == "constants")
+    std::printf("slots=%u load_cap=%u stack_cap=%u words=%u empty=%u round_max=%u\n", EXL_SLOTS, EXL_LOAD_CAP, EXL_STACK_CAP, EXL_WORDS, EXL_EMPTY, EXL_ROUND_MAX);
+  else if (c == "full")
+  {
+    std::vector<uint32_t> t(16, EXL_EMPTY);
+    int news = 0;
+    for (int i = 0; i < 16; i++)
+      news += exl_insert(t.data(), 16, pack(i - 8, 3 * i - 20, 5), plain_cas) == EXL_NEW;
+    std::printf("new=%d seventeenth=%s again=%s", news, word(exl_insert(t.data(), 16, pack(20, 20, 20), plain_cas)), word(exl_insert(t.data(), 16, pack(7 - 8, 21 - 20, 5), plain_cas)));
+    print_slots(t);
+    std::printf("\n");
+  }
+  else if (c == "collide")
+  {
+    std::vector<uint32_t> t(16, EXL_EMPTY);
+    const std::vector<uint32_t> k = keys_at(5, 16, 8);
+    int news = 0, present = 0;
+    for (uint32_t key : k)
+      news += exl_insert(t.data(), 16, key, plain_cas) == EXL_NEW;
+    for (uint32_t key : k)
+      present += exl_insert(t.data(), 16, key, plain_cas) == EXL_PRESENT;
+    bool in_order = k.size() == 8;
+    for (size_t i = 0; i < k.size(); i++)
+      in_order &= t[5 + i] == k[i];
+    std::printf("keys=%zu new=%d present=%d in_order=%d", k.size(), news, present, in_order ? 1 : 0);
+    print_slots(t);
+    std::printf("\n");
+  }
+  else if (c == "twice")
+  {
+    std::vector<uint32_t> t(EXL_SLOTS, EXL_EMPTY);
+    const int a = exl_insert(t.data(), EXL_SLOTS, pack(1, -2, 3), plain_cas), b = exl_insert(t.data(), EXL_SLOTS, pack(1, -2, 3), plain_cas);
+    size_t used = 0;
+    for (uint32_t v : t)
+      used += v != EXL_EMPTY;
+    std::printf("first=%s second=%s used_slots=%zu\n", word(a), word(b), used);
+  }
+  else if (c == "wrap")
+  {
+    std::vector<uint32_t> t(16, EXL_EMPTY);
+    const std::vector<uint32_t> k = keys_at(15, 16, 3);
+    int news = 0;
+    for (uint32_t key : k)
+      news += exl_insert(t.data(), 16, key, plain_cas) == EXL_NEW;
+    std::printf("keys=%zu new=%d last=%d zero=%d one=%d again=%s", k.size(), news, t[15] == k[0], t[0] == k[1], t[1] == k[2], word(exl_insert(t.data(), 16, k[2], plain_cas)));
+    print_slots(t);
+    std::printf("\n");
+  }
+  else if (c == "clear")
+  {
+    std::vector<uint32_t> t(EXL_SLOTS, EXL_EMPTY);
+    int news = 0;
+    for (uint32_t i = 0; i < EXL_LOAD_CAP; i++)
+      news += exl_insert(t.data(), EXL_SLOTS, pack(static_cast<int>(i % 32) - 16, static_cast<int>(i / 32) - 8, 0), plain_cas) == EXL_NEW;
+    std::fill(t.begin(), t.end(), EXL_EMPTY);
+    const int a = exl_insert(t.data(), EXL_SLOTS, pack(-16, -8, 0), plain_cas), b = exl_insert(t.data(), EXL_SLOTS, pack(-16, -8, 0), plain_cas);
+    size_t used = 0;
+    for (uint32_t v : t)
+      used += v != EXL_EMPTY;
+    std::printf("first_use_new=%d after_clear=%s then=%s used_slots=%zu\n", news, word(a), word(b), used);
+  }
+  else if (c == "twostep")
+  {
+    std::vector<uint32_t> t1(64, EXL_EMPTY), t2(64, EXL_EMPTY);
+    int same = 1, news = 0;
+    for (int i = 0; i < 48; i++)
+    {
+      const int k = i % 20;
+      const uint32_t key = pack(k % 7 - 3, (k * 5) % 11 - 5, k % 3);
+      const int a = exl_insert(t1.data(), 64, key, plain_cas);
+      const int b = exl_insert_rest(t2.data(), 64, key, plain_cas(&t2[exl_home(key, 64)], EXL_EMPTY, key), plain_cas);
+      same &= a == b;
+      news += a == EXL_NEW;
+    }
+    std::printf("same_answers=%d same_table=%d new=%d\n", same, t1 == t2 ? 1 : 0, news);
+  }
+  else if (c == "capacity")
+  {
+    uint32_t ns[6] = {0, 1, 63, 64, 65, EXL_STACK_CAP};
+    std::printf("visited_at_cap=%d visited_past_cap=%d stack_at_cap=%d stack_past_cap=%d stack_full_no_push=%d", exl_visited_fits(EXL_LOAD_CAP), exl_visited_fits(EXL_LOAD_CAP + 1),
+                exl_stack_fits(EXL_STACK_CAP - 6, 6), exl_stack_fits(EXL_STACK_CAP - 6, 7), exl_stack_fits(EXL_STACK_CAP, 0));
+    for (uint32_t v : ns)
+    {
+      uint32_t n_stack = v, base = 99;
+      const uint32_t take = exl_pop(n_stack, base);
+      std::printf(" pop%u=%u/%u/%u", v, take, base, n_stack);
+    }
+    std::printf("\n");
+  }
+  else if (c == "ball")
+    ball(n, false);
+  else if (c == "disc")
+    ball(n, true);
+  else
+  {
+    std::fprintf(stderr, "usage: explore_lds_check constants|full|collide|twice|wrap|clear|twostep|capacity|ball <r>|disc <r>\n");
+    return 2;
+  }
+  return 0;
+}
diff --git a/vofod_amd/csrc/frame_prof.h b/vofod_amd/csrc/frame_prof.h
--- a/vofod_amd/csrc/frame_prof.h
+++ b/vofod_amd/csrc/frame_prof.h
@@ -92,6 +92,9 @@
   unsigned long long* d_wave = d_prof + 32 * static_cast<size_t>(FR_PROF_FRAMES) + 32 * static_cast<size_t>(s0);
   std::vector<unsigned long long> tw(32 * cnt);
   HIPCHK(hipMemcpy(tw.data(), d_wave, sizeof(unsigned long long) * 32 * cnt, hipMemcpyDeviceToHost));
+  unsigned long long* d_fill = d_prof + 64 * static_cast<size_t>(FR_PROF_FRAMES) + 32 * static_cast<size_t>(s0);
+  std::vector<unsigned long long> tf(32 * cnt);
+  HIPCHK(hipMemcpy(tf.data(), d_fill, sizeof(unsigned long long) * 32 * cnt, hipMemcpyDeviceToHost));
   if (const char* rawf = std::getenv("VOFOD_LDS_PROF_RAW"))
   {
     struct RawLog
@@ -250,6 +253,18 @@
         std::fprintf(fp, ", ");
         Quantiles(lag).json(fp, "start_after_frame_end");
         std::fprintf(fp, "}");
+        static const char* const fnames[vc::EXC_N] = {"started", "fast", "rounds", "max_visited", "max_stack", "redone", "lds", "global"};
+        std::fprintf(fp, ", \"fills\": {");
+        for (int i = 0; i < vc::EXC_N; i++)
+        {
+          std::vector<double> v;
+          for (auto& b : byd)
+            if (t[32 * b.second + 22])
+              v.push_back(static_cast<double>(tf[32 * b.second + i]));
+          std::fprintf(fp, "%s", i ? ", " : "");
+          Quantiles(v).json(fp, fnames[i]);
+        }
+        std::fprintf(fp, "}");
       }
       std::fprintf(fp, "}\n");
       std::fclose(fp);
@@ -257,6 +272,7 @@
   }
   HIPCHK(hipMemset(d_prof + 32 * static_cast<size_t>(s0), 0, sizeof(unsigned long long) * 32 * cnt));
   HIPCHK(hipMemset(d_wave, 0, sizeof(unsigned long long) * 32 * cnt));
+  HIPCHK(hipMemset(d_fill, 0, sizeof(unsigned long long) * 32 * cnt));
   return VOFOD_OK;
 }
 
diff --git a/vofod_amd/csrc/frames_collect.h b/vofod_amd/csrc/frames_collect.h
--- a/vofod_amd/csrc/frames_collect.h
+++ b/vofod_amd/csrc/frames_collect.h
@@ -283,7 +283,7 @@
   HIPCHK(hipMemcpyAsync(eb.d_jobs, w.jobs.data(), sizeof(vc::ExploreJob) * w.jobs.size(), hipMemcpyHostToDevice, h->stream));
   HIPCHK(hipMemcpyAsync(eb.d_job_begin, w.job_begin.data(), sizeof(uint32_t) * (n + 1), hipMemcpyHostToDevice, h->stream));
   HIPCHK(hipMemcpyAsync(eb.d_members, w.job_members.data(), sizeof(int) * w.job_members.size(), hipMemcpyHostToDevice, h->stream));
-  const vc::ExploreParams ep = explore_params(*call.dp, thr_new, no_update);
+  const vc::ExploreParams ep = explore_params(h, *call.dp, thr_new, no_update);
   KLAUNCH(h, vc::k_explore, dim3(n), dim3(64), ep, h->mg, eb.d_jobs, eb.d_job_begin, eb.d_job_begin + 1, eb.d_members, h->d_map, eb.d_overlay, eb.d_stack, eb.d_explored, eb.d_touched,
           eb.d_ovl_list, eb.d_ovl_count, eb.d_results, eb.d_visited);
   HIPCHK(hipMemcpyAsync(w.results.data(), eb.d_results, sizeof(vc::ExploreResult) * w.jobs.size(), hipMemcpyDeviceToHost, h->stream));
diff --git a/vofod_amd/csrc/frames_launch.h b/vofod_amd/csrc/frames_launch.h
--- a/vofod_amd/csrc/frames_launch.h
+++ b/vofod_amd/csrc/frames_launch.h
@@ -77,9 +77,12 @@
   return VOFOD_OK;
 }
 
-vc::ExploreParams explore_params(const vofod_dyn_params& dp, float thr_new, bool no_update)
-{
+vc::ExploreParams explore_params(const vofod_handle* h, const vofod_dyn_params& dp, float thr_new, bool no_update)
+{
+  static const bool lds_off = std::getenv("VOFOD_EXPLORE_LDS") && std::strcmp(std::getenv("VOFOD_EXPLORE_LDS"), "0") == 0;
   vc::ExploreParams ep{};
+  ep.use_lds = lds_off ? 0 : 1;
+  ep.counts = h->prof.on ? static_cast<unsigned long long*>(h->d_fill_counts) : nullptr;
   ep.thr_unknown = static_cast<float>(dp.voxel_map__thresholds__frontiers);
   ep.thr_ground = thr_new;
   ep.frontier_value = static_cast<float>(dp.voxel_map__thresholds__frontiers);
@@ -486,14 +489,26 @@
   else
     HIPCHK(hipStreamWaitEvent(h->stream, h->ev_explore, 0));
   const vt::TailParams tp = tail_params(h, dp);
-  const vc::ExploreParams ep = explore_params(dp, static_cast<float>(dp.voxel_map__thresholds__new_obstacles), plan.no_update);
+  const vc::ExploreParams ep = explore_params(h, dp, static_cast<float>(dp.voxel_map__thresholds__new_obstacles), plan.no_update);
   static const bool diag_no_tail = std::getenv("VOFOD_DIAG_NO_TAIL") != nullptr;
   if (diag_no_tail && n >= 128u)
     ;
   else if (plan.tail == vplan::Tail::Far)
+  {
+    static const bool tail_lds_ok = [] {
+      hipFuncAttributes fa{};
+      if (vtd::TAIL_WPB > 8 || hipFuncGetAttributes(&fa, reinterpret_cast<const void*>(vtd::k_tail_far)) != hipSuccess)
+        return true;
+      if (fa.sharedSizeBytes > 80u * 1024u)
+        std::fprintf(stderr, "[vofod] k_tail_far occupies %zu B of LDS: two of its workgroups no longer share a CU\n", static_cast<size_t>(fa.sharedSizeBytes));
+      return fa.sharedSizeBytes <= 80u * 1024u;
+    }();
+    if (!tail_lds_ok)
+      return VOFOD_ERR_DEVICE;
     KLAUNCH(h, vtd::k_tail_far, dim3((n + vtd::TAIL_WPB - 1) / vtd::TAIL_WPB), dim3(64 * vtd::TAIL_WPB), g, ws.d_hdrs, ws.d_args, ws.d_table, ws.d_cand, ws.va, h->mg, tp, ep, eb.d_jobs, eb.d_members, h->d_map, eb.d_overlay, eb.d_stack, eb.d_explored, eb.d_touched,
             eb.d_ovl_list, eb.d_ovl_count, eb.d_results, eb.d_visited, ws.d_dets, ws.h_dets_dev, plan.far_single ? ws.d_tailc : static_cast<vtd::TailCluster*>(nullptr),
             (ws.prof_deferred && h->d_prof_ccl && !plan.far_single) ? h->d_prof_ccl + 32 * static_cast<size_t>(ws.prof_slot0) : static_cast<unsigned long long*>(nullptr));
+  }
   else
   {
     KLAUNCH(h, vtd::k_tail_prep, dim3(n), dim3(vtd::TP_THREADS), g, ws.d_hdrs, ws.d_args, ws.d_table, ws.d_cand, ws.va, h->mg, tp, eb.d_jobs, ws.d_job_be, ws.d_job_be + ws.F, eb.d_members, ws.d_tailc,
diff --git a/vofod_amd/csrc/kernels_classify.h b/vofod_amd/csrc/kernels_classify.h
--- a/vofod_amd/csrc/kernels_classify.h
+++ b/vofod_amd/csrc/kernels_classify.h
@@ -2,6 +2,7 @@
 #include <hip/hip_runtime.h>
 
 #include "common.h"
+#include "explore_lds.h"
 
 namespace vc
 {
@@ -36,6 +37,21 @@
   double ray_score;
   int32_t no_update;
   uint32_t stack_cap;
+  int32_t use_lds;
+  unsigned long long* counts;
+};
+
+enum ExploreCount
+{
+  EXC_STARTED = 0,
+  EXC_FAST,
+  EXC_ROUNDS,
+  EXC_MAX_VISITED,
+  EXC_MAX_STACK,
+  EXC_REDONE,
+  EXC_LDS,
+  EXC_GLOBAL,
+  EXC_N
 };
 
 __device__ __forceinline__ void wave_sync()
@@ -45,16 +61,22 @@
   __builtin_amdgcn_fence(__ATOMIC_ACQUIRE, "workgroup");
 }
 
+__device__ __forceinline__ constexpr int nbx(int q) { return q == 0 ? 1 : q == 3 ? -1 : 0; }
+__device__ __forceinline__ constexpr int nby(int q) { return q == 1 ? 1 : q == 4 ? -1 : 0; }
+__device__ __forceinline__ constexpr int nbz(int q) { return q == 2 ? 1 : q == 5 ? -1 : 0; }
+
 __device__ __forceinline__ uint32_t pack_rel(int dx, int dy, int dz) { return static_cast<uint32_t>((dx + 128) | ((dy + 128) << 8) | ((dz + 128) << 16)); }
 
 __device__ __forceinline__ void explore_frame(const ExploreParams& ep, const MapGeom& mg, const ExploreJob* __restrict__ jobs, const uint32_t jb, const uint32_t je, const int* __restrict__ members,
                                               float* __restrict__ map, unsigned long long* __restrict__ overlay_all, uint32_t* __restrict__ stack_all, uint32_t* __restrict__ explored_all,
                                               uint32_t* __restrict__ touched_all, uint32_t* __restrict__ ovl_list_all, uint32_t* __restrict__ ovl_count_all, ExploreResult* __restrict__ results,
-                                              uint32_t* __restrict__ visited_all, const uint32_t slot, uint8_t* s_float, uint8_t* s_walk)
+                                              uint32_t* __restrict__ visited_all, const uint32_t slot, uint8_t* s_float, uint8_t* s_walk,
+                                              uint32_t* s_fill, unsigned long long* frame_counts)
 {
   const int lane = threadIdx.x & 63;
   if (jb == je)
     return;
+  uint32_t cnt[EXC_N] = {};
   const uint64_t ovl_words = (mg.n + 63) >> 6;
   unsigned long long* overlay = overlay_all + static_cast<uint64_t>(slot) * ovl_words;
   uint32_t* stack = stack_all + static_cast<uint64_t>(slot) * ep.stack_cap;
@@ -102,8 +124,10 @@
         }
         const int first = __ffsll(static_cast<long long>(need)) - 1;
         m += first;
+        cnt[EXC_STARTED]++;
         if (__shfl(kind, first) == 1)
         {
+          cnt[EXC_FAST]++;
           floating = false;
           break;
         }
@@ -147,114 +171,241 @@
         wave_sync();
         if (any_walk)
         {
+          cnt[EXC_FAST]++;
           floating = false;
           break;
         }
       }
-      uint32_t n_stack = 1, n_expl = 0, n_touched = 1;
-      if (lane == 0)
-      {
-        stack[0] = pack_rel(0, 0, 0);
-        const uint32_t c = (EX_MAX_R * EX_SIDE + EX_MAX_R) * EX_SIDE + EX_MAX_R;
-        atomicOr(&visited[c >> 5], 1u << (c & 31));
-        touched[0] = c;
-      }
-      wave_sync();
       bool connected = false;
-      while (n_stack > 0 && !connected)
-      {
-        const uint32_t take = min(n_stack, 64u);
-        const uint32_t base = n_stack - take;
-        n_stack = base;
-        bool have = static_cast<uint32_t>(lane) < take;
-        int dx = 0, dy = 0, dz = 0;
-        float val = 0.0f;
-        if (have)
-        {
-          const uint32_t e = stack[base + lane];
-          dx = static_cast<int>(e & 255u) - 128;
-          dy = static_cast<int>((e >> 8) & 255u) - 128;
-          dz = static_cast<int>((e >> 16) & 255u) - 128;
-          val = map_read((static_cast<uint64_t>(oz + dz) * mg.sy + (oy + dy)) * mg.sx + (ox + dx));
-        }
-        const bool ground = have && val > ep.thr_ground;
-        const bool unknown = have && !ground && val > ep.thr_unknown;
-        const int md = abs(dx) + abs(dy) + abs(dz);
-        const bool rim = unknown && static_cast<float>(md) == max_voxel_dist - 1.0f;
-        if (__ballot(ground || rim))
-        {
-          connected = true;
-          break;
-        }
-        const unsigned long long um = __ballot(unknown);
-        if (unknown)
-        {
-          const uint32_t pos = n_expl + __popcll(um & ((1ull << lane) - 1ull));
-          if (pos < ep.stack_cap)
-            explored[pos] = pack_rel(dx, dy, dz);
-        }
-        n_expl += __popcll(um);
-        uint32_t mine[6];
-        int n_mine = 0;
-        if (unknown)
-        {
-          const int nb[6][3] = {{1, 0, 0}, {0, 1, 0}, {0, 0, 1}, {-1, 0, 0}, {0, -1, 0}, {0, 0, -1}};
-          uint32_t oldw[6], bitq[6];
-          bool okq[6];
+      uint32_t n_expl = 0;
+      bool in_lds = false;
+      if (s_fill && ep.use_lds)
+      {
+        uint32_t* tab = s_fill;
+        uint32_t* stk = s_fill + vxl::EXL_SLOTS;
+        {
+          uint4* t4 = reinterpret_cast<uint4*>(tab);
+          for (uint32_t w = lane; w < vxl::EXL_SLOTS / 4; w += 64)
+            t4[w] = make_uint4(vxl::EXL_EMPTY, vxl::EXL_EMPTY, vxl::EXL_EMPTY, vxl::EXL_EMPTY);
+        }
+        wave_sync();
+        if (lane == 0)
+        {
+          stk[0] = pack_rel(0, 0, 0);
+          tab[vxl::exl_home(pack_rel(0, 0, 0), vxl::EXL_SLOTS)] = pack_rel(0, 0, 0);
+        }
+        wave_sync();
+        auto cas = [](uint32_t* p, uint32_t expected, uint32_t desired) { return atomicCAS(p, expected, desired); };
+        uint32_t n_stack = 1, n_vis = 1;
+        in_lds = true;
+        while (n_stack > 0)
+        {
+          uint32_t base;
+          const uint32_t take = vxl::exl_pop(n_stack, base);
+          cnt[EXC_ROUNDS]++;
+          const bool have = static_cast<uint32_t>(lane) < take;
+          int dx = 0, dy = 0, dz = 0;
+          float val = 0.0f;
+          if (have)
+          {
+            const uint32_t e = stk[base + lane];
+            dx = static_cast<int>(e & 255u) - 128;
+            dy = static_cast<int>((e >> 8) & 255u) - 128;
+            dz = static_cast<int>((e >> 16) & 255u) - 128;
+            val = map_read((static_cast<uint64_t>(oz + dz) * mg.sy + (oy + dy)) * mg.sx + (ox + dx));
+          }
+          const bool ground = have && val > ep.thr_ground;
+          const bool unknown = have && !ground && val > ep.thr_unknown;
+          const int md = abs(dx) + abs(dy) + abs(dz);
+          const bool rim = unknown && static_cast<float>(md) == max_voxel_dist - 1.0f;
+          if (__ballot(ground || rim))
+          {
+            connected = true;
+            break;
+          }
+          const unsigned long long um = __ballot(unknown);
+          if (unknown)
+          {
+            const uint32_t pos = n_expl + __popcll(um & ((1ull << lane) - 1ull));
+            if (pos < ep.stack_cap)
+              explored[pos] = pack_rel(dx, dy, dz);
+          }
+          n_expl += __popcll(um);
+          uint32_t newm = 0;
+          bool full = false;
+          if (unknown)
+          {
+            uint32_t oldq[6];
+            bool okq[6];
+#pragma unroll
+            for (int q = 0; q < 6; q++)
+            {
+              const int tx = dx + nbx(q), ty = dy + nby(q), tz = dz + nbz(q);
+              const int ax = ox + tx, ay = oy + ty, az = oz + tz;
+              const int tmd = abs(tx) + abs(ty) + abs(tz);
+              okq[q] = !(ax < 0 || ax > mg.sx - 1 || ay < 0 || ay > mg.sy - 1 || az < 0 || az > mg.sz - 1) && static_cast<float>(tmd) <= max_voxel_dist;
+              const uint32_t key = pack_rel(tx, ty, tz);
+              oldq[q] = okq[q] ? cas(&tab[vxl::exl_home(key, vxl::EXL_SLOTS)], vxl::EXL_EMPTY, key) : key;
+            }
+#pragma unroll
+            for (int q = 0; q < 6; q++)
+              if (okq[q])
+              {
+                const int r = vxl::exl_insert_rest(tab, vxl::EXL_SLOTS, pack_rel(dx + nbx(q), dy + nby(q), dz + nbz(q)), oldq[q], cas);
+                if (r == vxl::EXL_NEW)
+                  newm |= 1u << q;
+                full |= r == vxl::EXL_FULL;
+              }
+          }
+          const uint32_t n_mine = __popc(newm);
+          uint32_t incl = n_mine;
+#pragma unroll
+          for (int s = 1; s < 64; s <<= 1)
+          {
+            const uint32_t t = __shfl_up(incl, s);
+            if (lane >= s)
+              incl += t;
+          }
+          const uint32_t total = __shfl(incl, 63);
+          n_vis += total;
+          if (__ballot(full) != 0ull || !vxl::exl_visited_fits(n_vis) || !vxl::exl_stack_fits(n_stack, total))
+          {
+            in_lds = false;
+            break;
+          }
+          uint32_t at = n_stack + incl - n_mine;
 #pragma unroll
           for (int q = 0; q < 6; q++)
-          {
-            const int tx = dx + nb[q][0], ty = dy + nb[q][1], tz = dz + nb[q][2];
-            const int ax = ox + tx, ay = oy + ty, az = oz + tz;
-            const int tmd = abs(tx) + abs(ty) + abs(tz);
-            okq[q] = !(ax < 0 || ax > mg.sx - 1 || ay < 0 || ay > mg.sy - 1 || az < 0 || az > mg.sz - 1) && static_cast<float>(tmd) <= max_voxel_dist;
-            const uint32_t c = okq[q] ? ((tz + EX_MAX_R) * EX_SIDE + (ty + EX_MAX_R)) * EX_SIDE + (tx + EX_MAX_R) : 0u;
-            bitq[q] = 1u << (c & 31);
-            oldw[q] = okq[q] ? atomicOr(&visited[c >> 5], bitq[q]) : 0xffffffffu;
-          }
+            if (newm & (1u << q))
+              stk[at++] = pack_rel(dx + nbx(q), dy + nby(q), dz + nbz(q));
+          n_stack += total;
+          cnt[EXC_MAX_STACK] = max(cnt[EXC_MAX_STACK], n_stack);
+          wave_sync();
+        }
+        wave_sync();
+        if (in_lds)
+        {
+          cnt[EXC_LDS]++;
+          cnt[EXC_MAX_VISITED] = max(cnt[EXC_MAX_VISITED], n_vis);
+        }
+        else
+        {
+          cnt[EXC_REDONE]++;
+          connected = false;
+          n_expl = 0;
+        }
+      }
+      if (!in_lds)
+      {
+        cnt[EXC_GLOBAL]++;
+        uint32_t n_stack = 1, n_touched = 1;
+        if (lane == 0)
+        {
+          stack[0] = pack_rel(0, 0, 0);
+          const uint32_t c = (EX_MAX_R * EX_SIDE + EX_MAX_R) * EX_SIDE + EX_MAX_R;
+          atomicOr(&visited[c >> 5], 1u << (c & 31));
+          touched[0] = c;
+        }
+        wave_sync();
+        while (n_stack > 0 && !connected)
+        {
+          cnt[EXC_ROUNDS]++;
+          const uint32_t take = min(n_stack, 64u);
+          const uint32_t base = n_stack - take;
+          n_stack = base;
+          bool have = static_cast<uint32_t>(lane) < take;
+          int dx = 0, dy = 0, dz = 0;
+          float val = 0.0f;
+          if (have)
+          {
+            const uint32_t e = stack[base + lane];
+            dx = static_cast<int>(e & 255u) - 128;
+            dy = static_cast<int>((e >> 8) & 255u) - 128;
+            dz = static_cast<int>((e >> 16) & 255u) - 128;
+            val = map_read((static_cast<uint64_t>(oz + dz) * mg.sy + (oy + dy)) * mg.sx + (ox + dx));
+          }
+          const bool ground = have && val > ep.thr_ground;
+          const bool unknown = have && !ground && val > ep.thr_unknown;
+          const int md = abs(dx) + abs(dy) + abs(dz);
+          const bool rim = unknown && static_cast<float>(md) == max_voxel_dist - 1.0f;
+          if (__ballot(ground || rim))
+          {
+            connected = true;
+            break;
+          }
+          const unsigned long long um = __ballot(unknown);
+          if (unknown)
+          {
+            const uint32_t pos = n_expl + __popcll(um & ((1ull << lane) - 1ull));
+            if (pos < ep.stack_cap)
+              explored[pos] = pack_rel(dx, dy, dz);
+          }
+          n_expl += __popcll(um);
+          uint32_t newm = 0;
+          if (unknown)
+          {
+            uint32_t oldw[6], bitq[6];
+            bool okq[6];
+#pragma unroll
+            for (int q = 0; q < 6; q++)
+            {
+              const int tx = dx + nbx(q), ty = dy + nby(q), tz = dz + nbz(q);
+              const int ax = ox + tx, ay = oy + ty, az = oz + tz;
+              const int tmd = abs(tx) + abs(ty) + abs(tz);
+              okq[q] = !(ax < 0 || ax > mg.sx - 1 || ay < 0 || ay > mg.sy - 1 || az < 0 || az > mg.sz - 1) && static_cast<float>(tmd) <= max_voxel_dist;
+              const uint32_t c = okq[q] ? ((tz + EX_MAX_R) * EX_SIDE + (ty + EX_MAX_R)) * EX_SIDE + (tx + EX_MAX_R) : 0u;
+              bitq[q] = 1u << (c & 31);
+              oldw[q] = okq[q] ? atomicOr(&visited[c >> 5], bitq[q]) : 0xffffffffu;
+            }
+#pragma unroll
+            for (int q = 0; q < 6; q++)
+              if (okq[q] && !(oldw[q] & bitq[q]))
+                newm |= 1u << q;
+          }
+          const uint32_t n_mine = __popc(newm);
+          uint32_t incl = n_mine;
+#pragma unroll
+          for (int s = 1; s < 64; s <<= 1)
+          {
+            const uint32_t t = __shfl_up(incl, s);
+            if (lane >= s)
+              incl += t;
+          }
+          const uint32_t total = __shfl(incl, 63);
+          uint32_t at = n_stack + incl - n_mine;
+          uint32_t tat = n_touched + incl - n_mine;
 #pragma unroll
           for (int q = 0; q < 6; q++)
-            if (okq[q] && !(oldw[q] & bitq[q]))
-              mine[n_mine++] = pack_rel(dx + nb[q][0], dy + nb[q][1], dz + nb[q][2]);
-        }
-        uint32_t incl = static_cast<uint32_t>(n_mine);
-#pragma unroll
-        for (int s = 1; s < 64; s <<= 1)
-        {
-          const uint32_t t = __shfl_up(incl, s);
-          if (lane >= s)
-            incl += t;
-        }
-        const uint32_t total = __shfl(incl, 63);
-        uint32_t at = n_stack + incl - n_mine;
-        uint32_t tat = n_touched + incl - n_mine;
-        for (int q = 0; q < n_mine; q++, at++, tat++)
-        {
-          if (at < ep.stack_cap)
-            stack[at] = mine[q];
-          else
-            overflow = 1;
-          if (tat < ep.stack_cap)
-          {
-            const int tx = static_cast<int>(mine[q] & 255u) - 128, ty = static_cast<int>((mine[q] >> 8) & 255u) - 128, tz = static_cast<int>((mine[q] >> 16) & 255u) - 128;
-            touched[tat] = ((tz + EX_MAX_R) * EX_SIDE + (ty + EX_MAX_R)) * EX_SIDE + (tx + EX_MAX_R);
-          }
-        }
-        n_stack = min(n_stack + total, ep.stack_cap);
-        n_touched += total;
-        wave_sync();
-      }
-      wave_sync();
-      if (n_touched <= ep.stack_cap)
-      {
-        for (uint32_t e = lane; e < n_touched; e += 64)
-          __hip_atomic_store(&visited[touched[e] >> 5], 0u, __ATOMIC_RELAXED, __HIP_MEMORY_SCOPE_AGENT);
-      }
-      else
-        for (uint32_t w = lane; w < EX_WORDS; w += 64)
-          __hip_atomic_store(&visited[w], 0u, __ATOMIC_RELAXED, __HIP_MEMORY_SCOPE_AGENT);
-      __threadfence_block();
-      wave_sync();
+            if (newm & (1u << q))
+            {
+              const int tx = dx + nbx(q), ty = dy + nby(q), tz = dz + nbz(q);
+              if (at < ep.stack_cap)
+                stack[at] = pack_rel(tx, ty, tz);
+              else
+                overflow = 1;
+              if (tat < ep.stack_cap)
+                touched[tat] = ((tz + EX_MAX_R) * EX_SIDE + (ty + EX_MAX_R)) * EX_SIDE + (tx + EX_MAX_R);
+              at++;
+              tat++;
+            }
+          n_stack = min(n_stack + total, ep.stack_cap);
+          n_touched += total;
+          cnt[EXC_MAX_STACK] = max(cnt[EXC_MAX_STACK], n_stack);
+          wave_sync();
+        }
+        cnt[EXC_MAX_VISITED] = max(cnt[EXC_MAX_VISITED], n_touched);
+        wave_sync();
+        if (n_touched <= ep.stack_cap)
+        {
+          for (uint32_t e = lane; e < n_touched; e += 64)
+            __hip_atomic_store(&visited[touched[e] >> 5], 0u, __ATOMIC_RELAXED, __HIP_MEMORY_SCOPE_AGENT);
+        }
+        else
+          for (uint32_t w = lane; w < EX_WORDS; w += 64)
+            __hip_atomic_store(&visited[w], 0u, __ATOMIC_RELAXED, __HIP_MEMORY_SCOPE_AGENT);
+        __threadfence_block();
+        wave_sync();
+      }
       if (connected)
       {
         floating = false;
@@ -301,12 +452,31 @@
       continue;
     const int nx = job.box_hi[0] - job.box_lo[0] + 1, ny = job.box_hi[1] - job.box_lo[1] + 1, nz = job.box_hi[2] - job.box_lo[2] + 1;
     const uint32_t cells = static_cast<uint32_t>(nx) * ny * nz;
+    const bool marked = s_fill && ep.use_lds && cells <= 32u * vxl::EXL_WORDS;
+    if (marked)
+    {
+      wave_sync();
+      for (uint32_t w = lane; w < (cells + 31u) >> 5; w += 64)
+        s_fill[w] = 0u;
+      wave_sync();
+      for (uint32_t m = lane; m < job.n_members; m += 64)
+      {
+        const int* o = &members[3 * (job.member_off + m)];
+        const int bx = o[0] - job.box_lo[0], by = o[1] - job.box_lo[1], bz = o[2] - job.box_lo[2];
+        if (bx >= 0 && bx < nx && by >= 0 && by < ny && bz >= 0 && bz < nz)
+        {
+          const uint32_t c = (static_cast<uint32_t>(bz) * ny + by) * nx + bx;
+          atomicOr(&s_fill[c >> 5], 1u << (c & 31));
+        }
+      }
+      wave_sync();
+    }
     double acc = 0.0;
     for (uint32_t c = lane; c < cells; c += 64)
     {
       const int x = job.box_lo[0] + static_cast<int>(c % nx), y = job.box_lo[1] + static_cast<int>((c / nx) % ny), z = job.box_lo[2] + static_cast<int>(c / (nx * ny));
-      bool is_member = false;
-      for (uint32_t m = 0; m < job.n_members; m++)
+      bool is_member = marked && ((s_fill[c >> 5] >> (c & 31)) & 1u);
+      for (uint32_t m = 0; !marked && m < job.n_members; m++)
       {
         const int* o = &members[3 * (job.member_off + m)];
         is_member |= (o[0] == x && o[1] == y && o[2] == z);
@@ -334,17 +504,30 @@
     if (lane == 0)
       ovl_count_all[slot] = 0;
   }
+  if (lane == 0 && (frame_counts || ep.counts))
+#pragma unroll
+    for (int i = 0; i < EXC_N; i++)
+    {
+      if (frame_counts)
+        frame_counts[i] = cnt[i];
+      if (ep.counts && (i == EXC_MAX_VISITED || i == EXC_MAX_STACK))
+        atomicMax(&ep.counts[i], static_cast<unsigned long long>(cnt[i]));
+      else if (ep.counts && cnt[i])
+        atomicAdd(&ep.counts[i], static_cast<unsigned long long>(cnt[i]));
+    }
 }
 
-__global__ __attribute__((amdgpu_waves_per_eu(8, 8))) __launch_bounds__(64) void k_explore(const ExploreParams ep, const MapGeom mg, const ExploreJob* __restrict__ jobs, const uint32_t* __restrict__ job_begin, const uint32_t* __restrict__ job_end,
+__global__ __attribute__((amdgpu_waves_per_eu(4, 8))) __launch_bounds__(64) void k_explore(const ExploreParams ep, const MapGeom mg, const ExploreJob* __restrict__ jobs, const uint32_t* __restrict__ job_begin, const uint32_t* __restrict__ job_end,
                                                 const int* __restrict__ members, float* __restrict__ map, unsigned long long* __restrict__ overlay_all,
                                                 uint32_t* __restrict__ stack_all, uint32_t* __restrict__ explored_all, uint32_t* __restrict__ touched_all,
                                                 uint32_t* __restrict__ ovl_list_all, uint32_t* __restrict__ ovl_count_all, ExploreResult* __restrict__ results, uint32_t* __restrict__ visited_all)
 {
   __shared__ uint8_t s_float[EX_MAX_JOBS];
   __shared__ uint8_t s_walk[6 * 32];
+  __shared__ __attribute__((aligned(16))) uint32_t s_fill[vxl::EXL_WORDS];
   const uint32_t slot = blockIdx.x;
-  explore_frame(ep, mg, jobs, job_begin[slot], job_end[slot], members, map, overlay_all, stack_all, explored_all, touched_all, ovl_list_all, ovl_count_all, results, visited_all, slot, s_float, s_walk);
+  explore_frame(ep, mg, jobs, job_begin[slot], job_end[slot], members, map, overlay_all, stack_all, explored_all, touched_all, ovl_list_all, ovl_count_all, results, visited_all, slot, s_float, s_walk, s_fill,
+                nullptr);
 }
 
 }
diff --git a/vofod_amd/csrc/kernels_frame.h b/vofod_amd/csrc/kernels_frame.h
--- a/vofod_amd/csrc/kernels_frame.h
+++ b/vofod_amd/csrc/kernels_frame.h
@@ -41,7 +41,7 @@
 constexpr uint16_t FR_VBASE_NONE = 0xffffu;
 constexpr uint32_t CF_LABEL_NONE = 0xffffffffu;
 constexpr uint32_t FR_PROF_FRAMES = 4096;
-constexpr size_t FR_PROF_WORDS = 2 * 32 * static_cast<size_t>(FR_PROF_FRAMES);
+constexpr size_t FR_PROF_WORDS = 3 * 32 * static_cast<size_t>(FR_PROF_FRAMES);
 
 struct FrameScratch
 {
diff --git a/vofod_amd/csrc/kernels_tail.h b/vofod_amd/csrc/kernels_tail.h
--- a/vofod_amd/csrc/kernels_tail.h
+++ b/vofod_amd/csrc/kernels_tail.h
@@ -12,10 +12,13 @@
 #define TAIL_WPB_DEF 8
 #endif
 constexpr int TAIL_WPB = TAIL_WPB_DEF;
-#if TAIL_WPB_DEF >= 16
+#ifndef TAIL_OCC_DEF
+#define TAIL_OCC_DEF 4
+#endif
+#if TAIL_WPB_DEF >= 16 || TAIL_OCC_DEF == 0
 #define TAIL_OCC_ATTR
 #else
-#define TAIL_OCC_ATTR __attribute__((amdgpu_waves_per_eu(5, 5)))
+#define TAIL_OCC_ATTR __attribute__((amdgpu_waves_per_eu(TAIL_OCC_DEF, TAIL_OCC_DEF)))
 #endif
 using namespace vk;
 
@@ -298,7 +301,13 @@
 {
   __shared__ uint8_t s_float_all[TAIL_WPB][TP_MAXC];
   __shared__ uint8_t s_walk_all[TAIL_WPB][6 * 32];
-  __shared__ float s_pts_all[TAIL_WPB][TAIL_STAGE][3];
+  union WaveArea
+  {
+    float pts[TAIL_STAGE][3];
+    uint32_t fill[vxl::EXL_WORDS];
+  };
+  static_assert(TAIL_WPB * (sizeof(WaveArea) + TP_MAXC + 6 * 32) <= (TAIL_WPB <= 8 ? 76u : 152u) * 1024u, "k_tail_far's LDS as declared: two workgroups per CU (160 KB) up to 8 waves");
+  __shared__ __attribute__((aligned(16))) WaveArea s_area_all[TAIL_WPB];
   const uint32_t f = blockIdx.x * TAIL_WPB + (threadIdx.x >> 6);
   if (f >= g.n_frames)
     return;
@@ -338,7 +347,7 @@
     }
     m_begin = incl - m_count;
   }
-  float (*s_pts)[3] = s_pts_all[threadIdx.x >> 6];
+  float (*s_pts)[3] = s_area_all[threadIdx.x >> 6].pts;
   {
     const uint32_t total = min(static_cast<uint32_t>(__shfl(m_begin + m_count, 63)), static_cast<uint32_t>(TAIL_STAGE));
     for (uint32_t i = lane; i < total; i += 64)
@@ -406,7 +415,8 @@
   vc::wave_sync();
   if (prof)
     tp1 = wall_clock64();
-  vc::explore_frame(ep, mg, jobs, jb, jb + n_jobs, members_out, map, overlay_all, stack_all, explored_all, touched_all, ovl_list_all, ovl_count_all, results, visited_all, f, s_float, s_walk);
+  vc::explore_frame(ep, mg, jobs, jb, jb + n_jobs, members_out, map, overlay_all, stack_all, explored_all, touched_all, ovl_list_all, ovl_count_all, results, visited_all, f, s_float, s_walk,
+                     s_area_all[threadIdx.x >> 6].fill, prof ? prof + 64 * static_cast<size_t>(FR_PROF_FRAMES) + 32 * static_cast<size_t>(f) : nullptr);
   __threadfence_block();
   vc::wave_sync();
   if (prof)
diff --git a/vofod_amd/csrc/vofod_hip.hip b/vofod_amd/csrc/vofod_hip.hip
--- a/vofod_amd/csrc/vofod_hip.hip
+++ b/vofod_amd/csrc/vofod_hip.hip
@@ -420,6 +420,7 @@
 struct vofod_handle
 {
   DevBuf<unsigned long long> d_prof_slab, d_prof_ccl;
+  DevBuf<unsigned long long> d_fill_counts;
   bool cf_off = false;
   uint64_t cf_off_bg = 0;
   bool bgcount_stale = false;
```

Result: slower. 1.192 million frames/s (-1.4%).
